# retir/Style-Big-GAN

Hardware: AMD Instinct MI355X
Metric: images/sec (G+D step) StyleGAN2-ADA 256x256 bf16 (higher is better)
Workload: dtype bf16; 1 GPU; configs/sg2ada.yaml @ 256x256: sg2_classic G (skip) + D (orig), softplus + R1(0.01)/4, idle Greg slot /16 (G lr x 16/17), global batch 64 = 1 rank(s) x 2 round(s) x batch_gpu 32 (the rounds of a phase evaluated in one pass, minibatch-std groups and loss those of the separate rounds), bf16 from 8x8 up (num_fp16_res 6; the reference recipe defaults to 4), conv_clamp 256, ADA off; global_batch=64, per_rank_batch=64, parallelism=dp1

## Files before the change

include/sbg_hip.h:

```cpp
#ifndef SBG_HIP_H
#define SBG_HIP_H

#include <stdint.h>

#ifdef __cplusplus
extern "C" {
#endif

typedef void* sbg_stream_t;

enum sbg_status {
    SBG_OK = 0,
    SBG_ERR_INVALID = 1,
    SBG_ERR_UNSUPPORTED = 2,
    SBG_ERR_LAUNCH = 3
};

enum sbg_dtype { SBG_F32 = 0, SBG_F16 = 1, SBG_BF16 = 2 };

enum sbg_act {
    SBG_ACT_LINEAR = 1, SBG_ACT_RELU = 2, SBG_ACT_LRELU = 3, SBG_ACT_TANH = 4, SBG_ACT_SIGMOID = 5,
    SBG_ACT_ELU = 6, SBG_ACT_SELU = 7, SBG_ACT_SOFTPLUS = 8, SBG_ACT_SWISH = 9
};

int         sbg_version(void);
const char* sbg_last_error(void);

int sbg_bias_act(const void* x, const void* b, const void* xref, const void* yref, const void* dy,
                 void* y, int dtype, int grad, int act, float alpha, float gain, float clamp,
                 int64_t sizeX, int sizeB, int64_t stepB, sbg_stream_t stream);

typedef struct sbg_upfirdn2d_params {
    const void*  x;
    const float* f;
    void*        y;
    int dtype;
    int upx, upy, downx, downy, padx0, pady0;
    int flip;
    float gain;
    int     inSize[4];      int64_t inStride[4];
    int     filterSize[2];  int     filterStride[2];
    int     outSize[4];     int64_t outStride[4];
    const float* oscale; const float* noise; int64_t noise_stride_n; const float* bias;
    int act; float alpha, act_gain, clamp;
    int     filter_exact16;
    const void* dact_y; float* dact_partial; int dact_act; float dact_alpha, dact_gain, dact_clamp;
    const float* post_scale;
} sbg_upfirdn2d_params;
int sbg_upfirdn2d_tail_supported(const sbg_upfirdn2d_params* p);
int64_t sbg_upfirdn2d_dact_rows(const sbg_upfirdn2d_params* p);
int sbg_upfirdn2d(const sbg_upfirdn2d_params* p, sbg_stream_t stream);

int sbg_upfirdn2d_separable_supported(int up, int down, int taps);
int sbg_upfirdn2d_separable(const float* x, const float* f, float* y, int M, int IH, int IW, int OH, int OW, int taps,
                            int up, int down, int padx0, int pady0, int flip, float gain, sbg_stream_t stream);

#define SBG_MAX_TAPS 16
typedef struct sbg_conv_params {
    const void* x; const void* w; void* y;
    const float* oscale;
    int xdtype, ydtype;
    int N, IH, IW, Cin, Cout, OH, OW;
    int64_t xs_n, xs_h, xs_w;
    int64_t ys_n, ys_h, ys_w;
    int64_t ws_slab, ws_co;
    int stride;
    int ntaps;
    int tap_dy[SBG_MAX_TAPS], tap_dx[SBG_MAX_TAPS], tap_slab[SBG_MAX_TAPS];
    int accumulate;
    const float* bias; const float* noise; int64_t noise_stride_n;
    int act; float alpha, gain, clamp;
    void* workspace; int ksplit;
    int nphase; int ph_ntaps[4], ph_oh[4], ph_ow[4]; int64_t ph_yoff[4];
} sbg_conv_params;
int64_t sbg_conv2d_igemm_workspace(const sbg_conv_params* p);
int     sbg_conv2d_igemm(const sbg_conv_params* p, sbg_stream_t stream);


typedef struct sbg_wgrad_params {
    const void* a; const void* b; float* out; void* workspace;
    int dtype;
    int N, PH, PW, Ca, BH, BW, Cb;
    int64_t as_n, as_h, as_w;
    int64_t bs_n, bs_h, bs_w;
    int stride;
    int ntaps;
    int tap_dy[SBG_MAX_TAPS], tap_dx[SBG_MAX_TAPS];
    int accumulate;
} sbg_wgrad_params;
int64_t sbg_conv2d_wgrad_workspace(const sbg_wgrad_params* p);
int     sbg_conv2d_wgrad(const sbg_wgrad_params* p, sbg_stream_t stream);


int sbg_scale_nc(const void* x, const float* a, const float* z, void* y, int dtype, int layout,
                 int N, int C, int64_t HW, int64_t z_stride_n, sbg_stream_t stream);
int sbg_scale_shift_nc(const void* x, const float* a, const float* b, void* y, int dtype, int layout,
                       int N, int C, int64_t HW, sbg_stream_t stream);

int sbg_dot_hw_splits(int layout, int N, int C, int64_t HW);
int sbg_dot_hw(const void* u, const void* v, float* partial, int dtype, int layout,
               int N, int C, int64_t HW, sbg_stream_t stream);
int sbg_moments_hw(const void* x, float* r, int dtype, int N, int C, int64_t HW, sbg_stream_t stream);

typedef struct sbg_gg_problem {
    const float *a0, *b0, *a1, *b1;
    float* c; const float* bias; float* rowsum;
    int64_t a0_rs, a0_cs, b0_rs, b0_cs, a1_rs, a1_cs, b1_rs, b1_cs, c_rs, c_cs;
    int M, N, K0, K1, nterms;
    float alpha0, alpha1, bias_scale, rowsum_scale;
} sbg_gg_problem;
int sbg_grouped_gemm(const sbg_gg_problem* problems, int count, sbg_stream_t stream);

int sbg_dot_hw_scale_supported(int C);
int sbg_dot_hw_scale(const void* u, const void* v, const float* scale, void* y, float* partial, int dtype,
                     int N, int C, int64_t HW, sbg_stream_t stream);


int sbg_modconv_bwd_supported(int C);
int sbg_modconv_bwd(const void* dy, const void* y, const float* dcoef, const float* noise, const float* bias,
                    void* d2, float* partial, float* dnoise, int dtype, int N, int C, int64_t HW, int64_t noise_stride_n,
                    int act, float alpha, float gain, float clamp, sbg_stream_t stream);
int sbg_modconv_bwd_prescaled(const void* dy, const void* y, const float* prescale, const float* dcoef, const float* noise, const float* bias,
                              void* d2, float* partial, float* partial3, float* dnoise, int dtype, int N, int C, int64_t HW,
                              int64_t noise_stride_n, int act, float alpha, float gain, float clamp, sbg_stream_t stream);

int64_t sbg_sn_workspace(int rows, int cols);
int sbg_sn_power_iteration(const float* W, const float* u, float* v, float* u_new, float* sigma, void* workspace,
                           int rows, int cols, float eps, sbg_stream_t stream);

int64_t sbg_mbstd_workspace(int N, int C, int HW, int G, int F);
int sbg_mbstd_fwd(const float* x, float* y, void* workspace, int N, int C, int HW, int G, int F, sbg_stream_t stream);
int sbg_mbstd_bwd(const float* x, const float* dy, float* dx, int N, int C, int HW, int G, int F, sbg_stream_t stream);

int sbg_split_bf16_cat(const float* x, void* y, int64_t outer, int64_t C, int64_t inner, int nseg, const int* order, sbg_stream_t stream);
int sbg_split_bf16_cat_nd(const float* x, const int64_t* shape, const int64_t* xstrides, int cat_dim, void* y, int nseg, const int* order, sbg_stream_t stream);

int sbg_attention_supported(int Q, int M, int D, int DV);
int sbg_attention_fwd(const float* theta, const float* phi, const float* g, float* out, int N, int Q, int M, int D, int DV,
                      sbg_stream_t stream);
int sbg_attention_bwd_supported(int Q, int M, int D, int DV);
int64_t sbg_attention_bwd_workspace(int N, int Q);
int sbg_attention_bwd(const float* theta, const float* phi, const float* g, const float* dout, float* dtheta, float* dphi, float* dg,
                      void* workspace, int N, int Q, int M, int D, int DV, sbg_stream_t stream);

int sbg_pack_weight(const float* w, void* out, int out_dtype, int A, int B, int KH, int KW,
                    int64_t sA, int64_t sB, int64_t sKH, int64_t sKW, int Bp, float gain, float* w2, sbg_stream_t stream);
int sbg_unpack_wgrad(const float* dwp, int64_t dwp_tap_stride, int64_t dwp_row_stride, float* dw, const float* w, const float* dw2,
                     int A, int B, int KH, int KW, int64_t sA, int64_t sB, int64_t sKH, int64_t sKW, float gain, sbg_stream_t stream);

int sbg_demod_coefs(const float* styles, const float* w2, float* dcoefs, int N, int O, int I, float eps, sbg_stream_t stream);
int sbg_demod_coefs_bwd(const float* g, const float* dcoefs, const float* styles, const float* w2, float* dstyles, float* dw2,
                        int N, int O, int I, sbg_stream_t stream);

int sbg_torgb_supported(int C, int O);
int sbg_torgb_bwd_blocks(int N, int C, int64_t HW);
int sbg_torgb_fwd(const void* x, const float* wmod, const float* bias, float* y, int dtype, int N, int C, int O, int64_t HW,
                  float clamp, sbg_stream_t stream);
int sbg_torgb_bwd(const void* x, const float* wmod, const float* dy, const float* y, void* dx, float* partial, int dtype,
                  int N, int C, int O, int64_t HW, float clamp, sbg_stream_t stream);

int sbg_fromrgb_supported(int Ci, int Co, int act);
int sbg_fromrgb_bwd_blocks(int N, int64_t HW);
int sbg_fromrgb_fwd(const float* img, const float* w, const float* bias, void* y, int dtype, int N, int Ci, int Co, int64_t HW,
                    int act, float alpha, float gain, float clamp, sbg_stream_t stream);
int sbg_fromrgb_bwd(const float* img, const float* w, const void* dy, const void* y, float* dimg, float* partial, int dtype,
                    int N, int Ci, int Co, int64_t HW, int act, float alpha, float gain, float clamp, sbg_stream_t stream);

typedef struct sbg_grid_sample_params {
    const void* x; const float* grid; const float* theta; const void* dy;
    void* y; void* dx; float* dgrid;
    int N, C, IH, IW, OH, OW;
    int64_t xs_n, xs_c, xs_h, xs_w;
    int64_t ys_n, ys_c, ys_h, ys_w;
    const float* theta_host;
} sbg_grid_sample_params;
int sbg_grid_sample2d(const sbg_grid_sample_params* p, sbg_stream_t stream);
int sbg_grid_sample2d_bwd(const sbg_grid_sample_params* p, sbg_stream_t stream);
int sbg_grid_sample2d_bwd_overwrites(const sbg_grid_sample_params* p);

int sbg_color_transform(const float* x, const float* M, float* y, int N, int64_t HW, sbg_stream_t stream);

int sbg_filter1d_batch(const float* x, const float* taps, float* y, int M, int H, int W, int T, int axis, int pad,
                       int planes_per_filter, int flip, sbg_stream_t stream);

int sbg_ppl_slerp_endpoints(const float* z0, const float* z1, const float* t, float eps, float* out, int B, int D, sbg_stream_t stream);
int sbg_ppl_lerp_endpoints(const float* w0, const float* w1, const float* t, float eps, float* out, int B, int64_t L, sbg_stream_t stream);
int sbg_ppl_prep_images(const float* img, float* out, int N, int C, int H, int W, int64_t sn, int64_t sc, int64_t sh, int64_t sw,
                        int crop, int factor, sbg_stream_t stream);
int64_t sbg_ppl_dist_workspace(int B, int64_t F);
int sbg_ppl_dist(const float* feats, float* dist, void* workspace, int B, int64_t F, float eps2, sbg_stream_t stream);

int64_t sbg_proj_noise_reg_workspace(const int* res, int nbuf);
int sbg_proj_noise_reg(const float* const* bufs, const int* res, int nbuf, float* means, float* reg, void* workspace, sbg_stream_t stream);
int sbg_proj_noise_reg_bwd(const float* const* bufs, float* const* grads, const int* res, int nbuf, const float* means, const float* g,
                           const void* workspace, sbg_stream_t stream);
int64_t sbg_proj_noise_normalize_workspace(const int* res, int nbuf);
int sbg_proj_noise_normalize(float* const* bufs, const int* res, int nbuf, void* workspace, sbg_stream_t stream);
int64_t sbg_proj_sqdist_workspace(int64_t F);
int sbg_proj_sqdist(const float* t, const float* s, float* dist, void* workspace, int64_t F, sbg_stream_t stream);
int sbg_proj_sqdist_bwd(const float* t, const float* s, const float* g, float* ds, int64_t F, sbg_stream_t stream);

enum sbg_quant_rule { SBG_QUANT_GRID = 0, SBG_QUANT_CLAMP = 1 };
int sbg_img_quantize_tile(const float* img, uint8_t* canvas, int N, int C, int H, int W, int64_t sn, int64_t sc, int64_t sh, int64_t sw,
                          int gw, int gh, int cell0, int rule, float lo, float scale, sbg_stream_t stream);
int sbg_ws_truncate_mix(const float* W, const float* w_avg, float psi, const int* rows, const int* cols, const int* mask, float* out,
                        int S, int L, int D, int R, int Cn, sbg_stream_t stream);

int sbg_u8_resample_h(const uint8_t* src, int64_t src_img_stride, int64_t src_pitch, uint8_t* dst, int64_t dst_img_stride, int64_t dst_pitch,
                      int N, int rows, int in_w, int out_w, int C, const int* bounds, const int* coeffs_t, int ksize, int strip, int span,
                      sbg_stream_t stream);
int sbg_u8_resample_v(const uint8_t* src, int64_t src_img_stride, int64_t src_pitch, uint8_t* dst, int64_t dst_img_stride, int64_t dst_pitch,
                      int N, int row_bytes, int in_h, int out_h, const int* bounds, const int* coeffs, int ksize, sbg_stream_t stream);

int64_t sbg_knn_workspace(int R, int C, int k, int membership);
int sbg_knn_kth_radius(const void* rows, const void* manifold, int R, int C, int64_t F, int k, void* out, void* workspace, sbg_stream_t stream);
int sbg_knn_in_manifold(const void* probes, const void* manifold, const void* radius, int P, int C, int64_t F, uint8_t* out, void* workspace,
                        sbg_stream_t stream);
int64_t sbg_knn_probe_workspace(int P, int C);
int sbg_knn_probe(const void* probes, const void* manifold, const void* radius, int P, int C, int64_t F, int32_t* count, void* nearest,
                  void* workspace, sbg_stream_t stream);

int64_t sbg_grad_finish_records(int64_t n);
int sbg_grad_finish_sweep(float* flat, int64_t n, float scale, double* partials, sbg_stream_t stream);
int sbg_grad_finish_merge(const double* partials, int64_t records, double* result, sbg_stream_t stream);

int sbg_u8_gather_images(const uint8_t* store, int64_t S, int C, int H, int W, const int32_t* slot, const uint8_t* flip, int B, void* out,
                         int out_f32, const float* lut, sbg_stream_t stream);

#define SBG_DIFFAUG_WORDS 12
int64_t sbg_diffaug_workspace(int N, int C, int H, int W);
int sbg_diffaug_fwd(const float* x, const int32_t* table, float* y, float* workspace, int N, int C, int H, int W, int drop_b, sbg_stream_t stream);
int sbg_diffaug_adj(const float* g, const int32_t* table, float* dx, float* workspace, int N, int C, int H, int W, sbg_stream_t stream);

enum sbg_kernel_kind {
    SBG_K_BIAS_ACT = 1, SBG_K_UPFIRDN2D = 2, SBG_K_CONV_IGEMM = 3, SBG_K_CONV_WGRAD = 4, SBG_K_WGRAD_REDUCE = 5,
    SBG_K_SCALE_NC = 6, SBG_K_DOT_HW = 7, SBG_K_SN_POWER = 9, SBG_K_ATTENTION = 10, SBG_K_GRID_SAMPLE = 11, SBG_K_FILTER1D = 12, SBG_K_COLOR = 13, SBG_K_WEIGHT_PREP = 14, SBG_K_TORGB = 15, SBG_K_FROMRGB = 16,
    SBG_K_GROUPED_GEMM = 17, SBG_K_PPL = 18,
    SBG_K_PROJECTOR = 19,
    SBG_K_IMAGE_EXPORT = 20,
    SBG_K_RESAMPLE = 21,
    SBG_K_PR = 22,
    SBG_K_GRAD_FINISH = 23,
    SBG_K_RESIDENT = 24,
    SBG_K_DIFFAUG = 25
};
typedef struct sbg_prof_record {
    int    kind;
    int    dims[7];
    double flops;
    double bytes;
    float  ms;
    int    pad;
} sbg_prof_record;
int sbg_prof_enable(int on);
int sbg_prof_fetch(sbg_prof_record* out, int max);

#ifdef __cplusplus
}
#endif
#endif
```

style-big-gan_amd/_lib.py:

```python
import ctypes
import os
import threading

import torch

_HERE = os.path.dirname(os.path.abspath(__file__))
LIB_PATH = os.environ.get("SBG_HIP_LIBRARY") or os.path.join(_HERE, "libsbg_hip.so")

SBG_F32, SBG_F16, SBG_BF16 = 0, 1, 2
SBG_MAX_TAPS = 16

_DTYPES = {torch.float32: SBG_F32, torch.float16: SBG_F16, torch.bfloat16: SBG_BF16}


def dtype_code(dtype):
    try:
        return _DTYPES[dtype]
    except KeyError:
        raise RuntimeError(f"style_big_gan_amd: unsupported dtype {dtype} (float32 / float16 / bfloat16 only)")


class UpfirdnParams(ctypes.Structure):
    _fields_ = [
        ("x", ctypes.c_void_p), ("f", ctypes.c_void_p), ("y", ctypes.c_void_p),
        ("dtype", ctypes.c_int),
        ("upx", ctypes.c_int), ("upy", ctypes.c_int), ("downx", ctypes.c_int), ("downy", ctypes.c_int),
        ("padx0", ctypes.c_int), ("pady0", ctypes.c_int),
        ("flip", ctypes.c_int), ("gain", ctypes.c_float),
        ("inSize", ctypes.c_int * 4), ("inStride", ctypes.c_int64 * 4),
        ("filterSize", ctypes.c_int * 2), ("filterStride", ctypes.c_int * 2),
        ("outSize", ctypes.c_int * 4), ("outStride", ctypes.c_int64 * 4),
        ("oscale", ctypes.c_void_p), ("noise", ctypes.c_void_p), ("noise_stride_n", ctypes.c_int64), ("bias", ctypes.c_void_p),
        ("act", ctypes.c_int), ("alpha", ctypes.c_float), ("act_gain", ctypes.c_float), ("clamp", ctypes.c_float),
        ("filter_exact16", ctypes.c_int),
        ("dact_y", ctypes.c_void_p), ("dact_partial", ctypes.c_void_p), ("dact_act", ctypes.c_int),
        ("dact_alpha", ctypes.c_float), ("dact_gain", ctypes.c_float), ("dact_clamp", ctypes.c_float),
        ("post_scale", ctypes.c_void_p),
    ]


class ConvParams(ctypes.Structure):
    _fields_ = [
        ("x", ctypes.c_void_p), ("w", ctypes.c_void_p), ("y", ctypes.c_void_p), ("oscale", ctypes.c_void_p),
        ("xdtype", ctypes.c_int), ("ydtype", ctypes.c_int),
        ("N", ctypes.c_int), ("IH", ctypes.c_int), ("IW", ctypes.c_int), ("Cin", ctypes.c_int), ("Cout", ctypes.c_int),
        ("OH", ctypes.c_int), ("OW", ctypes.c_int),
        ("xs_n", ctypes.c_int64), ("xs_h", ctypes.c_int64), ("xs_w", ctypes.c_int64),
        ("ys_n", ctypes.c_int64), ("ys_h", ctypes.c_int64), ("ys_w", ctypes.c_int64),
        ("ws_slab", ctypes.c_int64), ("ws_co", ctypes.c_int64),
        ("stride", ctypes.c_int), ("ntaps", ctypes.c_int),
        ("tap_dy", ctypes.c_int * SBG_MAX_TAPS), ("tap_dx", ctypes.c_int * SBG_MAX_TAPS), ("tap_slab", ctypes.c_int * SBG_MAX_TAPS),
        ("accumulate", ctypes.c_int),
        ("bias", ctypes.c_void_p), ("noise", ctypes.c_void_p), ("noise_stride_n", ctypes.c_int64),
        ("act", ctypes.c_int), ("alpha", ctypes.c_float), ("gain", ctypes.c_float), ("clamp", ctypes.c_float),
        ("workspace", ctypes.c_void_p), ("ksplit", ctypes.c_int),
        ("nphase", ctypes.c_int), ("ph_ntaps", ctypes.c_int * 4), ("ph_oh", ctypes.c_int * 4), ("ph_ow", ctypes.c_int * 4), ("ph_yoff", ctypes.c_int64 * 4),
    ]


class WgradParams(ctypes.Structure):
    _fields_ = [
        ("a", ctypes.c_void_p), ("b", ctypes.c_void_p), ("out", ctypes.c_void_p), ("workspace", ctypes.c_void_p),
        ("dtype", ctypes.c_int),
        ("N", ctypes.c_int), ("PH", ctypes.c_int), ("PW", ctypes.c_int), ("Ca", ctypes.c_int),
        ("BH", ctypes.c_int), ("BW", ctypes.c_int), ("Cb", ctypes.c_int),
        ("as_n", ctypes.c_int64), ("as_h", ctypes.c_int64), ("as_w", ctypes.c_int64),
        ("bs_n", ctypes.c_int64), ("bs_h", ctypes.c_int64), ("bs_w", ctypes.c_int64),
        ("stride", ctypes.c_int), ("ntaps", ctypes.c_int),
        ("tap_dy", ctypes.c_int * SBG_MAX_TAPS), ("tap_dx", ctypes.c_int * SBG_MAX_TAPS),
        ("accumulate", ctypes.c_int),
    ]


class GridSampleParams(ctypes.Structure):
    _fields_ = [
        ("x", ctypes.c_void_p), ("grid", ctypes.c_void_p), ("theta", ctypes.c_void_p), ("dy", ctypes.c_void_p),
        ("y", ctypes.c_void_p), ("dx", ctypes.c_void_p), ("dgrid", ctypes.c_void_p),
        ("N", ctypes.c_int), ("C", ctypes.c_int), ("IH", ctypes.c_int), ("IW", ctypes.c_int), ("OH", ctypes.c_int), ("OW", ctypes.c_int),
        ("xs_n", ctypes.c_int64), ("xs_c", ctypes.c_int64), ("xs_h", ctypes.c_int64), ("xs_w", ctypes.c_int64),
        ("ys_n", ctypes.c_int64), ("ys_c", ctypes.c_int64), ("ys_h", ctypes.c_int64), ("ys_w", ctypes.c_int64),
        ("theta_host", ctypes.c_void_p),
    ]


class GgProblem(ctypes.Structure):
    _fields_ = [("a0", ctypes.c_void_p), ("b0", ctypes.c_void_p), ("a1", ctypes.c_void_p), ("b1", ctypes.c_void_p),
                ("c", ctypes.c_void_p), ("bias", ctypes.c_void_p), ("rowsum", ctypes.c_void_p),
                ("a0_rs", ctypes.c_int64), ("a0_cs", ctypes.c_int64), ("b0_rs", ctypes.c_int64), ("b0_cs", ctypes.c_int64),
                ("a1_rs", ctypes.c_int64), ("a1_cs", ctypes.c_int64), ("b1_rs", ctypes.c_int64), ("b1_cs", ctypes.c_int64),
                ("c_rs", ctypes.c_int64), ("c_cs", ctypes.c_int64),
                ("M", ctypes.c_int), ("N", ctypes.c_int), ("K0", ctypes.c_int), ("K1", ctypes.c_int), ("nterms", ctypes.c_int),
                ("alpha0", ctypes.c_float), ("alpha1", ctypes.c_float), ("bias_scale", ctypes.c_float), ("rowsum_scale", ctypes.c_float)]


class ProfRecord(ctypes.Structure):
    _fields_ = [("kind", ctypes.c_int), ("dims", ctypes.c_int * 7), ("flops", ctypes.c_double), ("bytes", ctypes.c_double),
                ("ms", ctypes.c_float), ("pad", ctypes.c_int)]


KERNEL_KINDS = {1: "bias_act", 2: "upfirdn2d", 3: "conv_igemm", 4: "conv_wgrad", 5: "wgrad_reduce", 6: "scale_nc", 7: "dot_hw", 9: "sn_power", 10: "attention",
                11: "grid_sample", 12: "filter1d", 13: "color", 14: "weight_prep", 15: "torgb", 16: "fromrgb", 17: "grouped_gemm", 18: "ppl",
                19: "projector", 20: "image_export", 21: "resample", 22: "pr", 23: "grad_finish", 24: "resident", 25: "diffaug"}
RESIDENT_PATHS = {1: "dword", 2: "byte"}
PPL_VARIANTS = {0: "slerp", 1: "lerp", 2: "prep", 3: "dist"}
PROJ_VARIANTS = {0: "reg", 1: "reg_bwd", 2: "normalize", 3: "sqdist", 4: "sqdist_bwd"}
IMG_VARIANTS = {0: "quantize_tile", 1: "truncate_mix"}
QUANT_RULES = {"grid": 0, "clamp": 1}
RESAMPLE_VARIANTS = {0: "h", 1: "v"}
PR_VARIANTS = {0: "single", 1: "split", 2: "merge", 3: "norms"}
GRAD_FINISH_VARIANTS = {0: "sweep", 1: "merge"}
DIFFAUG_VARIANTS = {0: "sum", 1: "apply", 2: "adj_sum", 3: "adj_apply", 4: "single", 5: "adj_single"}
DIFFAUG_WORDS = 12
ATT_VARIANTS = {0: "single", 1: "stream", 2: "stream_stats", 3: "stream_dq", 4: "stream_dkv"}

_lib = None
_lock = threading.Lock()

_c = ctypes
SYMBOLS = [
    ("sbg_version", _c.c_int, []),
    ("sbg_last_error", _c.c_char_p, []),
    ("sbg_bias_act", _c.c_int, [_c.c_void_p] * 6 + [_c.c_int, _c.c_int, _c.c_int, _c.c_float, _c.c_float, _c.c_float,
                                                   _c.c_int64, _c.c_int, _c.c_int64, _c.c_void_p]),
    ("sbg_upfirdn2d_tail_supported", _c.c_int, [_c.POINTER(UpfirdnParams)]),
    ("sbg_upfirdn2d", _c.c_int, [_c.POINTER(UpfirdnParams), _c.c_void_p]),
    ("sbg_upfirdn2d_dact_rows", _c.c_int64, [_c.POINTER(UpfirdnParams)]),
    ("sbg_upfirdn2d_separable_supported", _c.c_int, [_c.c_int] * 3),
    ("sbg_upfirdn2d_separable", _c.c_int, [_c.c_void_p] * 3 + [_c.c_int] * 11 + [_c.c_float, _c.c_void_p]),
    ("sbg_conv2d_igemm_workspace", _c.c_int64, [_c.POINTER(ConvParams)]),
    ("sbg_conv2d_igemm", _c.c_int, [_c.POINTER(ConvParams), _c.c_void_p]),
    ("sbg_conv2d_wgrad_workspace", _c.c_int64, [_c.POINTER(WgradParams)]),
    ("sbg_conv2d_wgrad", _c.c_int, [_c.POINTER(WgradParams), _c.c_void_p]),
    ("sbg_scale_nc", _c.c_int, [_c.c_void_p] * 4 + [_c.c_int, _c.c_int, _c.c_int, _c.c_int, _c.c_int64, _c.c_int64, _c.c_void_p]),
    ("sbg_scale_shift_nc", _c.c_int, [_c.c_void_p] * 4 + [_c.c_int, _c.c_int, _c.c_int, _c.c_int, _c.c_int64, _c.c_void_p]),
    ("sbg_sn_workspace", _c.c_int64, [_c.c_int, _c.c_int]),
    ("sbg_sn_power_iteration", _c.c_int, [_c.c_void_p] * 6 + [_c.c_int, _c.c_int, _c.c_float, _c.c_void_p]),
    ("sbg_mbstd_workspace", _c.c_int64, [_c.c_int] * 5),
    ("sbg_mbstd_fwd", _c.c_int, [_c.c_void_p] * 3 + [_c.c_int] * 5 + [_c.c_void_p]),
    ("sbg_mbstd_bwd", _c.c_int, [_c.c_void_p] * 3 + [_c.c_int] * 5 + [_c.c_void_p]),
    ("sbg_split_bf16_cat", _c.c_int, [_c.c_void_p, _c.c_void_p, _c.c_int64, _c.c_int64, _c.c_int64, _c.c_int, _c.POINTER(_c.c_int), _c.c_void_p]),
    ("sbg_split_bf16_cat_nd", _c.c_int, [_c.c_void_p, _c.POINTER(_c.c_int64), _c.POINTER(_c.c_int64), _c.c_int, _c.c_void_p, _c.c_int, _c.POINTER(_c.c_int), _c.c_void_p]),
    ("sbg_attention_supported", _c.c_int, [_c.c_int] * 4),
    ("sbg_attention_fwd", _c.c_int, [_c.c_void_p] * 4 + [_c.c_int] * 5 + [_c.c_void_p]),
    ("sbg_attention_bwd_supported", _c.c_int, [_c.c_int] * 4),
    ("sbg_attention_bwd_workspace", _c.c_int64, [_c.c_int, _c.c_int]),
    ("sbg_attention_bwd", _c.c_int, [_c.c_void_p] * 8 + [_c.c_int] * 5 + [_c.c_void_p]),
    ("sbg_dot_hw_splits", _c.c_int, [_c.c_int, _c.c_int, _c.c_int, _c.c_int64]),
    ("sbg_dot_hw", _c.c_int, [_c.c_void_p] * 3 + [_c.c_int, _c.c_int, _c.c_int, _c.c_int, _c.c_int64, _c.c_void_p]),
    ("sbg_moments_hw", _c.c_int, [_c.c_void_p, _c.c_void_p, _c.c_int, _c.c_int, _c.c_int, _c.c_int64, _c.c_void_p]),
    ("sbg_grouped_gemm", _c.c_int, [_c.c_void_p, _c.c_int, _c.c_void_p]),
    ("sbg_dot_hw_scale_supported", _c.c_int, [_c.c_int]),
    ("sbg_dot_hw_scale", _c.c_int, [_c.c_void_p] * 5 + [_c.c_int, _c.c_int, _c.c_int, _c.c_int64, _c.c_void_p]),
    ("sbg_modconv_bwd_supported", _c.c_int, [_c.c_int]),
    ("sbg_modconv_bwd", _c.c_int, [_c.c_void_p] * 8 + [_c.c_int, _c.c_int, _c.c_int, _c.c_int64, _c.c_int64, _c.c_int, _c.c_float, _c.c_float, _c.c_float, _c.c_void_p]),
    ("sbg_modconv_bwd_prescaled", _c.c_int, [_c.c_void_p] * 10 + [_c.c_int, _c.c_int, _c.c_int, _c.c_int64, _c.c_int64, _c.c_int, _c.c_float, _c.c_float, _c.c_float, _c.c_void_p]),
    ("sbg_pack_weight", _c.c_int, [_c.c_void_p, _c.c_void_p, _c.c_int, _c.c_int, _c.c_int, _c.c_int, _c.c_int] + [_c.c_int64] * 4
     + [_c.c_int, _c.c_float, _c.c_void_p, _c.c_void_p]),
    ("sbg_unpack_wgrad", _c.c_int, [_c.c_void_p, _c.c_int64, _c.c_int64, _c.c_void_p, _c.c_void_p, _c.c_void_p] + [_c.c_int] * 4
     + [_c.c_int64] * 4 + [_c.c_float, _c.c_void_p]),
    ("sbg_demod_coefs", _c.c_int, [_c.c_void_p] * 3 + [_c.c_int] * 3 + [_c.c_float, _c.c_void_p]),
    ("sbg_demod_coefs_bwd", _c.c_int, [_c.c_void_p] * 6 + [_c.c_int] * 3 + [_c.c_void_p]),
    ("sbg_torgb_supported", _c.c_int, [_c.c_int, _c.c_int]),
    ("sbg_torgb_bwd_blocks", _c.c_int, [_c.c_int, _c.c_int, _c.c_int64]),
    ("sbg_torgb_fwd", _c.c_int, [_c.c_void_p] * 4 + [_c.c_int] * 4 + [_c.c_int64, _c.c_float, _c.c_void_p]),
    ("sbg_torgb_bwd", _c.c_int, [_c.c_void_p] * 6 + [_c.c_int] * 4 + [_c.c_int64, _c.c_float, _c.c_void_p]),
    ("sbg_fromrgb_supported", _c.c_int, [_c.c_int] * 3),
    ("sbg_fromrgb_bwd_blocks", _c.c_int, [_c.c_int, _c.c_int64]),
    ("sbg_fromrgb_fwd", _c.c_int, [_c.c_void_p] * 4 + [_c.c_int] * 4 + [_c.c_int64, _c.c_int, _c.c_float, _c.c_float, _c.c_float, _c.c_void_p]),
    ("sbg_fromrgb_bwd", _c.c_int, [_c.c_void_p] * 6 + [_c.c_int] * 4 + [_c.c_int64, _c.c_int, _c.c_float, _c.c_float, _c.c_float, _c.c_void_p]),
    ("sbg_grid_sample2d", _c.c_int, [_c.POINTER(GridSampleParams), _c.c_void_p]),
    ("sbg_grid_sample2d_bwd", _c.c_int, [_c.POINTER(GridSampleParams), _c.c_void_p]),
    ("sbg_grid_sample2d_bwd_overwrites", _c.c_int, [_c.POINTER(GridSampleParams)]),
    ("sbg_color_transform", _c.c_int, [_c.c_void_p] * 3 + [_c.c_int, _c.c_int64, _c.c_void_p]),
    ("sbg_filter1d_batch", _c.c_int, [_c.c_void_p] * 3 + [_c.c_int] * 8 + [_c.c_void_p]),
    ("sbg_ppl_slerp_endpoints", _c.c_int, [_c.c_void_p] * 3 + [_c.c_float, _c.c_void_p, _c.c_int, _c.c_int, _c.c_void_p]),
    ("sbg_ppl_lerp_endpoints", _c.c_int, [_c.c_void_p] * 3 + [_c.c_float, _c.c_void_p, _c.c_int, _c.c_int64, _c.c_void_p]),
    ("sbg_ppl_prep_images", _c.c_int, [_c.c_void_p] * 2 + [_c.c_int] * 4 + [_c.c_int64] * 4 + [_c.c_int, _c.c_int, _c.c_void_p]),
    ("sbg_ppl_dist_workspace", _c.c_int64, [_c.c_int, _c.c_int64]),
    ("sbg_ppl_dist", _c.c_int, [_c.c_void_p] * 3 + [_c.c_int, _c.c_int64, _c.c_float, _c.c_void_p]),
    ("sbg_proj_noise_reg_workspace", _c.c_int64, [_c.c_void_p, _c.c_int]),
    ("sbg_proj_noise_reg", _c.c_int, [_c.c_void_p] * 2 + [_c.c_int] + [_c.c_void_p] * 4),
    ("sbg_proj_noise_reg_bwd", _c.c_int, [_c.c_void_p] * 3 + [_c.c_int] + [_c.c_void_p] * 4),
    ("sbg_proj_noise_normalize_workspace", _c.c_int64, [_c.c_void_p, _c.c_int]),
    ("sbg_proj_noise_normalize", _c.c_int, [_c.c_void_p] * 2 + [_c.c_int] + [_c.c_void_p] * 2),
    ("sbg_proj_sqdist_workspace", _c.c_int64, [_c.c_int64]),
    ("sbg_proj_sqdist", _c.c_int, [_c.c_void_p] * 4 + [_c.c_int64, _c.c_void_p]),
    ("sbg_proj_sqdist_bwd", _c.c_int, [_c.c_void_p] * 4 + [_c.c_int64, _c.c_void_p]),
    ("sbg_img_quantize_tile", _c.c_int, [_c.c_void_p] * 2 + [_c.c_int] * 4 + [_c.c_int64] * 4 + [_c.c_int] * 4 + [_c.c_float] * 2 + [_c.c_void_p]),
    ("sbg_ws_truncate_mix", _c.c_int, [_c.c_void_p] * 2 + [_c.c_float] + [_c.c_void_p] * 4 + [_c.c_int] * 5 + [_c.c_void_p]),
    ("sbg_u8_resample_h", _c.c_int, [_c.c_void_p, _c.c_int64, _c.c_int64] * 2 + [_c.c_int] * 5 + [_c.c_void_p] * 2 + [_c.c_int] * 3 + [_c.c_void_p]),
    ("sbg_u8_resample_v", _c.c_int, [_c.c_void_p, _c.c_int64, _c.c_int64] * 2 + [_c.c_int] * 4 + [_c.c_void_p] * 2 + [_c.c_int, _c.c_void_p]),
    ("sbg_knn_workspace", _c.c_int64, [_c.c_int] * 4),
    ("sbg_knn_kth_radius", _c.c_int, [_c.c_void_p] * 2 + [_c.c_int, _c.c_int, _c.c_int64, _c.c_int] + [_c.c_void_p] * 3),
    ("sbg_knn_in_manifold", _c.c_int, [_c.c_void_p] * 3 + [_c.c_int, _c.c_int, _c.c_int64] + [_c.c_void_p] * 3),
    ("sbg_knn_probe_workspace", _c.c_int64, [_c.c_int] * 2),
    ("sbg_knn_probe", _c.c_int, [_c.c_void_p] * 3 + [_c.c_int, _c.c_int, _c.c_int64] + [_c.c_void_p] * 4),
    ("sbg_grad_finish_records", _c.c_int64, [_c.c_int64]),
    ("sbg_grad_finish_sweep", _c.c_int, [_c.c_void_p, _c.c_int64, _c.c_float, _c.c_void_p, _c.c_void_p]),
    ("sbg_grad_finish_merge", _c.c_int, [_c.c_void_p, _c.c_int64, _c.c_void_p, _c.c_void_p]),
    ("sbg_u8_gather_images", _c.c_int, [_c.c_void_p, _c.c_int64, _c.c_int, _c.c_int, _c.c_int, _c.c_void_p, _c.c_void_p, _c.c_int, _c.c_void_p, _c.c_int,
                                        _c.c_void_p, _c.c_void_p]),
    ("sbg_diffaug_workspace", _c.c_int64, [_c.c_int] * 4),
    ("sbg_diffaug_fwd", _c.c_int, [_c.c_void_p] * 4 + [_c.c_int] * 5 + [_c.c_void_p]),
    ("sbg_diffaug_adj", _c.c_int, [_c.c_void_p] * 4 + [_c.c_int] * 4 + [_c.c_void_p]),
    ("sbg_prof_enable", _c.c_int, [_c.c_int]),
    ("sbg_prof_fetch", _c.c_int, [_c.POINTER(ProfRecord), _c.c_int]),
]


def load():
    global _lib
    if _lib is not None:
        return _lib
    with _lock:
        if _lib is not None:
            return _lib
        if not os.path.isfile(LIB_PATH):
            raise RuntimeError(
                f"style_big_gan_amd: HIP extension {LIB_PATH} not found. Build it with "
                f"`make -C {os.path.join(_HERE, 'csrc')}` or `python -c 'import __graft_entry__ as g; g.build()'`. "
                "There is no CPU fallback.")
        lib = ctypes.CDLL(LIB_PATH)
        for name, restype, argtypes in SYMBOLS:
            fn = getattr(lib, name)
            fn.restype = restype
            fn.argtypes = argtypes
        _lib = lib
    return _lib


def check(status, what):
    if status != 0:
        msg = load().sbg_last_error()
        raise RuntimeError(f"{what} failed (status {status}): {msg.decode() if msg else ''}")


def stream_ptr(device=None):
    return ctypes.c_void_p(torch.cuda.current_stream(device).cuda_stream)


def ptr(t):
    return ctypes.c_void_p(t.data_ptr()) if t is not None else None


def require_cuda(t, what):
    if t.device.type != "cuda":
        raise RuntimeError(
            f"{what}: tensor is on '{t.device}'. style_big_gan_amd ops run only as HIP kernels on a ROCm device "
            "(device type 'cuda'); there is no CPU path in the product (the CPU restatement lives in oracle/ and is test-only).")


def require_dtype(t, dtype, what):
    if t.dtype != dtype:
        raise RuntimeError(f"{what}: expects {str(dtype).replace('torch.', '')}, got {t.dtype}")
    return t


def workspace(nbytes, device, what):
    if nbytes < 0:
        check(1, what)
    return torch.empty([max((nbytes + 3) // 4, 1)], dtype=torch.float32, device=device)


def prof_enable(on):
    return load().sbg_prof_enable(int(bool(on)))


def prof_fetch():
    lib = load()
    n = lib.sbg_prof_fetch(None, 0)
    if n <= 0:
        return []
    buf = (ProfRecord * n)()
    n = lib.sbg_prof_fetch(buf, n)
    return [dict(kind=KERNEL_KINDS.get(r.kind, str(r.kind)), dims=tuple(r.dims), flops=r.flops, bytes=r.bytes, ms=r.ms) for r in buf[:n]]
```

style-big-gan_amd/csrc/conv_wgrad.hip:

```cpp
#include "conv_common.h"
#include "lds_asm.h"

namespace {

struct bf16_mfma {}; struct f16_mfma {};
template <class MF> struct Mfma;
template <> struct Mfma<bf16_mfma> {
    static __device__ __forceinline__ float4_t run(short8_t a, short8_t b, float4_t c) {
        return __builtin_amdgcn_mfma_f32_16x16x32_bf16(__builtin_bit_cast(bf16x8_t, a), __builtin_bit_cast(bf16x8_t, b), c, 0, 0, 0);
    }
};
template <> struct Mfma<f16_mfma> {
    static __device__ __forceinline__ float4_t run(short8_t a, short8_t b, float4_t c) {
        return __builtin_amdgcn_mfma_f32_16x16x32_f16(__builtin_bit_cast(f16x8_t, a), __builtin_bit_cast(f16x8_t, b), c, 0, 0, 0);
    }
};

struct WgradArgs {
    const unsigned short* a; const unsigned short* b; float* out; float* ws;
    int N, PH, PW, Ca, BH, BW, Cb;
    int64_t as_n, as_h, as_w, bs_n, bs_h, bs_w;
    int stride, ntaps;
    int tap_dy[SBG_MAX_TAPS], tap_dx[SBG_MAX_TAPS];
    int accumulate;
// ... 196 lines not shown
    const int xblocks = p.PW >> 5;
    const int dy0 = p.tap_dy[0], dx0 = p.tap_dx[0];

    __amdgpu_buffer_rsrc_t ar = __builtin_amdgcn_make_buffer_rsrc((void*)p.a, 0, (int)a_bytes, 0x00020000);
    __amdgpu_buffer_rsrc_t br = __builtin_amdgcn_make_buffer_rsrc((void*)p.b, 0, (int)b_bytes, 0x00020000);

    const int drow = lane >> 3, dchunk = lane & 7;
    auto src_chunk = [&](int R) { return (((dchunk >> 1) ^ ((R >> 1) & 3)) << 1) | (dchunk & 1); };

    struct ChunkC { int py, n, px0; unsigned char* st; };
    auto chunk_coords = [&](int loc) -> ChunkC {
        const int c = chunk_begin + loc;
        const int xb = c % xblocks, rowid = c / xblocks;
        ChunkC r; r.py = rowid % p.PH; r.n = rowid / p.PH; r.px0 = xb << 5; r.st = smem + (loc % NSTAGE) * STAGE;
        return r;
    };
    auto issue_piece = [&](const ChunkC& cc, int i) {
        const int py = cc.py, n = cc.n, px0 = cc.px0;
        unsigned char* st = cc.st;
        {
            const int piece = wave + NWAVE * i;
            if (piece < APIECES) {
                const int R = (piece & 3) * 8 + drow;
                const int ch = ca0 + (piece >> 2) * 64 + src_chunk(R) * 8;
                const unsigned okm = 0u - (unsigned)(ch < p.Ca);
                const unsigned real = (unsigned)(n * (int)p.as_n + py * (int)p.as_h + (px0 + R) * (int)p.as_w + ch) * 2u;
                __builtin_amdgcn_raw_ptr_buffer_load_lds(ar, (lds_void_ptr)(st + piece * 1024), 16, (real & okm) | (SBG_OOB_OFFSET & ~okm), 0, 0, 0);
            } else {
                const int q = piece - APIECES;
                const int r = q / PPR, jb = q - r * PPR;
                const int R = r * PROW + jb * 8 + drow;
                constexpr int NEVEN = (PCOLS + 1) / 2, EVROWS = ((NEVEN + 7) / 8) * 8;
                const int pcol = (S == 1) ? jb * 8 + drow : (jb * 8 < EVROWS ? 2 * (jb * 8 + drow) : 2 * (jb * 8 - EVROWS + drow) + 1);
                const int by = S * py + dy0 + r, bx = S * px0 + dx0 + pcol;
                const int ch = cb0 + src_chunk(R) * 8;
                const unsigned okm = 0u - (unsigned)((q < 3 * PPR) & (pcol < PCOLS) & ((unsigned)by < (unsigned)p.BH) & ((unsigned)bx < (unsigned)p.BW) & (ch < p.Cb));
                const unsigned real = (unsigned)(n * (int)p.bs_n + by * (int)p.bs_h + bx * (int)p.bs_w + ch) * 2u;
                unsigned char* dst = (q < 3 * PPR) ? st + A_BYTES + q * 1024 : smem + DUMP;
                __builtin_amdgcn_raw_ptr_buffer_load_lds(br, (lds_void_ptr)dst, 16, (real & okm) | (SBG_OOB_OFFSET & ~okm), 0, 0, 0);
            }
        }
    };
    auto issue = [&](int loc) {
        const ChunkC cc = chunk_coords(loc);
#pragma unroll
        for (int i = 0; i < PIECES; i++) issue_piece(cc, i);
    };
    constexpr bool late = true;

    const int wa = (wave >> 2) * (BCA / 2), wb = (wave & 3) * 16;
    const int fi = lane & 15, fg = lane >> 4, fq = fi >> 2, fp = fi & 3;
    const unsigned lds_base = (unsigned)(uintptr_t)((lds_void_ptr)smem);
    float4_t acc[NT][TA];
#pragma unroll
    for (int t = 0; t < NT; t++)
#pragma unroll
        for (int i = 0; i < TA; i++) acc[t][i] = float4_t{0.f, 0.f, 0.f, 0.f};

    auto frag_off = [&](int Rrel, int col) {
        const int chunk = (col >> 3) + (fp >> 1);
        const int sw = (((chunk >> 1) ^ ((Rrel >> 1) & 3)) << 1) | (chunk & 1);
        return Rrel * 128 + sw * 16 + (fp & 1) * 8;
    };
    int offA[TA], offB[3];
#pragma unroll
    for (int i = 0; i < TA; i++) {
        const int col = wa + 16 * i;
        offA[i] = (col >> 6) * 4096 + frag_off(4 * fg + fq, col & 63);
    }
#pragma unroll
    for (int d = 0; d < 3; d++) {
        constexpr int EVROWS_ = (((PCOLS + 1) / 2 + 7) / 8) * 8;
        offB[d] = frag_off((S == 1 ? d : (d & 1) * EVROWS_ + (d >> 1)) + 4 * fg + fq, wb);
    }
    auto read_frag = [&](const unsigned char* base, int off, int hi_off) -> short8_t {
        short4_t lo = lds_tr_read(base + off), hi = lds_tr_read(base + off + hi_off);
        return short8_t{lo[0], lo[1], lo[2], lo[3], hi[0], hi[1], hi[2], hi[3]};
    };

#pragma unroll
    for (int s = 0; s < DEPTH; s++) if (s < nloc) issue(s);
    for (int s = 0; s < nloc; s++) {
        {
            const int later = nloc - 1 - s;
            if (DEPTH >= 2 && later >= DEPTH - 1) asm volatile("s_waitcnt vmcnt(%0)" :: "n"((DEPTH - 1) * PIECES) : "memory");
            else if (DEPTH >= 3 && later == DEPTH - 2) asm volatile("s_waitcnt vmcnt(%0)" :: "n"((DEPTH >= 3 ? DEPTH - 2 : 0) * PIECES) : "memory");
            else if (DEPTH >= 4 && later == DEPTH - 3) asm volatile("s_waitcnt vmcnt(%0)" :: "n"((DEPTH >= 4 ? DEPTH - 3 : 0) * PIECES) : "memory");
            else if (DEPTH >= 5 && later == DEPTH - 4) asm volatile("s_waitcnt vmcnt(%0)" :: "n"((DEPTH >= 5 ? DEPTH - 4 : 0) * PIECES) : "memory");
            else                                       asm volatile("s_waitcnt vmcnt(0)" ::: "memory");
        }
        __builtin_amdgcn_s_barrier();
        const bool more = s + DEPTH < nloc;
        ChunkC nxt = chunk_coords(more ? s + DEPTH : s);
        if (more && !late) {
#pragma unroll
            for (int i = 0; i < PIECES; i++) issue_piece(nxt, i);
        }
        const unsigned stage = lds_base + (unsigned)((s % NSTAGE) * STAGE);
        short4_t alo[TA], ahi[TA], blo[3], bhi[3];
        sbg_static_for<TA>([&](auto it) {
            constexpr int i = decltype(it)::value;
            lds_tr_issue<0>(alo[i], stage + (unsigned)offA[i]);
            lds_tr_issue<16 * 128>(ahi[i], stage + (unsigned)offA[i]);
        });
        unsigned pb[3];
#pragma unroll
        for (int d = 0; d < 3; d++) pb[d] = stage + (unsigned)offB[d];
        auto issue_b = [&](auto tt) {
            constexpr int t = decltype(tt)::value, dyi = t / 3, dxi = t % 3, OFF = A_BYTES + dyi * PROW * 128;
            lds_tr_issue<OFF>(blo[t % 3], pb[dxi]);
            lds_tr_issue<OFF + 16 * 128>(bhi[t % 3], pb[dxi]);
        };
        issue_b(std::integral_constant<int, 0>{});
        issue_b(std::integral_constant<int, 1>{});
        sbg_static_for<9>([&](auto tt) {
            constexpr int t = decltype(tt)::value;
            if constexpr (t + 2 < 9) issue_b(std::integral_constant<int, t + 2>{});
            lds_wait<(t + 2 < 9 ? 4 : t + 1 < 9 ? 2 : 0)>(blo[t % 3], bhi[t % 3]);
            const short8_t fb = short8_t{blo[t % 3][0], blo[t % 3][1], blo[t % 3][2], blo[t % 3][3], bhi[t % 3][0], bhi[t % 3][1], bhi[t % 3][2], bhi[t % 3][3]};
#pragma unroll
            for (int i = 0; i < TA; i++) {
                const short8_t fa_i = short8_t{alo[i][0], alo[i][1], alo[i][2], alo[i][3], ahi[i][0], ahi[i][1], ahi[i][2], ahi[i][3]};
                acc[t][i] = Mfma<MF>::run(fa_i, fb, acc[t][i]);
            }
            if (more && late) {
                sbg_static_for<PIECES>([&](auto pt) {
                    constexpr int i = decltype(pt)::value;
                    if constexpr (i * 9 / PIECES == t) issue_piece(nxt, i);
                });
            }
        });
    }

    const bool direct = (p.nsplit == 1);
    float* dst_base = direct ? p.out : p.ws + (int64_t)split * p.ntaps_total * p.Ca * p.Cb;
    const int cb = cb0 + wb + fi;
#pragma unroll
    for (int t = 0; t < NT; t++) {
        if (t >= p.ntaps || cb >= p.Cb) continue;
        float* slab = dst_base + (int64_t)(p.tap0 + t) * p.Ca * p.Cb;
#pragma unroll
        for (int i = 0; i < TA; i++)
#pragma unroll
            for (int e = 0; e < 4; e++) {
                const int ca = ca0 + wa + 16 * i + 4 * fg + e;
                if (ca >= p.Ca) continue;
                float* d = slab + (int64_t)ca * p.Cb + cb;
                const float v = acc[t][i][e];
                *d = (direct && p.accumulate) ? *d + v : v;
            }
    }
}

template <int LANES>
__global__ __launch_bounds__(256) void wgrad_reduce_kernel(const float* ws, float* out, int64_t n, int nsplit, int accumulate)
{
    const int sub = threadIdx.x % LANES;
    const int64_t step = (int64_t)gridDim.x * (256 / LANES);
    for (int64_t i = (int64_t)blockIdx.x * (256 / LANES) + threadIdx.x / LANES; i < n; i += step) {
        float s = 0.f;
        int k = sub;
        for (; k + 7 * LANES < nsplit; k += 8 * LANES) {
            float v[8];
#pragma unroll
            for (int u = 0; u < 8; u++) v[u] = ws[(int64_t)(k + u * LANES) * n + i];
#pragma unroll
            for (int u = 0; u < 8; u++) s += v[u];
        }
        for (; k < nsplit; k += LANES) s += ws[(int64_t)k * n + i];
#pragma unroll
        for (int m = LANES >> 1; m >= 1; m >>= 1) s += __shfl_xor(s, m, 64);
        if (sub == 0) out[i] = accumulate ? out[i] + s : s;
    }
}

template <class MF, int TA, int TB>
__global__ __launch_bounds__(256) void conv_wgrad_thin_kernel(WgradArgs p, int dymin, int dxmin, int RY, int PCOLS, int wave_lds)
{
    extern __shared__ __attribute__((aligned(16))) unsigned char smem[];
    const int tid = threadIdx.x, lane = tid & 63, wave = tid >> 6;
    unsigned short* la = reinterpret_cast<unsigned short*>(smem + wave * wave_lds);
    unsigned short* lb = la + 32 * p.Ca;
    const int slab = blockIdx.x * 4 + wave;
    const int nwaves = gridDim.x * 4;
    const int xblocks = (p.PW + 31) >> 5;
    const int nchunks = p.N * p.PH * xblocks;
    const int fi = lane & 15, fg = lane >> 4;
    const int ca8 = p.Ca >> 3, cb8 = p.Cb >> 3;
    float4_t acc[9][TA][TB];
#pragma unroll
    for (int t = 0; t < 9; t++)
#pragma unroll
        for (int i = 0; i < TA; i++)
#pragma unroll
            for (int j = 0; j < TB; j++) acc[t][i][j] = float4_t{0.f, 0.f, 0.f, 0.f};
    int tdy[9], tdx[9];
#pragma unroll
    for (int t = 0; t < 9; t++) { tdy[t] = (t < p.ntaps ? p.tap_dy[t] : 0) - dymin; tdx[t] = (t < p.ntaps ? p.tap_dx[t] : 0) - dxmin; }

    for (int c = slab; c < nchunks; c += nwaves) {
        const int xb = c % xblocks, rowid = c / xblocks;
        const int py = rowid % p.PH, n = rowid / p.PH;
        const int px0 = xb << 5;
        for (int piece = lane; piece < 32 * ca8; piece += 64) {
            const int px = piece / ca8, ch = (piece - px * ca8) * 8;
            short8_t v = {0, 0, 0, 0, 0, 0, 0, 0};
            if (px0 + px < p.PW) v = *reinterpret_cast<const short8_t*>(p.a + (int64_t)n * p.as_n + (int64_t)py * p.as_h + (int64_t)(px0 + px) * p.as_w + ch);
            *reinterpret_cast<short8_t*>(la + piece * 8) = v;
        }
        const int npieces = RY * PCOLS * cb8;
        for (int piece = lane; piece < npieces; piece += 64) {
            const int ch = (piece % cb8) * 8, pc = piece / cb8;
            const int col = pc % PCOLS, r = pc / PCOLS;
            const int by = p.stride * py + dymin + r, bx = p.stride * px0 + dxmin + col;
            short8_t v = {0, 0, 0, 0, 0, 0, 0, 0};
            if ((unsigned)by < (unsigned)p.BH && (unsigned)bx < (unsigned)p.BW)
                v = *reinterpret_cast<const short8_t*>(p.b + (int64_t)n * p.bs_n + (int64_t)by * p.bs_h + (int64_t)bx * p.bs_w + ch);
            *reinterpret_cast<short8_t*>(lb + piece * 8) = v;
        }
        __builtin_amdgcn_s_waitcnt(0xC07F);
        __builtin_amdgcn_wave_barrier();
        short8_t fa[TA];
#pragma unroll
        for (int i = 0; i < TA; i++)
#pragma unroll
            for (int j = 0; j < 8; j++) fa[i][j] = (short)la[(8 * fg + j) * p.Ca + 16 * i + fi];
#pragma unroll
        for (int t = 0; t < 9; t++) {
            if (t < p.ntaps) {
                const unsigned short* row = lb + (tdy[t] * PCOLS + tdx[t]) * p.Cb;
#pragma unroll
                for (int jb = 0; jb < TB; jb++) {
                    short8_t fb;
#pragma unroll
                    for (int j = 0; j < 8; j++) fb[j] = (short)row[(p.stride * (8 * fg + j)) * p.Cb + 16 * jb + fi];
#pragma unroll
                    for (int i = 0; i < TA; i++) acc[t][i][jb] = Mfma<MF>::run(fa[i], fb, acc[t][i][jb]);
                }
            }
        }
        __builtin_amdgcn_wave_barrier();
    }
    float* dst = p.ws + (int64_t)slab * p.ntaps_total * p.Ca * p.Cb;
#pragma unroll
    for (int t = 0; t < 9; t++) {
        if (t < p.ntaps) {
#pragma unroll
            for (int i = 0; i < TA; i++)
#pragma unroll
                for (int jb = 0; jb < TB; jb++)
#pragma unroll
                    for (int e = 0; e < 4; e++) {
                        const int ca = 16 * i + 4 * fg + e, cb = 16 * jb + fi;
                        if (ca < p.Ca && cb < p.Cb) dst[((int64_t)(p.tap0 + t) * p.Ca + ca) * p.Cb + cb] = acc[t][i][jb][e];
                    }
        }
    }
}

struct ThinPlan { bool ok; int dymin, dxmin, RY, PCOLS, wave_lds, nwg; };

static ThinPlan thin_plan(const sbg_wgrad_params* q)
{
    ThinPlan t; t.ok = false;
    if (q->Ca > 32 || q->Cb > 32 || q->Ca * q->Cb > 512 || q->ntaps > 9 || q->ntaps < 1 || q->stride < 1 || q->stride > 2 || q->N < 1) return t;
    int dy0 = q->tap_dy[0], dy1 = dy0, dx0 = q->tap_dx[0], dx1 = dx0;
    for (int i = 1; i < q->ntaps; i++) {
        if (q->tap_dy[i] < dy0) dy0 = q->tap_dy[i]; if (q->tap_dy[i] > dy1) dy1 = q->tap_dy[i];
        if (q->tap_dx[i] < dx0) dx0 = q->tap_dx[i]; if (q->tap_dx[i] > dx1) dx1 = q->tap_dx[i];
    }
    if (dy1 - dy0 > 2 || dx1 - dx0 > 2) return t;
    t.dymin = dy0; t.dxmin = dx0; t.RY = dy1 - dy0 + 1; t.PCOLS = q->stride * 31 + (dx1 - dx0) + 1;
    t.wave_lds = ((32 * q->Ca + t.RY * t.PCOLS * q->Cb) * 2 + 15) & ~15;
    const int64_t nchunks = (int64_t)q->N * q->PH * ((q->PW + 31) / 32);
    int64_t nwg = (nchunks + 15) / 16;
    if (nwg > 2048) nwg = 2048;
    if (nwg < 1) nwg = 1;
    t.nwg = (int)nwg;
    t.ok = nchunks < INT32_MAX;
    return t;
}

static void plan_split(WgradArgs& a, int bca, int bcb, int target)
{
    a.atiles = (a.Ca + bca - 1) / bca;
    a.btiles = (a.Cb + bcb - 1) / bcb;
    a.nchunks = (int)((a.P + 31) / 32);
    const int tiles = a.atiles * a.btiles;
    int want = (target + tiles - 1) / tiles;
    int maxsplit = a.nchunks / 8; if (maxsplit < 1) maxsplit = 1;
    if (want > maxsplit) want = maxsplit;
    if (want < 1) want = 1;
    a.chunks_per_split = (a.nchunks + want - 1) / want;
    a.nsplit = (a.nchunks + a.chunks_per_split - 1) / a.chunks_per_split;
}

static bool use_big_tile(int ntaps) { return ntaps == 1; }

static int rows_bca(const WgradArgs& a)
{
    return a.Ca >= 128 ? 128 : 64;
}

static constexpr int rows_nstage(int stride, int bca)
{
    if (bca == 128) return 4;
    return stride == 1 ? 4 : 2;
}

static bool rows_kernel_ok(const sbg_wgrad_params* q, const WgradArgs& a)
{
    if ((q->stride != 1 && q->stride != 2) || (q->PW % 32) != 0 || q->ntaps != 9) return false;
    for (int t = 0; t < 9; t++)
        if (q->tap_dy[t] != q->tap_dy[0] + t / 3 || q->tap_dx[t] != q->tap_dx[0] + t % 3) return false;
    if (q->as_n < 0 || q->as_h < 0 || q->as_w < 0 || q->bs_n < 0 || q->bs_h < 0 || q->bs_w < 0) return false;
    const int64_t ab = 2 * ((int64_t)(q->N - 1) * q->as_n + (int64_t)(q->PH - 1) * q->as_h + (int64_t)(q->PW - 1) * q->as_w + q->Ca);
    const int64_t bb = 2 * ((int64_t)(q->N - 1) * q->bs_n + (int64_t)(q->BH - 1) * q->bs_h + (int64_t)(q->BW - 1) * q->bs_w + q->Cb);
    return ab < (int64_t)SBG_OOB_OFFSET && bb < (int64_t)SBG_OOB_OFFSET && a.P > 0;
}

static int fill_args(const sbg_wgrad_params* q, WgradArgs& a)
{
    SBG_CHECK(q && q->a && q->b && q->out, "conv2d_wgrad: null pointer");
    SBG_CHECK(q->dtype == SBG_BF16 || q->dtype == SBG_F16, "conv2d_wgrad: a/b must be bf16 or f16 (fp32 inputs are split by the host)");
    SBG_CHECK(q->N >= 0 && q->PH >= 1 && q->PW >= 1 && q->BH >= 1 && q->BW >= 1, "conv2d_wgrad: bad sizes");
    SBG_CHECK(q->Ca >= 8 && q->Cb >= 8 && (q->Ca % 8) == 0 && (q->Cb % 8) == 0, "conv2d_wgrad: channel counts must be multiples of 8 (pad on the host)");
    SBG_CHECK(q->ntaps >= 1 && q->ntaps <= SBG_MAX_TAPS, "conv2d_wgrad: 1..%d taps", SBG_MAX_TAPS);
    SBG_CHECK(q->stride >= 1, "conv2d_wgrad: stride must be >= 1");
    SBG_CHECK(sbg_aligned16(q->a) && sbg_aligned16(q->b), "conv2d_wgrad: a and b must be 16-byte aligned");
    SBG_CHECK((q->as_n % 8) == 0 && (q->as_h % 8) == 0 && (q->as_w % 8) == 0 && (q->bs_n % 8) == 0 && (q->bs_h % 8) == 0 && (q->bs_w % 8) == 0,
              "conv2d_wgrad: pixel / row strides must be multiples of 8 elements");
    a.a = (const unsigned short*)q->a; a.b = (const unsigned short*)q->b; a.out = q->out; a.ws = (float*)q->workspace;
    a.N = q->N; a.PH = q->PH; a.PW = q->PW; a.Ca = q->Ca; a.BH = q->BH; a.BW = q->BW; a.Cb = q->Cb;
    a.as_n = q->as_n; a.as_h = q->as_h; a.as_w = q->as_w; a.bs_n = q->bs_n; a.bs_h = q->bs_h; a.bs_w = q->bs_w;
    a.stride = q->stride; a.ntaps = q->ntaps; a.accumulate = q->accumulate;
    for (int t = 0; t < SBG_MAX_TAPS; t++) { a.tap_dy[t] = q->tap_dy[t]; a.tap_dx[t] = q->tap_dx[t]; }
    a.P = (int64_t)q->N * q->PH * q->PW;
    a.tap0 = 0; a.ntaps_total = q->ntaps;
    if (use_big_tile(q->ntaps)) plan_split(a, 128, 128, 1024); else plan_split(a, 64, 64, 1024);
    if (rows_kernel_ok(q, a)) plan_split(a, rows_bca(a), 64, 512);
    const ThinPlan tp = thin_plan(q);
    if (tp.ok) { a.atiles = a.btiles = 1; a.nsplit = 4 * tp.nwg; a.chunks_per_split = 0; }
    return SBG_OK;
}

template <class MF, int BCA, int BCB, int NT>
static int launch_wgrad(const WgradArgs& a, hipStream_t stream)
{
    constexpr int lds = 32 * (BCA * 2 + 32) + NT * 32 * (BCB * 2 + 32);
    auto kern = conv_wgrad_kernel<MF, BCA, BCB, NT>;
    if (lds > 64 * 1024 && !SBG_RAISE_LDS_ONCE(kern, lds))
        return sbg_fail(SBG_ERR_LAUNCH, "conv2d_wgrad: cannot raise the dynamic LDS limit to %d bytes", lds);
    SbgProfScope prof(stream, SBG_K_CONV_WGRAD, 2.0 * (double)a.P * a.Ca * (double)a.Cb * a.ntaps,
                      2.0 * (double)a.P * a.Ca + 2.0 * (double)a.N * a.BH * a.BW * a.Cb + 4.0 * a.ntaps * (double)a.Ca * a.Cb * (a.nsplit > 1 ? a.nsplit : 1),
                      {(int)(a.P > INT32_MAX ? INT32_MAX : a.P), a.Ca, a.Cb, a.ntaps, a.stride, a.nsplit, BCA * 1000 + BCB});
    SBG_LAUNCH(kern, dim3(wgrad_grid(a)), dim3(256), lds, stream, a);
    SBG_HIP_LAUNCH_CHECK();
    return SBG_OK;
}

}

extern "C" int64_t sbg_conv2d_wgrad_workspace(const sbg_wgrad_params* q)
{
    WgradArgs a;
    if (fill_args(q, a) != SBG_OK) return -1;
    if (a.nsplit <= 1) return 0;
    return (int64_t)a.nsplit * a.ntaps_total * a.Ca * a.Cb * (int64_t)sizeof(float);
}

extern "C" int sbg_conv2d_wgrad(const sbg_wgrad_params* q, sbg_stream_t stream)
{
    WgradArgs a;
    int rc = fill_args(q, a);
    if (rc != SBG_OK) return rc;
    hipStream_t s = (hipStream_t)stream;
    const int64_t out_n = (int64_t)a.ntaps_total * a.Ca * a.Cb;
    if (a.P == 0) {
        if (!a.accumulate) { if (hipMemsetAsync(a.out, 0, out_n * sizeof(float), s) != hipSuccess) return sbg_fail(SBG_ERR_LAUNCH, "conv2d_wgrad: memset failed"); }
        return SBG_OK;
    }
    SBG_CHECK(a.nsplit == 1 || a.ws != nullptr, "conv2d_wgrad: workspace required (%d pixel splits)", a.nsplit);
    const bool bf = (q->dtype == SBG_BF16);
    const ThinPlan tp = thin_plan(q);
    if (tp.ok) {
        const int ta = (a.Ca + 15) / 16, tb = (a.Cb + 15) / 16;
        const int lds = 4 * tp.wave_lds;
        SbgProfScope prof(s, SBG_K_CONV_WGRAD, 2.0 * (double)a.P * a.Ca * (double)a.Cb * a.ntaps,
                          2.0 * (double)a.P * a.Ca + 2.0 * (double)a.N * a.BH * a.BW * a.Cb + 4.0 * a.ntaps * (double)a.Ca * a.Cb * a.nsplit,
                          {(int)(a.P > INT32_MAX ? INT32_MAX : a.P), a.Ca, a.Cb, a.ntaps, a.stride, a.nsplit, 3000000 + ta * 10 + tb});
#define SBG_THIN_LAUNCH(MFT, A_, B_) do { auto kern = conv_wgrad_thin_kernel<MFT, A_, B_>; \
        if (lds > 64 * 1024 && !SBG_RAISE_LDS_ONCE(kern, lds)) return sbg_fail(SBG_ERR_LAUNCH, "conv2d_wgrad: cannot raise the dynamic LDS limit to %d bytes", lds); \
        SBG_LAUNCH(kern, dim3((unsigned)tp.nwg), dim3(256), lds, s, a, tp.dymin, tp.dxmin, tp.RY, tp.PCOLS, tp.wave_lds); } while (0)
        if (bf) { if (ta == 1 && tb == 1) SBG_THIN_LAUNCH(bf16_mfma, 1, 1); else if (ta == 2 && tb == 1) SBG_THIN_LAUNCH(bf16_mfma, 2, 1);
                  else if (ta == 1) SBG_THIN_LAUNCH(bf16_mfma, 1, 2); else SBG_THIN_LAUNCH(bf16_mfma, 2, 2); }
        else    { if (ta == 1 && tb == 1) SBG_THIN_LAUNCH(f16_mfma, 1, 1); else if (ta == 2 && tb == 1) SBG_THIN_LAUNCH(f16_mfma, 2, 1);
                  else if (ta == 1) SBG_THIN_LAUNCH(f16_mfma, 1, 2); else SBG_THIN_LAUNCH(f16_mfma, 2, 2); }
#undef SBG_THIN_LAUNCH
        SBG_HIP_LAUNCH_CHECK();
    } else if (rows_kernel_ok(q, a)) {
        const unsigned ab = (unsigned)(2 * ((int64_t)(q->N - 1) * q->as_n + (int64_t)(q->PH - 1) * q->as_h + (int64_t)(q->PW - 1) * q->as_w + q->Ca));
        const unsigned bb = (unsigned)(2 * ((int64_t)(q->N - 1) * q->bs_n + (int64_t)(q->BH - 1) * q->bs_h + (int64_t)(q->BW - 1) * q->bs_w + q->Cb));
        const int bca = rows_bca(a);
        const int s_ = q->stride;
        auto stage_kib = [](int S, int BCA) { const int ppr = (S * 31 + 3 + 7) / 8; return BCA / 16 + 3 * ppr; };
        const int lds = (rows_nstage(s_, bca) * stage_kib(s_, bca) + 1) * 1024;
        SbgProfScope prof(s, SBG_K_CONV_WGRAD, 2.0 * (double)a.P * a.Ca * (double)a.Cb * a.ntaps,
                          2.0 * (double)a.P * a.Ca + 2.0 * (double)a.N * a.BH * a.BW * a.Cb + 4.0 * a.ntaps * (double)a.Ca * a.Cb * (a.nsplit > 1 ? a.nsplit : 1),
                          {(int)(a.P > INT32_MAX ? INT32_MAX : a.P), a.Ca, a.Cb, a.ntaps, a.stride, a.nsplit, 1000000 + bca * 1000 + 64});
        const dim3 grid(wgrad_grid(a));
#define SBG_ROWS_LAUNCH(MFT, SS, BB) do { auto kern = conv_wgrad_rows_kernel<MFT, SS, BB, rows_nstage(SS, BB)>; \
        if (lds > 64 * 1024 && !SBG_RAISE_LDS_ONCE(kern, lds)) return sbg_fail(SBG_ERR_LAUNCH, "conv2d_wgrad: cannot raise the dynamic LDS limit to %d bytes", lds); \
        SBG_LAUNCH(kern, grid, dim3(512), lds, s, a, ab, bb); } while (0)
        if (s_ == 1 && bca == 64)       { if (bf) SBG_ROWS_LAUNCH(bf16_mfma, 1, 64);  else SBG_ROWS_LAUNCH(f16_mfma, 1, 64); }
        else if (s_ == 1)               { if (bf) SBG_ROWS_LAUNCH(bf16_mfma, 1, 128); else SBG_ROWS_LAUNCH(f16_mfma, 1, 128); }
        else if (bca == 64)             { if (bf) SBG_ROWS_LAUNCH(bf16_mfma, 2, 64);  else SBG_ROWS_LAUNCH(f16_mfma, 2, 64); }
        else                            { if (bf) SBG_ROWS_LAUNCH(bf16_mfma, 2, 128); else SBG_ROWS_LAUNCH(f16_mfma, 2, 128); }
#undef SBG_ROWS_LAUNCH
        SBG_HIP_LAUNCH_CHECK();
    } else if (use_big_tile(a.ntaps)) {
        rc = bf ? launch_wgrad<bf16_mfma, 128, 128, 1>(a, s) : launch_wgrad<f16_mfma, 128, 128, 1>(a, s);
        if (rc != SBG_OK) return rc;
    } else {
        const int total = a.ntaps;
        for (int t0 = 0; t0 < total; t0 += 9) {
            WgradArgs g = a;
            g.tap0 = t0; g.ntaps = (total - t0 < 9) ? total - t0 : 9;
            for (int t = 0; t < g.ntaps; t++) { g.tap_dy[t] = a.tap_dy[t0 + t]; g.tap_dx[t] = a.tap_dx[t0 + t]; }
            rc = bf ? launch_wgrad<bf16_mfma, 64, 64, 9>(g, s) : launch_wgrad<f16_mfma, 64, 64, 9>(g, s);
            if (rc != SBG_OK) return rc;
        }
    }
    if (a.nsplit > 1) {
        SbgProfScope prof(s, SBG_K_WGRAD_REDUCE, 0.0, 4.0 * out_n * (a.nsplit + 1), {(int)out_n, a.nsplit});
        if (out_n >= (1 << 18) || a.nsplit < 16)
            SBG_LAUNCH(wgrad_reduce_kernel<1>, dim3(sbg_stream_grid(out_n, 256)), dim3(256), 0, s, a.ws, a.out, out_n, a.nsplit, a.accumulate);
        else if (out_n >= (1 << 14))
            SBG_LAUNCH(wgrad_reduce_kernel<4>, dim3(sbg_stream_grid(out_n * 4, 256)), dim3(256), 0, s, a.ws, a.out, out_n, a.nsplit, a.accumulate);
        else
            SBG_LAUNCH(wgrad_reduce_kernel<64>, dim3(sbg_stream_grid(out_n * 64, 256)), dim3(256), 0, s, a.ws, a.out, out_n, a.nsplit, a.accumulate);
        SBG_HIP_LAUNCH_CHECK();
    }
    return SBG_OK;
}
```

style-big-gan_amd/csrc/weight_prep.hip:

```cpp
#include "sbg_common.h"

namespace {

struct PackArgs {
    const float* w; void* out; float* w2;
    int A, B, KH, KW, Bp, dtype;
    int64_t sA, sB, sKH, sKW;
    float gain;
};

template <class T>
__global__ void __launch_bounds__(256) pack_weight_kernel(PackArgs p)
{
    const int64_t total = (int64_t)p.A * p.Bp;
    const int taps = p.KH * p.KW;
    T* out = (T*)p.out;
    for (int64_t i = (int64_t)blockIdx.x * blockDim.x + threadIdx.x; i < total; i += (int64_t)gridDim.x * blockDim.x) {
        const int b = (int)(i % p.Bp), a = (int)(i / p.Bp);
        const bool real = b < p.B;
        const float* src = p.w + (int64_t)a * p.sA + (int64_t)b * p.sB;
        float sq = 0.0f;
        for (int kh = 0; kh < p.KH; kh++)
            for (int kw = 0; kw < p.KW; kw++) {
                const float v = real ? src[kh * p.sKH + kw * p.sKW] * p.gain : 0.0f;
                sq += v * v;
                Elem<T>::st(out + ((int64_t)(kh * p.KW + kw) * p.A + a) * p.Bp + b, v);
            }
        if (p.w2 && real) p.w2[(int64_t)a * p.B + b] = sq;
    }
}

template <class T>
__global__ void __launch_bounds__(256) pack_weight_t_kernel(PackArgs p)
{
    __shared__ float tile[32][33];
    const int tx = threadIdx.x & 31, ty = threadIdx.x >> 5;
    const int a0 = blockIdx.x * 32, b0 = blockIdx.y * 32, t = blockIdx.z;
    const int kh = t / p.KW, kw = t - kh * p.KW;
    const float* src = p.w + (int64_t)kh * p.sKH + (int64_t)kw * p.sKW;
#pragma unroll
    for (int r = 0; r < 4; r++) {
        const int a = a0 + tx, b = b0 + ty + 8 * r;
        tile[ty + 8 * r][tx] = (a < p.A && b < p.B) ? src[(int64_t)a * p.sA + (int64_t)b * p.sB] * p.gain : 0.0f;
    }
    __syncthreads();
    T* out = (T*)p.out + (int64_t)t * p.A * p.Bp;
#pragma unroll
    for (int r = 0; r < 4; r++) {
        const int a = a0 + ty + 8 * r, b = b0 + tx;
        if (a < p.A && b < p.Bp) Elem<T>::st(out + (int64_t)a * p.Bp + b, tile[tx][ty + 8 * r]);
    }
}

struct UnpackArgs {
    const float* dwp; float* dw; const float* w; const float* dw2;
    int A, B, KH, KW;
    int64_t pT, pA;
    int64_t sA, sB, sKH, sKW;
    float gain;
};

__global__ void __launch_bounds__(256) unpack_wgrad_kernel(UnpackArgs p)
{
    const int64_t total = (int64_t)p.A * p.B;
    for (int64_t i = (int64_t)blockIdx.x * blockDim.x + threadIdx.x; i < total; i += (int64_t)gridDim.x * blockDim.x) {
        const int b = (int)(i % p.B), a = (int)(i / p.B);
        const int64_t off = (int64_t)a * p.sA + (int64_t)b * p.sB;
        const float extra = p.dw2 ? 2.0f * p.gain * p.gain * p.dw2[(int64_t)a * p.B + b] : 0.0f;
        for (int kh = 0; kh < p.KH; kh++)
            for (int kw = 0; kw < p.KW; kw++) {
                const int64_t o = off + kh * p.sKH + kw * p.sKW;
                float v = p.dwp ? p.gain * p.dwp[(int64_t)(kh * p.KW + kw) * p.pT + (int64_t)a * p.pA + b] : 0.0f;
                if (p.dw2) v += extra * p.w[o];
                p.dw[o] = v;
            }
    }
}

}

extern "C" int sbg_pack_weight(const float* w, void* out, int out_dtype, int A, int B, int KH, int KW,
                               int64_t sA, int64_t sB, int64_t sKH, int64_t sKW, int Bp, float gain, float* w2, sbg_stream_t stream_)
{
    SBG_CHECK(w && out, "pack_weight: null pointer");
    SBG_CHECK(A >= 1 && B >= 1 && KH >= 1 && KW >= 1 && Bp >= B, "pack_weight: bad sizes");
    SBG_CHECK((int64_t)A * Bp * KH * KW <= INT32_MAX, "pack_weight: tensor too large");
    PackArgs a;
    a.w = w; a.out = out; a.w2 = w2; a.A = A; a.B = B; a.KH = KH; a.KW = KW; a.Bp = Bp; a.dtype = out_dtype;
    a.sA = sA; a.sB = sB; a.sKH = sKH; a.sKW = sKW; a.gain = gain;
    hipStream_t stream = (hipStream_t)stream_;
    const int64_t total = (int64_t)A * Bp;
    const bool transposing = !w2 && sA == 1 && sB >= 64 && A >= 32 && B >= 32 && KH * KW <= 65535;
    SbgProfScope prof(stream, SBG_K_WEIGHT_PREP, 0.0, (double)A * B * KH * KW * (4.0 + sbg_dtype_size(out_dtype)), {A, B, KH * KW, 0, transposing ? 1 : 2, 0, 0});
    dim3 grid(sbg_stream_grid(total, 256)), block(256);
    if (transposing) {
        const dim3 tgrid((unsigned)((A + 31) / 32), (unsigned)((Bp + 31) / 32), (unsigned)(KH * KW));
        if (out_dtype == SBG_BF16)      SBG_LAUNCH(pack_weight_t_kernel<bf16_s>, tgrid, block, 0, stream, a);
        else if (out_dtype == SBG_F16)  SBG_LAUNCH(pack_weight_t_kernel<f16_s>, tgrid, block, 0, stream, a);
        else if (out_dtype == SBG_F32)  SBG_LAUNCH(pack_weight_t_kernel<float>, tgrid, block, 0, stream, a);
        else return sbg_fail(SBG_ERR_INVALID, "pack_weight: bad dtype %d", out_dtype);
        SBG_HIP_LAUNCH_CHECK();
        return 0;
    }
    if (out_dtype == SBG_BF16)      SBG_LAUNCH(pack_weight_kernel<bf16_s>, grid, block, 0, stream, a);
    else if (out_dtype == SBG_F16)  SBG_LAUNCH(pack_weight_kernel<f16_s>, grid, block, 0, stream, a);
    else if (out_dtype == SBG_F32)  SBG_LAUNCH(pack_weight_kernel<float>, grid, block, 0, stream, a);
    else return sbg_fail(SBG_ERR_INVALID, "pack_weight: bad dtype %d", out_dtype);
    SBG_HIP_LAUNCH_CHECK();
    return 0;
}

extern "C" int sbg_unpack_wgrad(const float* dwp, int64_t dwp_tap_stride, int64_t dwp_row_stride, float* dw, const float* w, const float* dw2,
                                int A, int B, int KH, int KW, int64_t sA, int64_t sB, int64_t sKH, int64_t sKW, float gain, sbg_stream_t stream_)
{
    SBG_CHECK(dw && (dwp || dw2), "unpack_wgrad: null pointer");
    SBG_CHECK(!dw2 || w, "unpack_wgrad: dw2 needs w");
    SBG_CHECK(A >= 1 && B >= 1 && KH >= 1 && KW >= 1, "unpack_wgrad: bad sizes");
    UnpackArgs a;
    a.dwp = dwp; a.dw = dw; a.w = w; a.dw2 = dw2; a.A = A; a.B = B; a.KH = KH; a.KW = KW;
    a.pT = dwp_tap_stride; a.pA = dwp_row_stride; a.sA = sA; a.sB = sB; a.sKH = sKH; a.sKW = sKW; a.gain = gain;
    hipStream_t stream = (hipStream_t)stream_;
    SbgProfScope prof(stream, SBG_K_WEIGHT_PREP, 0.0, (double)A * B * KH * KW * 8.0, {A, B, KH * KW, 1, 0, 0, 0});
    SBG_LAUNCH(unpack_wgrad_kernel, dim3(sbg_stream_grid((int64_t)A * B, 256)), dim3(256), 0, stream, a);
    SBG_HIP_LAUNCH_CHECK();
    return 0;
}

namespace {

__global__ void __launch_bounds__(256) demod_coefs_kernel(const float* __restrict__ s, const float* __restrict__ w2, float* __restrict__ d,
                                                          int N, int O, int I, float eps)
{
    const int lane = threadIdx.x & 63;
    const int64_t pair = (int64_t)blockIdx.x * 4 + (threadIdx.x >> 6);
    if (pair >= (int64_t)N * O) return;
    const int n = (int)(pair / O), o = (int)(pair % O);
    const float* sr = s + (int64_t)n * I;
    const float* wr = w2 + (int64_t)o * I;
    float acc = 0.0f;
    for (int i = lane; i < I; i += 64) { const float sv = sr[i]; acc += sv * sv * wr[i]; }
#pragma unroll
    for (int m = 32; m >= 1; m >>= 1) acc += __shfl_xor(acc, m, 64);
    if (lane == 0) d[pair] = rsqrtf(acc + eps);
}

__global__ void __launch_bounds__(256) demod_bwd_styles_kernel(const float* __restrict__ g, const float* __restrict__ d, const float* __restrict__ s,
                                                               const float* __restrict__ w2, float* __restrict__ ds, int N, int O, int I)
{
    extern __shared__ float q[];
    float* part = q + O;
    const int chunks = (I + 63) / 64;
    const int n = blockIdx.x / chunks, lane = threadIdx.x & 63, wave = threadIdx.x >> 6;
    const int i = (blockIdx.x % chunks) * 64 + lane;
    for (int o = threadIdx.x; o < O; o += 256) { const float dv = d[(int64_t)n * O + o]; q[o] = -0.5f * g[(int64_t)n * O + o] * dv * dv * dv; }
    __syncthreads();
    float acc = 0.0f;
    if (i < I) {
        int o = wave;
        for (; o + 28 < O; o += 32) {
            float v[8];
#pragma unroll
            for (int u = 0; u < 8; u++) v[u] = w2[(int64_t)(o + 4 * u) * I + i];
#pragma unroll
            for (int u = 0; u < 8; u++) acc += q[o + 4 * u] * v[u];
        }
        for (; o < O; o += 4) acc += q[o] * w2[(int64_t)o * I + i];
    }
    part[wave * 64 + lane] = acc;
    __syncthreads();
    if (wave == 0 && i < I)
        ds[(int64_t)n * I + i] = 2.0f * s[(int64_t)n * I + i] * (part[lane] + part[64 + lane] + part[128 + lane] + part[192 + lane]);
}

__global__ void __launch_bounds__(256) demod_bwd_w2_kernel(const float* __restrict__ g, const float* __restrict__ d, const float* __restrict__ s,
                                                           float* __restrict__ dw2, int N, int O, int I)
{
    const int64_t idx = (int64_t)blockIdx.x * 256 + threadIdx.x;
    if (idx >= (int64_t)O * I) return;
    const int o = (int)(idx / I), i = (int)(idx % I);
    float acc = 0.0f;
#pragma unroll 8
    for (int n = 0; n < N; n++) {
        const float dv = d[(int64_t)n * O + o], sv = s[(int64_t)n * I + i];
        acc += (-0.5f * g[(int64_t)n * O + o] * dv * dv * dv) * sv * sv;
    }
    dw2[idx] = acc;
}

}

extern "C" int sbg_demod_coefs(const float* styles, const float* w2, float* dcoefs, int N, int O, int I, float eps, sbg_stream_t stream_)
{
    SBG_CHECK(styles && w2 && dcoefs && N >= 1 && O >= 1 && I >= 1, "demod_coefs: bad arguments");
    hipStream_t stream = (hipStream_t)stream_;
    SbgProfScope prof(stream, SBG_K_WEIGHT_PREP, 2.0 * N * O * (double)I, 4.0 * ((double)N * I + (double)O * I + (double)N * O), {N, O, I, 2, 0, 0, 0});
    SBG_LAUNCH(demod_coefs_kernel, dim3((unsigned)(((int64_t)N * O + 3) / 4)), dim3(256), 0, stream, styles, w2, dcoefs, N, O, I, eps);
    SBG_HIP_LAUNCH_CHECK();
    return 0;
}

extern "C" int sbg_demod_coefs_bwd(const float* g, const float* dcoefs, const float* styles, const float* w2, float* dstyles, float* dw2,
                                   int N, int O, int I, sbg_stream_t stream_)
{
    SBG_CHECK(g && dcoefs && styles && w2 && (dstyles || dw2) && N >= 1 && O >= 1 && I >= 1, "demod_coefs_bwd: bad arguments");
    SBG_CHECK((O + 256) * sizeof(float) <= 64 * 1024, "demod_coefs_bwd: too many output channels");
    hipStream_t stream = (hipStream_t)stream_;
    SbgProfScope prof(stream, SBG_K_WEIGHT_PREP, 4.0 * N * O * (double)I, 4.0 * (2.0 * N * I + 2.0 * O * I + 2.0 * N * O), {N, O, I, 3, 0, 0, 0});
    if (dstyles) {
        const int chunks = (I + 63) / 64;
        SBG_LAUNCH(demod_bwd_styles_kernel, dim3((unsigned)(N * chunks)), dim3(256), (O + 256) * sizeof(float), stream, g, dcoefs, styles, w2, dstyles, N, O, I);
        SBG_HIP_LAUNCH_CHECK();
    }
    if (dw2) {
        SBG_LAUNCH(demod_bwd_w2_kernel, dim3((unsigned)(((int64_t)O * I + 255) / 256)), dim3(256), 0, stream, g, dcoefs, styles, dw2, N, O, I);
        SBG_HIP_LAUNCH_CHECK();
    }
    return 0;
}


namespace {
struct SplitArgs { const float* x; unsigned short* y; int64_t total; int64_t C, inner; int nseg; int order[8]; };

__global__ __launch_bounds__(256) void split_bf16_cat_kernel(SplitArgs a)
{
    const int64_t stride = (int64_t)gridDim.x * blockDim.x;
    for (int64_t idx = (int64_t)blockIdx.x * blockDim.x + threadIdx.x; idx < a.total; idx += stride) {
        const int64_t i = idx % a.inner, oc = idx / a.inner;
        const int64_t c = oc % a.C, o = oc / a.C;
        const float v = a.x[idx];
        unsigned short part[3];
        float r = v;
#pragma unroll
        for (int k = 0; k < 3; k++) { part[k] = f32_to_bf16_bits(r); r -= bf16_bits_to_f32(part[k]); }
        unsigned short* dst = a.y + (o * a.nseg * a.C + c) * a.inner + i;
        for (int s = 0; s < a.nseg; s++) dst[(int64_t)s * a.C * a.inner] = part[a.order[s]];
    }
}

struct SplitNdArgs { const float* x; unsigned short* y; int64_t total; int64_t shape[4], xs[4]; int cat; int nseg; int order[8]; };

__global__ __launch_bounds__(256) void split_bf16_cat_nd_kernel(SplitNdArgs a)
{
    const int64_t stride = (int64_t)gridDim.x * blockDim.x;
    for (int64_t idx = (int64_t)blockIdx.x * blockDim.x + threadIdx.x; idx < a.total; idx += stride) {
        int64_t d[4], r = idx;
#pragma unroll
        for (int k = 3; k >= 0; k--) { d[k] = r % a.shape[k]; r /= a.shape[k]; }
        float v = a.x[d[0] * a.xs[0] + d[1] * a.xs[1] + d[2] * a.xs[2] + d[3] * a.xs[3]];
        unsigned short part[3];
#pragma unroll
        for (int k = 0; k < 3; k++) { part[k] = f32_to_bf16_bits(v); v -= bf16_bits_to_f32(part[k]); }
        int64_t off = 0, seg = 1;
#pragma unroll
        for (int k = 0; k < 4; k++) off = off * (k == a.cat ? a.shape[k] * a.nseg : a.shape[k]) + d[k];
#pragma unroll
        for (int k = 3; k >= 0; k--) { if (k == a.cat) { seg *= a.shape[k]; break; } seg *= a.shape[k]; }
        for (int s = 0; s < a.nseg; s++) a.y[off + (int64_t)s * seg] = part[a.order[s]];
    }
}
}

extern "C" int sbg_split_bf16_cat_nd(const float* x, const int64_t* shape, const int64_t* xstrides, int cat_dim, void* y, int nseg, const int* order,
                                     sbg_stream_t stream_)
{
    SBG_CHECK(x && y && order && shape && xstrides, "split_bf16_cat_nd: null pointer");
    SBG_CHECK(cat_dim >= 0 && cat_dim < 4 && nseg >= 1 && nseg <= 8, "split_bf16_cat_nd: bad sizes");
    SplitNdArgs a;
    a.x = x; a.y = (unsigned short*)y; a.cat = cat_dim; a.nseg = nseg; a.total = 1;
    for (int k = 0; k < 4; k++) {
        SBG_CHECK(shape[k] >= 0 && xstrides[k] >= 0, "split_bf16_cat_nd: negative extent or stride");
        a.shape[k] = shape[k]; a.xs[k] = xstrides[k]; a.total *= shape[k];
    }
    for (int s = 0; s < 8; s++) { a.order[s] = s < nseg ? order[s] : 0; SBG_CHECK(a.order[s] >= 0 && a.order[s] <= 2, "split_bf16_cat_nd: part index out of range"); }
    if (a.total == 0) return 0;
    hipStream_t stream = (hipStream_t)stream_;
    SbgProfScope prof(stream, SBG_K_WEIGHT_PREP, 0.0, (double)a.total * (4.0 + 2.0 * nseg), {(int)shape[0], (int)shape[1], (int)shape[2], 5, nseg, (int)shape[3], 0});
    SBG_LAUNCH(split_bf16_cat_nd_kernel, dim3(sbg_stream_grid(a.total, 256)), dim3(256), 0, stream, a);
    SBG_HIP_LAUNCH_CHECK();
    return 0;
}

extern "C" int sbg_split_bf16_cat(const float* x, void* y, int64_t outer, int64_t C, int64_t inner, int nseg, const int* order, sbg_stream_t stream_)
{
    SBG_CHECK(x && y && order, "split_bf16_cat: null pointer");
    SBG_CHECK(outer >= 0 && C >= 1 && inner >= 1 && nseg >= 1 && nseg <= 8, "split_bf16_cat: bad sizes");
    SplitArgs a;
    a.x = x; a.y = (unsigned short*)y; a.total = outer * C * inner; a.C = C; a.inner = inner; a.nseg = nseg;
    for (int s = 0; s < 8; s++) { a.order[s] = s < nseg ? order[s] : 0; SBG_CHECK(a.order[s] >= 0 && a.order[s] <= 2, "split_bf16_cat: part index out of range"); }
    if (a.total == 0) return 0;
    hipStream_t stream = (hipStream_t)stream_;
    SbgProfScope prof(stream, SBG_K_WEIGHT_PREP, 0.0, (double)a.total * (4.0 + 2.0 * nseg), {(int)(outer > INT32_MAX ? INT32_MAX : outer), (int)C, (int)inner, 4, nseg, 0, 0});
    SBG_LAUNCH(split_bf16_cat_kernel, dim3(sbg_stream_grid(a.total, 256)), dim3(256), 0, stream, a);
    SBG_HIP_LAUNCH_CHECK();
    return 0;
}
```

style-big-gan_amd/torch_utils/ops/conv2d_gradfix.py:

```python
import contextlib

import weakref

import numpy as np

import torch

from ... import _lib

enabled = False
weight_gradients_disabled = False


@contextlib.contextmanager
def no_weight_gradients():
    global weight_gradients_disabled
    old = weight_gradients_disabled
    weight_gradients_disabled = True
    try:
        yield
    finally:
        weight_gradients_disabled = old


def _pair(v):
    v = tuple(v) if isinstance(v, (tuple, list)) else (v, v)
    assert len(v) == 2 and all(isinstance(i, int) for i in v)
    return v



def _cl(t):
    return t.contiguous(memory_format=torch.channels_last)


def _pad_channels(t, mult=8):
    c = t.shape[1]
    cp = (c + mult - 1) // mult * mult
    if cp == c:
        return _cl(t)
    out = torch.empty([t.shape[0], cp, t.shape[2], t.shape[3]], dtype=t.dtype, device=t.device, memory_format=torch.channels_last).zero_()
    out[:, :c] = t
    return out


def _split_bf16(t, parts):
    out, rest = [], t
    for _ in range(parts):
        h = rest.to(torch.bfloat16)
        out.append(h)
        rest = rest - h.to(torch.float32)
    return out


def _operand_passes(a, b):
    if a.dtype in (torch.bfloat16, torch.float16):
        return [(a, b)]
    if a.dtype == torch.float32:
        a0, a1, a2 = _split_bf16(a, 3)
        b0, b1, b2 = _split_bf16(b, 3)
        return [(a2, b0), (a0, b2), (a1, b1), (a1, b0), (a0, b1), (a0, b0)]
    raise RuntimeError(f"conv2d: unsupported dtype {a.dtype}")


class Epilogue:
    __slots__ = ("oscale", "noise", "bias", "act", "alpha", "gain", "clamp", "_keep")

    def __init__(self, oscale=None, noise=None, bias=None, act="linear", alpha=0.0, gain=1.0, clamp=-1.0):
        assert act in ("linear", "relu", "lrelu")
        self.oscale, self.noise, self.bias = oscale, noise, bias
        self.act, self.alpha, self.gain, self.clamp = {"linear": 1, "relu": 2, "lrelu": 3}[act], float(alpha), float(gain), float(clamp)
        self._keep = []

    def fill(self, p, n, cout, oh, ow):
        def f32(t, shape):
            t = t.detach().to(torch.float32).reshape(shape).contiguous()
            self._keep.append(t)
            return t
        if self.oscale is not None:
            p.oscale = f32(self.oscale, [n, cout]).data_ptr()
        if self.bias is not None:
            p.bias = f32(self.bias, [cout]).data_ptr()
        if self.noise is not None:
            per_sample = self.noise.numel() != oh * ow
            nz = f32(self.noise, [n if per_sample else 1, oh * ow])
            p.noise, p.noise_stride_n = nz.data_ptr(), (oh * ow if per_sample else 0)
        p.act, p.alpha, p.gain, p.clamp = self.act, self.alpha, self.gain, self.clamp


_KSPLIT_MAX_TILES = 128
_KSPLIT_TARGET = 256

CONCAT_NUMEL = 1 << 28


_ORDER6 = ((2, 0, 1, 1, 0, 0), (0, 2, 1, 0, 1, 0))


def _split_cat(t, dim, order, dense=False):
    import ctypes
    arr = (ctypes.c_int * len(order))(*order)
    if dense and t.ndim <= 4 and not t.is_contiguous():
        lead = 4 - t.ndim
        shape = [1] * lead + list(t.shape)
        out = torch.empty([len(order) * n if d == dim else n for d, n in enumerate(t.shape)], dtype=torch.bfloat16, device=t.device)
        _lib.check(_lib.load().sbg_split_bf16_cat_nd(_lib.ptr(t), (ctypes.c_int64 * 4)(*shape), (ctypes.c_int64 * 4)(*([0] * lead + list(t.stride()))),
                                                     lead + dim, _lib.ptr(out), len(order), arr, _lib.stream_ptr(t.device)), "sbg_split_bf16_cat_nd")
        return out
    perm = sorted(range(t.ndim), key=lambda d: (-t.stride(d), d))
    tt = t.permute(perm)
    if not tt.is_contiguous():
        tt = tt.contiguous()
    k = perm.index(dim)
    outer = int(np.prod(tt.shape[:k], dtype=np.int64)) if k > 0 else 1
    C, inner = tt.shape[k], (int(np.prod(tt.shape[k + 1:], dtype=np.int64)) if k + 1 < tt.ndim else 1)
    out = torch.empty(list(tt.shape[:k]) + [len(order) * C] + list(tt.shape[k + 1:]), dtype=torch.bfloat16, device=t.device)
    _lib.check(_lib.load().sbg_split_bf16_cat(_lib.ptr(tt), _lib.ptr(out), outer, C, inner, len(order), arr, _lib.stream_ptr(t.device)), "sbg_split_bf16_cat")
    inv = [perm.index(d) for d in range(t.ndim)]
    return out.permute(inv)


def _mfma_operands(a, b, a_cat_dim, b_cat_dim, b_dense=False):
    if (a.dtype == torch.float32 and b.dtype == torch.float32 and a.device.type == "cuda" and a.numel() <= CONCAT_NUMEL and a.numel() > 0 and b.numel() > 0):
        return [(_split_cat(a, a_cat_dim, _ORDER6[0]), _split_cat(b, b_cat_dim, _ORDER6[1], dense=b_dense))]
    return _fold_passes(_operand_passes(a, b), a_cat_dim, b_cat_dim)


def _fold_passes(passes, x_cat_dim, w_cat_dim):
    if len(passes) == 1 or passes[0][0].numel() > CONCAT_NUMEL:
        return passes
    a = torch.cat([a_ for a_, _ in passes], dim=x_cat_dim)
    b = torch.cat([b_ for _, b_ in passes], dim=w_cat_dim)
    if x_cat_dim == 1:
        a = a.contiguous(memory_format=torch.channels_last)
    return [(a, b)]



_pack_cache = {}
_ptr_epoch = {}


def _on_optimizer_step(optimizer, args, kwargs):
    for group in optimizer.param_groups:
        for q in group["params"]:
            if isinstance(q, torch.Tensor) and q.device.type == "cuda":
                k = q.data_ptr()
                _ptr_epoch[k] = _ptr_epoch.get(k, 0) + 1


from torch.optim.optimizer import register_optimizer_step_post_hook as _register_step_hook
_register_step_hook(_on_optimizer_step)


def invalidate_packed_weights():
    _pack_cache.clear()


def is_mixed(x, w):
    return w.dtype == torch.float32 and x.dtype in (torch.bfloat16, torch.float16)


def _packed_weight(w, rows_dim, dtype, bp, gain):
    assert w.dtype == torch.float32 and w.ndim == 4 and rows_dim in (0, 1)
    a_dim, b_dim = rows_dim, 1 - rows_dim
    A, B, kh, kw = w.shape[a_dim], w.shape[b_dim], w.shape[2], w.shape[3]
    base = w._base if w._base is not None else w
    cacheable = isinstance(base, torch.nn.Parameter)
    key = None
    if cacheable:
        key = (base.data_ptr(), w.storage_offset(), tuple(w.shape), tuple(w.stride()), rows_dim, dtype, bp, float(gain))
        hit = _pack_cache.get(key)
        stamp = (base._version, _ptr_epoch.get(base.data_ptr(), 0))
        if hit is not None and hit[0]() is base and hit[1] == stamp:
            return hit[2], hit[3]
    out = torch.empty([kh * kw, A, bp], dtype=dtype, device=w.device)
    w2 = torch.empty([A, B], dtype=torch.float32, device=w.device) if rows_dim == 0 else None
    wd = w.detach()
    _lib.check(_lib.load().sbg_pack_weight(wd.data_ptr(), out.data_ptr(), _lib.dtype_code(dtype), A, B, kh, kw, wd.stride(a_dim), wd.stride(b_dim),
                                           wd.stride(2), wd.stride(3), bp, float(gain), _lib.ptr(w2), _lib.stream_ptr(w.device)), "sbg_pack_weight")
    if cacheable:
        if len(_pack_cache) > 256:
            for k in [k for k, v in _pack_cache.items() if v[0]() is None]:
                del _pack_cache[k]
            if len(_pack_cache) > 2048:
                _pack_cache.clear()
        _pack_cache[key] = (weakref.ref(base), (base._version, _ptr_epoch.get(base.data_ptr(), 0)), out, w2)
    return out, w2


def _unpack_wgrad(out, ca, cb, wshape, wstride, rows_dim, gain, w=None, dw2=None):
    dev = out.device if out is not None else w.device
    dw = torch.empty_strided(wshape, wstride, dtype=torch.float32, device=dev)
    a_dim, b_dim = rows_dim, 1 - rows_dim
    assert wshape[a_dim] == ca and wshape[b_dim] == cb
    _lib.check(_lib.load().sbg_unpack_wgrad(_lib.ptr(out), out.stride(0) if out is not None else 0, out.stride(1) if out is not None else 0,
                                            dw.data_ptr(), _lib.ptr(w), _lib.ptr(dw2), ca, cb, wshape[2], wshape[3],
                                            wstride[a_dim], wstride[b_dim], wstride[2], wstride[3], float(gain), _lib.stream_ptr(dev)), "sbg_unpack_wgrad")
    return dw


def _igemm(x, wp, y, taps, stride, oh, ow, y_off=(0, 0), y_step=(1, 1), oscale=None, accumulate=False, epi=None):
    lib = _lib.load()
    p = _lib.ConvParams()
    n, cin, ih, iw = x.shape
    cout = wp.shape[1]
    assert wp.shape[2] == cin and x.stride(1) == 1 and y.stride(1) == 1 and wp.is_contiguous() and x.dtype == wp.dtype
    es = y.element_size()
    p.x, p.w = x.data_ptr(), wp.data_ptr()
    p.y = y.data_ptr() + (y_off[0] * y.stride(2) + y_off[1] * y.stride(3)) * es
    p.oscale = oscale.data_ptr() if oscale is not None else None
    p.xdtype, p.ydtype = _lib.dtype_code(x.dtype), _lib.dtype_code(y.dtype)
    p.N, p.IH, p.IW, p.Cin, p.Cout, p.OH, p.OW = n, ih, iw, cin, cout, oh, ow
    p.xs_n, p.xs_h, p.xs_w = x.stride(0), x.stride(2), x.stride(3)
    p.ys_n, p.ys_h, p.ys_w = y.stride(0), y.stride(2) * y_step[0], y.stride(3) * y_step[1]
    p.ws_slab, p.ws_co = wp.stride(0), wp.stride(1)
    p.stride, p.ntaps = stride, len(taps)
    assert 1 <= len(taps) <= _lib.SBG_MAX_TAPS
    for i, (dy, dx, slab) in enumerate(taps):
        p.tap_dy[i], p.tap_dx[i], p.tap_slab[i] = dy, dx, slab
    p.accumulate = int(accumulate)
    p.act, p.alpha, p.gain, p.clamp = 1, 0.0, 1.0, -1.0
    if epi is not None:
        assert not accumulate and y_step == (1, 1)
        epi.fill(p, n, cout, oh, ow)
    ws = None
    tiles = -(-(n * oh * ow) // 128) * -(-cout // 128)
    ksteps = len(taps) * -(-cin // 64)
    plain_f32 = epi is None and y.dtype == torch.float32
    if ((epi is None or not accumulate) and (y.dtype == torch.float32 or not accumulate) and y_step == (1, 1) and y_off == (0, 0) and cout > 64
            and (cout % 8 == 0 or plain_f32) and tiles < _KSPLIT_MAX_TILES and ksteps >= 16 and y.is_contiguous(memory_format=torch.channels_last)):
        p.ksplit = max(1, min(ksteps // 4, -(-_KSPLIT_TARGET // tiles)))
        if p.ksplit > 1:
            ws = torch.empty([lib.sbg_conv2d_igemm_workspace(p) // 4], dtype=torch.float32, device=x.device)
            p.workspace = ws.data_ptr()
    _lib.check(lib.sbg_conv2d_igemm(p, _lib.stream_ptr(x.device)), "sbg_conv2d_igemm")


def _igemm_phases(x, wp, y, phases, s):
    lib = _lib.load()
    p = _lib.ConvParams()
    n, cin, ih, iw = x.shape
    cout = wp.shape[1]
    p.x, p.w, p.y = x.data_ptr(), wp.data_ptr(), y.data_ptr()
    p.xdtype, p.ydtype = _lib.dtype_code(x.dtype), _lib.dtype_code(y.dtype)
    p.N, p.IH, p.IW, p.Cin, p.Cout = n, ih, iw, cin, cout
    p.OH, p.OW = max(ph[2] for ph in phases), max(ph[3] for ph in phases)
    p.xs_n, p.xs_h, p.xs_w = x.stride(0), x.stride(2), x.stride(3)
    p.ys_n, p.ys_h, p.ys_w = y.stride(0), y.stride(2) * s, y.stride(3) * s
    p.ws_slab, p.ws_co = wp.stride(0), wp.stride(1)
    p.stride = 1
    p.act, p.alpha, p.gain, p.clamp = 1, 0.0, 1.0, -1.0
    t = 0
    for i, (a, b, goh, gow, taps) in enumerate(phases):
        p.ph_ntaps[i], p.ph_oh[i], p.ph_ow[i] = len(taps), goh, gow
        p.ph_yoff[i] = a * y.stride(2) + b * y.stride(3)
        for dy, dx, slab in taps:
            p.tap_dy[t], p.tap_dx[t], p.tap_slab[t] = dy, dx, slab
            t += 1
    p.ntaps, p.nphase = t, len(phases)
    _lib.check(lib.sbg_conv2d_igemm(p, _lib.stream_ptr(x.device)), "sbg_conv2d_igemm")


def _launch_groups(taps):
    m = _lib.SBG_MAX_TAPS
    return [taps[i:i + m] for i in range(0, len(taps), m)]


def epilogue_fusable(x):
    return x.dtype in (torch.bfloat16, torch.float16)


def _conv_forward(x, w, stride, padding, epi=None, wgain=1.0):
    n, cin, ih, iw = x.shape
    cout, cin_w, kh, kw = w.shape
    mixed = is_mixed(x, w)
    assert cin == cin_w and (x.dtype == w.dtype or mixed) and (mixed or wgain == 1.0)
    (sh, sw), (ph, pw) = stride, padding
    assert sh == sw, "conv2d: only square strides are implemented"
    oh = (ih + 2 * ph - kh) // sh + 1
    ow = (iw + 2 * pw - kw) // sw + 1
    assert oh >= 1 and ow >= 1
    xp = _pad_channels(x)
    taps = [(i - ph, j - pw, i * kw + j) for i in range(kh) for j in range(kw)]
    if mixed:
        passes = [(xp, _packed_weight(w, 0, x.dtype, xp.shape[1], wgain)[0])]
    else:
        wpk = w.permute(2, 3, 0, 1).reshape(kh * kw, cout, cin)
        if xp.shape[1] != cin:
            wpk = torch.nn.functional.pad(wpk, (0, xp.shape[1] - cin))
        passes = _mfma_operands(xp, wpk, 1, 2, b_dense=True)
    multi = len(passes) > 1 or len(taps) > _lib.SBG_MAX_TAPS
    y = torch.empty([n, cout, oh, ow], dtype=torch.float32 if multi else x.dtype, device=x.device, memory_format=torch.channels_last)
    assert epi is None or (not multi)
    first = True
    for xa, wa in passes:
        wa = wa.contiguous()
        for grp in _launch_groups(taps):
            _igemm(xa, wa, y, grp, sh, oh, ow, accumulate=not first, epi=epi)
            first = False
    return y.to(x.dtype) if y.dtype != x.dtype else y


def _conv_transpose_forward(x, w, stride, padding, output_padding, wgain=1.0):
    n, cin, ih, iw = x.shape
    cin_w, cout, kh, kw = w.shape
    mixed = is_mixed(x, w)
    assert cin == cin_w and (x.dtype == w.dtype or mixed) and (mixed or wgain == 1.0)
    (sh, sw), (ph, pw), (oph, opw) = stride, padding, output_padding
    assert sh == sw, "conv_transpose2d: only square strides are implemented"
    s = sh
    oh = (ih - 1) * s - 2 * ph + kh + oph
    ow = (iw - 1) * s - 2 * pw + kw + opw
    assert oh >= 1 and ow >= 1
    xp = _pad_channels(x)
    if mixed:
        passes = [(xp, _packed_weight(w, 1, x.dtype, xp.shape[1], wgain)[0])]
    else:
        wpk = w.permute(2, 3, 1, 0).reshape(kh * kw, cout, cin)
        if xp.shape[1] != cin:
            wpk = torch.nn.functional.pad(wpk, (0, xp.shape[1] - cin))
        passes = _mfma_operands(xp, wpk, 1, 2, b_dense=True)
    phases = []
    need_zero = False
    for a in range(s):
        for b in range(s):
            goh, gow = (oh - a + s - 1) // s, (ow - b + s - 1) // s
            if goh <= 0 or gow <= 0:
                continue
            taps = [((a + ph - i) // s, (b + pw - j) // s, i * kw + j)
                    for i in range(kh) if (a + ph - i) % s == 0
                    for j in range(kw) if (b + pw - j) % s == 0]
            if not taps:
                need_zero = True
                continue
            phases.append((a, b, goh, gow, taps))
    multi = len(passes) > 1 or any(len(t) > _lib.SBG_MAX_TAPS for *_, t in phases)
    y = torch.empty([n, cout, oh, ow], dtype=torch.float32 if multi else x.dtype, device=x.device, memory_format=torch.channels_last)
    if need_zero:
        y.zero_()
    first = True
    if (not multi and 2 <= len(phases) <= 4 and sum(len(t) for *_, t in phases) <= _lib.SBG_MAX_TAPS):
        xa, wa = passes[0]
        _igemm_phases(xa, wa.contiguous(), y, phases, s)
        return y
    for xa, wa in passes:
        wa = wa.contiguous()
        for a, b, goh, gow, taps in phases:
            for gi, grp in enumerate(_launch_groups(taps)):
                _igemm(xa, wa, y, grp, 1, goh, gow, y_off=(a, b), y_step=(s, s), accumulate=(not first) or gi > 0)
        first = False
    return y.to(x.dtype) if y.dtype != x.dtype else y


def _wgrad(a, b, stride, taps):
    lib = _lib.load()
    assert a.dtype == b.dtype and a.shape[0] == b.shape[0]
    ca, cb = a.shape[1], b.shape[1]
    pw = a.shape[3]
    if (len(taps) == 9 and stride in (1, 2) and pw in (8, 16)
            and all(taps[t] == (taps[0][0] + t // 3, taps[0][1] + t % 3) for t in range(9))):
        a = torch.nn.functional.pad(a, (0, 32 - pw))
    ap, bp = _pad_channels(a), _pad_channels(b)
    cap, cbp = ap.shape[1], bp.shape[1]
    out = torch.empty([len(taps), cap, cbp], dtype=torch.float32, device=a.device)
    first = True
    for aa, bb in _mfma_operands(ap, bp, 0, 0):
        aa, bb = _cl(aa), _cl(bb)
        for g0 in range(0, len(taps), _lib.SBG_MAX_TAPS):
            grp = taps[g0:g0 + _lib.SBG_MAX_TAPS]
            p = _lib.WgradParams()
            p.a, p.b, p.out = aa.data_ptr(), bb.data_ptr(), out[g0:].data_ptr()
            p.dtype = _lib.dtype_code(aa.dtype)
            p.N, p.PH, p.PW, p.Ca = aa.shape[0], aa.shape[2], aa.shape[3], cap
            p.BH, p.BW, p.Cb = bb.shape[2], bb.shape[3], cbp
            p.as_n, p.as_h, p.as_w = aa.stride(0), aa.stride(2), aa.stride(3)
            p.bs_n, p.bs_h, p.bs_w = bb.stride(0), bb.stride(2), bb.stride(3)
            p.stride, p.ntaps = stride, len(grp)
            for i, (dy, dx) in enumerate(grp):
                p.tap_dy[i], p.tap_dx[i] = dy, dx
            p.accumulate = int(not first)
            nbytes = lib.sbg_conv2d_wgrad_workspace(p)
            if nbytes < 0:
                _lib.check(1, "sbg_conv2d_wgrad_workspace")
            ws = torch.empty([max(nbytes, 4) // 4], dtype=torch.float32, device=a.device) if nbytes > 0 else None
            p.workspace = ws.data_ptr() if ws is not None else None
            _lib.check(lib.sbg_conv2d_wgrad(p, _lib.stream_ptr(a.device)), "sbg_conv2d_wgrad")
        first = False
    return out[:, :ca, :cb]



def _output_padding_for(transpose, stride, padding, in_hw, out_hw, k_hw):
    if transpose:
        return (0, 0)
    return tuple(in_hw[i] - (out_hw[i] - 1) * stride[i] - (1 - 2 * padding[i]) - (k_hw[i] - 1) for i in range(2))


class _Conv(torch.autograd.Function):

    @staticmethod
    def forward(ctx, x, w, cfg):
        transpose, stride, padding, output_padding = cfg[:4]
        wgain = cfg[4] if len(cfg) > 4 else 1.0
        _lib.require_cuda(x, "conv2d")
        if x.dtype != w.dtype and not is_mixed(x, w):
            raise RuntimeError(f"conv2d: input ({x.dtype}) and weight ({w.dtype}) must have the same dtype (or an fp32 weight with 16-bit input)")
        if not transpose:
            y = _conv_forward(x, w, stride, padding, wgain=wgain)
        else:
            y = _conv_transpose_forward(x, w, stride, padding, output_padding, wgain=wgain)
        ctx.save_for_backward(x, w)
        ctx.cfg = cfg
        return y

    @staticmethod
    def backward(ctx, dy):
        x, w = ctx.saved_tensors
        transpose, stride, padding, output_padding = ctx.cfg[:4]
        wgain = ctx.cfg[4] if len(ctx.cfg) > 4 else 1.0
        dx = dw = None
        if ctx.needs_input_grad[0]:
            op = _output_padding_for(transpose, stride, padding, x.shape[2:], dy.shape[2:], w.shape[2:])
            if dy.dtype != x.dtype:
                dy = dy.to(x.dtype)
            dx = _Conv.apply(dy, w, (not transpose, stride, padding, op, wgain))
            assert dx.shape == x.shape
        if ctx.needs_input_grad[1] and not weight_gradients_disabled:
            dw = _ConvWgrad.apply(dy, x, ctx.cfg, tuple(w.shape), wmeta_of(x, w))
        return dx, dw, None


def wmeta_of(x, w):
    return tuple(w.stride()) if is_mixed(x, w) else None


class _ConvWgrad(torch.autograd.Function):

    @staticmethod
    def forward(ctx, dy, x, cfg, wshape, wmeta=None):
        transpose, stride, padding, _ = cfg[:4]
        wgain = cfg[4] if len(cfg) > 4 else 1.0
        kh, kw = wshape[2], wshape[3]
        taps = [(i - padding[0], j - padding[1]) for i in range(kh) for j in range(kw)]
        assert stride[0] == stride[1]
        if dy.dtype != x.dtype:
            dy = dy.to(x.dtype)
        if not transpose:
            out = _wgrad(dy, x, stride[0], taps)
        else:
            out = _wgrad(x, dy, stride[0], taps)
        if wmeta is not None:
            dw = _unpack_wgrad(out, wshape[0], wshape[1], wshape, wmeta, 0, wgain)
        else:
            dw = out.reshape(kh, kw, wshape[0], wshape[1]).permute(2, 3, 0, 1).to(x.dtype)
        ctx.save_for_backward(dy, x)
        ctx.cfg, ctx.wshape = cfg, wshape
        return dw

    @staticmethod
    def backward(ctx, ddw):
        dy, x = ctx.saved_tensors
        transpose, stride, padding, output_padding = ctx.cfg[:4]
        d_dy = d_x = None
        if ctx.needs_input_grad[0]:
            d_dy = _Conv.apply(x, ddw, ctx.cfg)
            assert d_dy.shape == dy.shape
        if ctx.needs_input_grad[1]:
            op = _output_padding_for(transpose, stride, padding, x.shape[2:], dy.shape[2:], ctx.wshape[2:])
            d_x = _Conv.apply(dy, ddw, (not transpose, stride, padding, op) + tuple(ctx.cfg[4:]))
            assert d_x.shape == x.shape
        return d_dy, d_x, None, None, None


def _grouped(fn, input, weight, groups, transpose):
    cin_g = input.shape[1] // groups
    outs = []
    wg = weight.shape[0] // groups
    for g in range(groups):
        outs.append(fn(input[:, g * cin_g:(g + 1) * cin_g], weight[g * wg:(g + 1) * wg]))
    return torch.cat(outs, dim=1)


def _add_bias(y, bias):
    if bias is None:
        return y
    from . import bias_act
    return bias_act.bias_act(y, bias.to(y.dtype))


def conv2d(input, weight, bias=None, stride=1, padding=0, dilation=1, groups=1, wgain=1.0):
    _lib.require_cuda(input, "conv2d")
    assert _pair(dilation) == (1, 1), "conv2d: dilation is not implemented"
    cfg = (False, _pair(stride), _pair(padding), (0, 0), float(wgain))
    assert groups == 1 or not is_mixed(input, weight)
    assert all(p >= 0 for p in cfg[2]) and all(s >= 1 for s in cfg[1])
    if groups == 1:
        y = _Conv.apply(input, weight, cfg)
    else:
        y = _grouped(lambda a, b: _Conv.apply(a, b, cfg), input, weight, groups, False)
    return _add_bias(y, bias)


def conv_transpose2d(input, weight, bias=None, stride=1, padding=0, output_padding=0, groups=1, dilation=1, wgain=1.0):
    _lib.require_cuda(input, "conv_transpose2d")
    assert _pair(dilation) == (1, 1), "conv_transpose2d: dilation is not implemented"
    cfg = (True, _pair(stride), _pair(padding), _pair(output_padding), float(wgain))
    assert groups == 1 or not is_mixed(input, weight)
    assert all(0 <= cfg[3][i] < max(cfg[1][i], 1) or cfg[3][i] == 0 for i in range(2))
    if groups == 1:
        y = _Conv.apply(input, weight, cfg)
    else:
        y = _grouped(lambda a, b: _Conv.apply(a, b, cfg), input, weight, groups, True)
    return _add_bias(y, bias)
```

style-big-gan_amd/torch_utils/ops/modconv.py:

```python
import torch

from ... import _lib
from . import bias_act as _ba
from . import conv2d_gradfix as _cg
from . import modulate as _mod
from . import upfirdn2d as _up

enabled = True
import os as _os
chain_heads = _os.environ.get("SBG_CHAIN_HEADS", "1") != "0"

_ACT = {"linear": 1, "relu": 2, "lrelu": 3}


def usable(x, weight, act, up):
    return (enabled and up == 1 and act in _ACT and x.device.type == "cuda" and x.dtype in (torch.bfloat16, torch.float16)
            and weight.shape[2] == weight.shape[3] and bool(_lib.load().sbg_modconv_bwd_supported(weight.shape[0])))


class _ModConvBiasAct(torch.autograd.Function):

    @staticmethod
    def forward(ctx, x, w, styles, dcoefs, noise, b, cfg, x_tail=None):
        ctx.x_tail = x_tail
        padding, act, alpha, gain, clamp = cfg
        xs = _mod._scale_nc_launch(x, styles, None)
        epi = _cg.Epilogue(oscale=dcoefs, noise=noise, bias=b, act=act, alpha=alpha, gain=gain, clamp=clamp)
        y = _cg._conv_forward(xs, w, (1, 1), (padding, padding), epi=epi)
        ctx.save_for_backward(x, xs, w, styles, dcoefs, noise, b, y)
        ctx.cfg = cfg
        return y

    @staticmethod
    def backward(ctx, dy):
        x, xs, w, styles, dcoefs, noise, b, y = ctx.saved_tensors
        padding, act, alpha, gain, clamp = ctx.cfg
        if torch.is_grad_enabled():
            raise RuntimeError("modconv: the fused layer is first-order only; set torch_utils.ops.modconv.enabled = False "
                               "before building a graph that is differentiated twice (path-length regularisation)")
        n, cout, h, wd = y.shape
        want_dn = noise is not None and ctx.needs_input_grad[4]
        d2, sums, dn, dc32 = _up.backward_head(dy, y, dcoefs, noise, b, act, alpha, gain, clamp, want_dn)
        dx = dw = dstyles = ddcoefs = dnoise = db = None
        if ctx.needs_input_grad[3]:
            ddcoefs = (sums[1] / dc32).to(dcoefs.dtype).reshape(dcoefs.shape)
        if b is not None and ctx.needs_input_grad[5]:
            db = sums[0].sum(0).to(b.dtype)
        if want_dn:
            dnoise = dn if noise.numel() != h * wd else dn.sum(0, keepdim=True)
            dnoise = dnoise.reshape(noise.shape).to(noise.dtype)
        ccfg = (False, (1, 1), (padding, padding), (0, 0))
        if ctx.needs_input_grad[0] or ctx.needs_input_grad[2]:
            dxs = _cg._Conv.apply(d2, w, (True, (1, 1), (padding, padding), (0, 0)))
            tail = ctx.x_tail
            both = None
            if (tail is not None and ctx.needs_input_grad[0] and ctx.needs_input_grad[2] and dxs.dtype == x.dtype
                    and _lib.load().sbg_modconv_bwd_supported(x.shape[1])):
                hd2, hsums, hdn, hdc32, dst = _up.backward_head(dxs, x, tail.dcoefs, tail.noise, tail.b, tail.act, tail.alpha, tail.act_gain, tail.clamp,
                                                                tail.noise is not None, prescale=styles)
                tail.result = dict(ptr=hd2.data_ptr(), sums=hsums, dn=hdn, dc32=hdc32)
                dx, dstyles = hd2, dst.to(styles.dtype).reshape(styles.shape)
            else:
                if ctx.needs_input_grad[0] and ctx.needs_input_grad[2]:
                    both = _mod._dot_hw_scale_launch(dxs, x, styles)
                if both is not None:
                    dx, dstyles = both[0], both[1].to(styles.dtype).reshape(styles.shape)
                else:
                    if ctx.needs_input_grad[0]:
                        dx = _mod._scale_nc_launch(dxs, styles, None)
                    if ctx.needs_input_grad[2]:
                        dstyles = _mod._dot_hw_launch(dxs, x).to(styles.dtype).reshape(styles.shape)
        if ctx.needs_input_grad[1] and not _cg.weight_gradients_disabled:
            dw = _cg._ConvWgrad.apply(d2, xs, ccfg, tuple(w.shape), _cg.wmeta_of(xs, w))
        return dx, dw, dstyles, ddcoefs, dnoise, db, None, None


class _DemodCoefs(torch.autograd.Function):

    @staticmethod
    def forward(ctx, weight, styles, act_dtype):
        assert weight.dtype == torch.float32 and weight.ndim == 4
        o, i = weight.shape[0], weight.shape[1]
        n = styles.shape[0]
        _, w2 = _cg._packed_weight(weight, 0, act_dtype, (i + 7) // 8 * 8, 1.0)
        s32 = styles.detach().to(torch.float32).contiguous()
        d = torch.empty([n, o], dtype=torch.float32, device=weight.device)
        _lib.check(_lib.load().sbg_demod_coefs(s32.data_ptr(), w2.data_ptr(), d.data_ptr(), n, o, i, 1e-8, _lib.stream_ptr(weight.device)), "sbg_demod_coefs")
        ctx.save_for_backward(weight, s32, w2, d)
        ctx.s_dtype = styles.dtype
        return d

    @staticmethod
    def backward(ctx, g):
        weight, s32, w2, d = ctx.saved_tensors
        if torch.is_grad_enabled():
            raise RuntimeError("demod_coefs: first-order only; set torch_utils.ops.modconv.enabled = False for double backward")
        n, o = d.shape
        i = s32.shape[1]
        g = g.to(torch.float32).contiguous()
        ds = torch.empty_like(s32) if ctx.needs_input_grad[1] else None
        dw2 = torch.empty_like(w2) if ctx.needs_input_grad[0] else None
        _lib.check(_lib.load().sbg_demod_coefs_bwd(g.data_ptr(), d.data_ptr(), s32.data_ptr(), w2.data_ptr(), _lib.ptr(ds), _lib.ptr(dw2), n, o, i,
                                                   _lib.stream_ptr(g.device)), "sbg_demod_coefs_bwd")
        dw = None
        if dw2 is not None:
            dw = _cg._unpack_wgrad(None, o, i, tuple(weight.shape), tuple(weight.stride()), 0, 1.0, w=weight.detach(), dw2=dw2)
        return dw, (ds.to(ctx.s_dtype) if ds is not None else None), None


def demod_coefs(weight, styles, act_dtype):
    return _DemodCoefs.apply(weight, styles, act_dtype)


def modconv_bias_act(x, weight, styles, dcoefs, noise, bias, padding, act="lrelu", alpha=None, gain=None, clamp=None, x_sole_consumer=False):
    spec = _ba.activation_funcs[act]
    cfg = (int(padding), act, float(alpha if alpha is not None else spec.def_alpha), float(gain if gain is not None else spec.def_gain),
           float(clamp if clamp is not None else -1))
    x_tail = getattr(x, "_sbg_tail", None) if (x_sole_consumer and chain_heads) else None
    return _ModConvBiasAct.apply(x, weight, styles, dcoefs, noise, bias, cfg, x_tail)
```

style-big-gan_amd/train_parts/generators.py:

```python
import numpy as np
import torch

from .. import utils
from ..torch_utils import misc
from ..torch_utils.ops import bias_act, conv2d_gradfix, conv2d_resample, conv_bias_act, grouped_gemm, modconv, modulate, torgb, upfirdn2d

generators = utils.ClassRegistry()

LOW_PRECISION = torch.bfloat16
import os as _os
style_bank_enabled = _os.environ.get('SBG_STYLE_BANK', '1') != '0'
premodulate = _os.environ.get('SBG_PREMODULATE', '1') != '0'


def set_low_precision(dtype):
    global LOW_PRECISION
    assert dtype in (torch.bfloat16, torch.float16)
    LOW_PRECISION = dtype


def low_precision():
    return LOW_PRECISION


# ... 337 lines not shown


def _attention_module(channels):
    from ..biggan.layers import Attention
    return Attention(channels)


class SynthesisBlock(torch.nn.Module):
    def __init__(self,
        in_channels         = None,
        out_channels        = None,
        w_dim               = None,
        resolution          = None,
        img_channels        = None,
        is_last             = None,
        architecture        = 'skip',
        resample_filter     = (1,3,3,1),
        conv_clamp          = None,
        use_fp16            = False,
        fp16_channels_last  = False,
        attention           = False,
        layer_kwargs        = Synthlayerkwargs(),
    ):
        assert None not in (in_channels, out_channels, w_dim, resolution, img_channels, is_last)
        assert architecture in ['orig', 'skip', 'resnet']
        super().__init__()
        self.in_channels = in_channels
        self.w_dim = w_dim
        self.resolution = resolution
        self.img_channels = img_channels
        self.is_last = is_last
        self.architecture = architecture
        self.use_fp16 = use_fp16
        self.channels_last = bool(use_fp16)
        self.register_buffer('resample_filter', upfirdn2d.setup_filter(list(resample_filter)))
        self.num_conv = 0
        self.num_torgb = 0
        self.attention = _attention_module(out_channels) if attention else None

        if in_channels == 0:
            self.const = torch.nn.Parameter(torch.randn([out_channels, resolution, resolution]))
        lk = dict(layer_kwargs.items()) if layer_kwargs is not None else {}
        lk.update(in_channels=in_channels, out_channels=out_channels, w_dim=w_dim, resolution=resolution, up=2,
                  resample_filter=resample_filter, conv_clamp=conv_clamp, channels_last=self.channels_last)
        if in_channels != 0:
            self.conv0 = SynthesisLayer(**lk)
            self.num_conv += 1
        lk.update(in_channels=out_channels, up=1, resample_filter=[1, 3, 3, 1])
        self.conv1 = SynthesisLayer(**lk)
        self.num_conv += 1
        if is_last or architecture == 'skip':
            self.torgb = ToRGBLayer(out_channels, img_channels, w_dim=w_dim, conv_clamp=conv_clamp, channels_last=self.channels_last)
            self.num_torgb += 1
        if in_channels != 0 and architecture == 'resnet':
            self.skip = Conv2dLayer(in_channels, out_channels, kernel_size=1, bias=False, up=2,
                                    resample_filter=resample_filter, channels_last=self.channels_last)

    def forward(self, x, img, ws, force_fp32=False, fused_modconv=None, styles=None, **layer_kwargs):
        s0, s1, srgb = styles if styles is not None else (None, None, None)
        misc.assert_shape(ws, [None, self.num_conv + self.num_torgb, self.w_dim])
        w_iter = iter(ws.unbind(dim=1))
        reduced = self.use_fp16 and not force_fp32
        dtype = LOW_PRECISION if reduced else torch.float32
        fmt = torch.channels_last if reduced else torch.contiguous_format
        if fused_modconv is None:
            fused_modconv = (not self.training) and (dtype == torch.float32 or int(x.shape[0]) == 1)

        lk = dict(fused_modconv=fused_modconv, **layer_kwargs)
        first = self.in_channels == 0
        if first:
            x = self.const.to(dtype=dtype, memory_format=fmt).unsqueeze(0).repeat([ws.shape[0], 1, 1, 1])
        else:
            misc.assert_shape(x, [None, self.in_channels, self.resolution // 2, self.resolution // 2])
            x = x.to(dtype=dtype, memory_format=fmt)

        residual = (not first) and self.architecture == 'resnet'
        shortcut = self.skip(x, gain=np.sqrt(0.5)) if residual else None
        sole = not first
        g1 = np.sqrt(0.5) if residual else 1
        records_graph = torch.is_grad_enabled() and (x.requires_grad or ws.requires_grad or self.conv1.weight.requires_grad or (sole and self.conv0.weight.requires_grad))
        if sole and premodulate and self.conv1.premodulated_input_ok(dtype, x.device, records_graph):
            w0, w1 = next(w_iter), next(w_iter)
            styles1 = self.conv1.affine(w1) if s1 is None else s1
            x = self.conv0(x, w0, post_scale=styles1, styles=s0, **lk)
            x = self.conv1(x, w1, gain=g1, styles=styles1, x_premodulated=True, **lk)
        else:
            if not first:
                x = self.conv0(x, next(w_iter), styles=s0, **lk)
            x = self.conv1(x, next(w_iter), gain=g1, x_sole_consumer=sole, styles=s1, **lk)
        if residual:
            x = shortcut + x
        if self.attention is not None:
            x = self.attention(x.to(torch.float32)).to(dtype)

        if img is not None:
            misc.assert_shape(img, [None, self.img_channels, self.resolution // 2, self.resolution // 2])
            img = upfirdn2d.upsample2d(img, self.resample_filter)
        if self.is_last or self.architecture == 'skip':
            rgb = self.torgb(x, next(w_iter), fused_modconv=fused_modconv, styles=srgb).to(dtype=torch.float32, memory_format=torch.contiguous_format)
            img = rgb if img is None else img.add_(rgb)
        assert x.dtype == dtype and (img is None or img.dtype == torch.float32)
        return x, img


Synthblockkwargs = generators.make_dataclass_from_init(SynthesisBlock.__init__, 'Synthblockkwargs', None)


class SynthesisNetwork(torch.nn.Module):
    def __init__(self,
        w_dim           = None,
        img_resolution  = None,
        img_channels    = None,
        channel_base    = 32768,
        channel_max     = 512,
        num_fp16_res    = 0,
        attentions      = (),
        block_kwargs    = Synthblockkwargs(),
    ):
        assert None not in (w_dim, img_resolution, img_channels)
        assert img_resolution >= 4 and img_resolution & (img_resolution - 1) == 0
        super().__init__()
        self.w_dim = w_dim
        self.img_resolution = img_resolution
        self.img_resolution_log2 = int(np.log2(img_resolution))
        self.img_channels = img_channels
        self.block_resolutions = [2 ** i for i in range(2, self.img_resolution_log2 + 1)]
        channels = {res: min(channel_base // res, channel_max) for res in self.block_resolutions}
        fp16_resolution = max(2 ** (self.img_resolution_log2 + 1 - num_fp16_res), 8)
        bk = dict(block_kwargs.items()) if block_kwargs is not None else {}
        self.num_ws = 0
        for res in self.block_resolutions:
            bk.update(in_channels=(channels[res // 2] if res > 4 else 0), out_channels=channels[res], w_dim=w_dim, resolution=res,
                      img_channels=img_channels, is_last=(res == img_resolution), use_fp16=(res >= fp16_resolution),
                      attention=(res in attentions))
            block = SynthesisBlock(**bk)
            self.num_ws += block.num_conv
            if res == img_resolution:
                self.num_ws += block.num_torgb
            setattr(self, f'b{res}', block)

    def forward(self, ws, **block_kwargs):
        misc.assert_shape(ws, [None, self.num_ws, self.w_dim])
        ws = ws.to(torch.float32)
        per_block, w_idx = [], 0
        for res in self.block_resolutions:
            block = getattr(self, f'b{res}')
            per_block.append(ws.narrow(1, w_idx, block.num_conv + block.num_torgb))
            w_idx += block.num_conv
        x = img = None
        plan = self.pass_plan(ws.shape[0]) if ws.shape[0] > 1 else None
        tail, chunk = plan if plan is not None else (0, ws.shape[0])
        head = len(self.block_resolutions) - tail
        bank = self._style_bank(ws)
        for res, cur_ws in zip(self.block_resolutions[:head], per_block[:head]):
            x, img = getattr(self, f'b{res}')(x, img, cur_ws, styles=(bank[res] if bank else None), **block_kwargs)
        if tail > 0:
            imgs = []
            for i in range(0, ws.shape[0], chunk):
                xc, ic = x.narrow(0, i, chunk), (img.narrow(0, i, chunk) if img is not None else None)
                for res, cur_ws in zip(self.block_resolutions[head:], per_block[head:]):
                    st = tuple(None if s is None else s.narrow(0, i, chunk) for s in bank[res]) if bank else None
                    xc, ic = getattr(self, f'b{res}')(xc, ic, cur_ws.narrow(0, i, chunk), styles=st, **block_kwargs)
                imgs.append(ic)
            img = misc.cat0(imgs)
        return img

    def _style_bank(self, ws):
        if not (style_bank_enabled and ws.is_cuda and ws.dtype == torch.float32 and (modconv.enabled or not torch.is_grad_enabled())):
            return None
        layers, where, w_idx = [], [], 0
        for res in self.block_resolutions:
            block = getattr(self, f'b{res}')
            has0 = block.in_channels != 0
            entries = [(block.conv0.affine, w_idx, 1.0) if has0 else None, (block.conv1.affine, w_idx + (1 if has0 else 0), 1.0),
                       (block.torgb.affine, w_idx + block.num_conv, float(block.torgb.weight_gain)) if block.num_torgb else None]
            for pos, e in enumerate(entries):
                if e is None:
                    continue
                fc, slot, post = e
                if fc.activation != 'linear' or fc.bias is None or fc.weight.dtype != torch.float32 or not fc.weight.is_contiguous():
                    return None
                layers.append((slot, fc.weight, fc.bias, float(fc.weight_gain) * post, float(fc.bias_gain) * post))
                where.append((res, pos))
            w_idx += block.num_conv
        styles = grouped_gemm.style_bank(ws, layers)
        bank = {res: [None, None, None] for res in self.block_resolutions}
        for (res, pos), s in zip(where, styles):
            bank[res][pos] = s
        return {res: tuple(v) for res, v in bank.items()}

    pass_bytes_limit = 1 << 31

    def pass_plan(self, n):
        cache = self.__dict__.setdefault('_pass_plans', {})
        key = (n, self.pass_bytes_limit)
        if key not in cache:
            blocks = [getattr(self, f'b{res}') for res in self.block_resolutions]
            peaks = [int(b.conv1.weight.shape[0]) * (b.resolution + 1) ** 2 * (2 if b.use_fp16 else 12) for b in blocks]
            k = 0
            while k < len(peaks) - 1 and n * peaks[-1 - k] >= self.pass_bytes_limit:
                k += 1
            plan = (0, n)
            if k > 0:
                plan = None
                if not any(b.attention is not None for b in blocks[len(blocks) - k:]):
                    for chunk in range(n // 2, 0, -1):
                        if n % chunk == 0 and chunk * max(peaks[len(peaks) - k:]) < self.pass_bytes_limit:
                            plan = (k, chunk)
                            break
            cache[key] = plan
        return cache[key]


Mappingkwargs = generators.make_dataclass_from_init(MappingNetwork.__init__, 'Mappingkwargs', None)
Synthesiskwargs = generators.make_dataclass_from_init(SynthesisNetwork.__init__, 'Synthesiskwargs', None)


@generators.add_to_registry("sg2_classic")
class Generator(torch.nn.Module):
    def __init__(self,
        z_dim               = 128,
        c_dim               = None,
        w_dim               = 128,
        img_resolution      = None,
        img_channels        = None,
        attentions          = (),
        mapping_kwargs      = Mappingkwargs(),
        synthesis_kwargs    = Synthesiskwargs(),
    ):
        super().__init__()
        self.z_dim, self.c_dim, self.w_dim = z_dim, c_dim, w_dim
        self.img_resolution, self.img_channels = img_resolution, img_channels
        sk = dict(synthesis_kwargs.items()) if synthesis_kwargs is not None else {}
        sk.update(w_dim=w_dim, img_resolution=img_resolution, img_channels=img_channels, attentions=attentions)
        self.synthesis = SynthesisNetwork(**sk)
        self.num_ws = self.synthesis.num_ws
        mk = dict(mapping_kwargs.items()) if mapping_kwargs is not None else {}
        mk.update(z_dim=z_dim, c_dim=c_dim, w_dim=w_dim, num_ws=self.num_ws)
        self.mapping = MappingNetwork(**mk)
        self.rounds_mergeable = len(tuple(attentions)) == 0

    def peak_activation_bytes(self):
        blocks = [getattr(self.synthesis, f'b{res}') for res in self.synthesis.block_resolutions]
        return max(int(b.conv1.weight.shape[0]) * (b.resolution + 1) ** 2 * (2 if b.use_fp16 else 12) for b in blocks)

    def forward(self, z, c, truncation_psi=1, truncation_cutoff=None, **synthesis_kwargs):
        ws = self.mapping(z, c, truncation_psi=truncation_psi, truncation_cutoff=truncation_cutoff)
        return self.synthesis(ws, **synthesis_kwargs)



def _dcgan_up(cin, cout, k, stride, pad, last=False):
    conv = torch.nn.ConvTranspose2d(cin, cout, k, stride, pad, bias=False)
    return [conv, torch.nn.Tanh()] if last else [conv, torch.nn.BatchNorm2d(cout), torch.nn.ReLU(True)]


class Generator_dcgan(torch.nn.Module):

    def __init__(self, z_dim, M):
        super().__init__()
        self.z_dim = z_dim
        layers = _dcgan_up(z_dim, 1024, M, 1, 0)
        for cin, cout in [(1024, 512), (512, 256), (256, 128)]:
            layers += _dcgan_up(cin, cout, 4, 2, 1)
        layers += _dcgan_up(128, 3, 4, 2, 1, last=True)
        self.main = torch.nn.Sequential(*layers)

    def forward(self, z, c, noise_mode=None):
        return self.main(z.view(-1, self.z_dim, 1, 1))


@generators.add_to_registry("cnn32_dcgan")
class Generator32_dcgan(Generator_dcgan):
    def __init__(self, z_dim, c_dim, img_resolution, *args, **kwargs):
        super().__init__(z_dim, M=2)
        self.c_dim = c_dim
        self.img_resolution = img_resolution


@generators.add_to_registry("cnn48_dcgan")
class Generator48_dcgan(Generator_dcgan):
    def __init__(self, z_dim):
        super().__init__(z_dim, M=4)



def G_arch(ch=64, attention='64', ksize='333333', dilation='111111'):
    att = [int(item) for item in attention.split('_')]
    table = {512: ([16, 16, 8, 8, 4, 2, 1], [16, 8, 8, 4, 2, 1, 1]), 256: ([16, 16, 8, 8, 4, 2], [16, 8, 8, 4, 2, 1]),
             128: ([16, 16, 8, 4, 2], [16, 8, 4, 2, 1]), 64: ([16, 16, 8, 4], [16, 8, 4, 2]), 32: ([4, 4, 4], [4, 4, 4])}
    arch = {}
    for res, (cin, cout) in table.items():
        resolutions = [2 ** i for i in range(3, int(np.log2(res)) + 1)]
        arch[res] = {'in_channels': [ch * m for m in cin], 'out_channels': [ch * m for m in cout], 'upsample': [True] * len(cin),
                     'resolution': resolutions, 'attention': {r: (r in att) for r in resolutions}}
    return arch


@generators.add_to_registry("big_gan")
class BigGAnGenerator(torch.nn.Module):
    def __init__(self, G_ch=64, z_dim=128, c_dim=10, bottom_width=4, img_resolution=128,
                 G_kernel_size=3, G_attn='64', n_classes=10,
                 num_G_SVs=1, num_G_SV_itrs=1,
                 G_shared=True, shared_dim=0, hier=False,
                 cross_replica=False, mybn=False,
                 G_activation='relu',
                 BN_eps=1e-5, SN_eps=1e-12, G_mixed_precision=False, G_fp16=False,
                 G_init='ortho',
                 G_param='SN', norm_style='bn',
                 **kwargs):
        super().__init__()
        import functools
        from ..biggan import layers
        self.c_dim, self.ch, self.z_dim = c_dim, G_ch, z_dim
        self.bottom_width, self.img_resolution = bottom_width, img_resolution
        self.kernel_size, self.attention, self.n_classes = G_kernel_size, G_attn, n_classes
        self.G_shared = G_shared
        self.shared_dim = shared_dim if shared_dim > 0 else z_dim
# ... 63 lines not shown
```

style-big-gan_amd/train_parts/trainers.py:

```python
import copy
import json
import os
import time

import numpy as np
import torch

from .. import utils
from ..parallel import GradReducer
from ..torch_utils import misc, training_stats
from ..utils import EasyDict
from .discriminators import discriminators
from .generators import generators
from .losses_base import losses_arch
from .optimizers import optimizers

trainers = utils.ClassRegistry()

merge_rounds = os.environ.get('SBG_MERGE_ROUNDS', '1') != '0'


def setup_snapshot_image_grid(training_set, random_seed=0):
    rnd = np.random.RandomState(random_seed)
    gw = int(np.clip(7680 // training_set.image_shape[2], 7, 32))
    gh = int(np.clip(4320 // training_set.image_shape[1], 4, 32))
    if not training_set.has_labels:
        all_indices = list(range(len(training_set)))
        rnd.shuffle(all_indices)
        grid_indices = [all_indices[i % len(all_indices)] for i in range(gw * gh)]
    else:
        label_groups = dict()
        for idx in range(len(training_set)):
            label = tuple(training_set.get_details(idx).raw_label.flat[::-1])
            label_groups.setdefault(label, []).append(idx)
        label_order = sorted(label_groups.keys())
        for label in label_order:
            rnd.shuffle(label_groups[label])
        grid_indices = []
        for y in range(gh):
            label = label_order[y % len(label_order)]
            indices = label_groups[label]
            grid_indices += [indices[x % len(indices)] for x in range(gw)]
            label_groups[label] = [indices[(i + gw) % len(indices)] for i in range(len(indices))]
    images, labels = zip(*[training_set[i] for i in grid_indices])
    return (gw, gh), np.stack(images), np.stack(labels)


def write_grid_png(canvas, fname):
    import PIL.Image
    canvas = np.ascontiguousarray(canvas)
    assert canvas.ndim == 3 and canvas.shape[2] in [1, 3]
    if canvas.shape[2] == 1:
        PIL.Image.fromarray(canvas[:, :, 0], 'L').save(fname)
    else:
        PIL.Image.fromarray(canvas, 'RGB').save(fname)


def save_image_grid(img, fname, drange, grid_size):
    from ..torch_utils.ops import image_export
    img = img if isinstance(img, torch.Tensor) else torch.from_numpy(np.ascontiguousarray(img))
    gw, gh = grid_size
    assert img.shape[0] == gw * gh
    write_grid_png(image_export.tile(img.to(torch.float32), (gw, gh), 'grid', drange).cpu().numpy(), fname)


def lazy_reg_opt_kwargs(opt_kwargs, interval):
    mb_ratio = interval / (interval + 1)
    out = dict(opt_kwargs)
    out['lr'] = opt_kwargs['lr'] * mb_ratio
    out['betas'] = [beta ** mb_ratio for beta in opt_kwargs['betas']]
    return out


def format_time(seconds):
    s = int(np.rint(seconds))
    if s < 60:
        return f"{s}s"
    if s < 60 * 60:
        return f"{s // 60}m {s % 60:02}s"
    if s < 24 * 60 * 60:
        return f"{s // (60 * 60)}h {(s // 60) % 60:02}m {s % 60:02}s"
    return f"{s // (24 * 60 * 60)}d {(s // (60 * 60)) % 24:02}h {(s // 60) % 60:02}m"


def cpu_mem_gb():
    try:
        with open("/proc/self/statm") as fh:
            return int(fh.read().split()[1]) * os.sysconf("SC_PAGE_SIZE") / 2 ** 30
    except (OSError, ValueError, IndexError):
        return 0.0


def _option_lines(obj, tabs=0):
    out = []
    for key, value in obj.items():
        if isinstance(value, dict):
            out.append(" " * tabs + f"{key}:")
            out += _option_lines(value, tabs + 4)
        else:
            out.append(" " * tabs + f"{key} : {value}")
    return out


@trainers.add_to_registry("step_engine")
class StepEngine:

    def __init__(self, device, generator='sg2_classic', discriminator='sg2_classic', gen_kwargs=None, disc_kwargs=None,
                 loss_arch='sg2', loss='softplus', loss_arch_kwargs=None, gen_regs=(), dis_regs=(('r1', dict(r1_gamma=10.)),),
                 optim_gen=('adam', dict(lr=0.0025, betas=[0, 0.99], eps=1e-8)), optim_disc=('adam', dict(lr=0.0025, betas=[0, 0.99], eps=1e-8)),
                 g_reg_interval=16, d_reg_interval=4, n_dis=1, batch=64, batch_gpu=32, ema_kimg=10., ema_rampup=None, use_ema=True,
                 world_size=1, rank=0, process_group=None, seed=0,
                 augment_kwargs=None, augment_type='sg2_ada', augment_p=0.0, ada_target=None, ada_interval=4, ada_kimg=500):
        self.device = torch.device(device)
        self.rank, self.world_size = rank, world_size
        self.batch, self.batch_gpu = batch, batch_gpu
        assert batch % batch_gpu == 0
        self.ema_kimg, self.ema_rampup, self.use_ema = ema_kimg, ema_rampup, use_ema
        self.cur_nimg = 0
        self.batch_idx = 0
        self._round_plan = {}
        self._round_proven = set()
        self._count_nonfinite = False
        self.comm_stats = None
        self.time_phases = False
        self.report_grad_health = False
        self._phase_events = {}

        torch.manual_seed(seed * max(world_size, 1) + rank)
        self.G = generators[generator](**(gen_kwargs or {})).train().requires_grad_(False).to(self.device)
        self.D = discriminators[discriminator](**(disc_kwargs or {})).train().requires_grad_(False).to(self.device)
        self.G_ema = copy.deepcopy(self.G).eval() if use_ema else None
        self.z_dim = self.G.z_dim
        self.c_dim = self.G.c_dim or 0

        self.sg2 = (loss_arch == 'sg2')
        dp = dict(world_size=world_size, process_group=process_group)
        if self.sg2:
            self.dp_modules = dict(G_mapping=GradReducer(self.G.mapping, **dp), G_synthesis=GradReducer(self.G.synthesis, **dp),
                                   D=GradReducer(self.D, **dp))
            la = dict(G_mapping=self.dp_modules['G_mapping'], G_synthesis=self.dp_modules['G_synthesis'])
        else:
            self.dp_modules = dict(G=GradReducer(self.G, **dp), D=GradReducer(self.D, **dp))
            la = dict(G=self.dp_modules['G'])
        la.update(loss_arch_kwargs or {})
        if self.G_ema is not None:
            misc.copy_params_and_buffers(self.G, self.G_ema, require_all=True)

        self.augment_pipe, self.ada_stats = None, None
        self.ada_target, self.ada_interval, self.ada_kimg = ada_target, ada_interval, ada_kimg
        if augment_kwargs is not None and (augment_p > 0 or ada_target is not None):
            from .augmentations import augmentations
            self.augment_pipe = augmentations[augment_type](**augment_kwargs).train().requires_grad_(False).to(self.device)
            self.augment_pipe.p.copy_(torch.as_tensor(float(augment_p)))
            if ada_target is not None:
                self.ada_stats = training_stats.Collector(regex='Loss/signs/real')
                self._ada_sync = os.environ.get('SBG_ADA_SYNC', '0') == '1' or self.device.type != 'cuda'
                if not self._ada_sync:
                    self._ada_acc = torch.zeros([2], dtype=torch.float64, device=self.device)
                    def tap(v, acc=self._ada_acc):
                        if v.device == acc.device:
                            acc.add_(torch.stack([torch.full([], float(v.numel()), dtype=torch.float64, device=v.device), v.sum(dtype=torch.float64)]))
                    self._ada_tap = training_stats.add_tap('Loss/signs/real', tap)
                    self._ada_adopt_at = None
            la['augment_pipe'] = self.augment_pipe
        from ..torch_utils.ops import modconv
        modconv.enabled = True
        self.loss = losses_arch[loss_arch](device=self.device, gen_regs=list(gen_regs), dis_regs=list(dis_regs),
                                           D=self.dp_modules['D'], loss=loss, **la)

        self.phases = []
        g_reducers = [self.dp_modules[k] for k in self.dp_modules if k.startswith('G')]
        for name, module, reducers, (opt_name, opt_kwargs), interval, both_interval in [
                ('G', self.G, g_reducers, optim_gen, g_reg_interval, int(n_dis)),
                ('D', self.D, [self.dp_modules['D']], optim_disc, d_reg_interval, 1)]:
            if interval is None or interval <= 0:
                opt = optimizers[opt_name](params=module.parameters(), **dict(opt_kwargs))
                slots = [(name + 'both', both_interval)]
            else:
                opt = optimizers[opt_name](params=module.parameters(), **lazy_reg_opt_kwargs(dict(opt_kwargs), interval))
                slots = [(name + 'main', 1), (name + 'reg', int(interval))]
            for phase_name, phase_interval in slots:
                self.phases.append(EasyDict(name=phase_name, module=module, reducers=reducers, opt=opt, interval=phase_interval,
                                            idle=len(self.loss.program(phase_name)) == 0))

    def close(self):
        tap = getattr(self, '_ada_tap', None)
        if tap is not None:
            training_stats.remove_tap('Loss/signs/real', tap)
            self._ada_tap = None

    def __del__(self):
        try:
            self.close()
        except Exception:
            pass

    def train_iteration(self, real_img, real_c, all_gen_z=None, all_gen_c=None):
        assert real_img.shape[0] == self.batch
        if getattr(self, '_ada_adopt_at', None) is not None and self.batch_idx >= self._ada_adopt_at:
            self.augment_pipe.adopt_strength()
            self._ada_adopt_at = None
        n_phase = len(self.phases)
        if all_gen_z is None:
            all_gen_z = torch.randn([n_phase * self.batch, self.z_dim], device=self.device)
        if all_gen_c is None:
            all_gen_c = real_c.repeat(n_phase, 1) if real_c is not None and real_c.numel() else torch.zeros([n_phase * self.batch, self.c_dim], device=self.device)
        reals = real_img.split(self.batch_gpu)
        real_cs = (real_c if real_c is not None else torch.zeros([self.batch, self.c_dim], device=self.device)).split(self.batch_gpu)
        zs = [z.split(self.batch_gpu) for z in all_gen_z.split(self.batch)]
        cs = [c.split(self.batch_gpu) for c in all_gen_c.split(self.batch)]
        rounds = self.batch // self.batch_gpu

        for phase, phase_z, phase_c in zip(self.phases, zs, cs):
            if phase.idle or self.batch_idx % phase.interval != 0:
                continue
            events = None
            if self.time_phases and self.device.type == 'cuda':
                events = self._phase_events.get(phase.name) or (torch.cuda.Event(enable_timing=True), torch.cuda.Event(enable_timing=True))
                self._phase_events[phase.name] = None
                events[0].record(torch.cuda.current_stream(self.device))
            with torch.autograd.profiler.record_function(phase.name):
                for r in phase.reducers:
                    r.zero_grad()
                phase.module.requires_grad_(True)
                merged = self._rounds_in_one_pass(phase.name, rounds)
                if merged:
                    mapping = getattr(self.G, 'mapping', None)
                    first_try = (phase.name, rounds) not in self._round_proven
                    w_avg0 = mapping.w_avg.clone() if first_try and mapping is not None and hasattr(mapping, 'w_avg') else None
                    if mapping is not None:
                        mapping.w_avg_rounds = rounds
                    try:
                        self.loss.accumulate_gradients(phase=phase.name, real_img=real_img, real_c=torch.cat(real_cs), gen_z=torch.cat(phase_z),
                                                       gen_c=torch.cat(phase_c), sync=True, gain=phase.interval * rounds, segments=rounds)
                        self._round_proven.add((phase.name, rounds))
                    except torch.OutOfMemoryError:
                        if not first_try:
                            raise
                        merged = False
                        self._round_plan[(phase.name, rounds)] = False
                        for r in phase.reducers:
                            r.finish(nan_to_num=False, reduce=False); r.zero_grad()
                        if w_avg0 is not None:
                            mapping.w_avg.copy_(w_avg0)
                        torch.cuda.empty_cache()
                    finally:
                        if mapping is not None:
                            mapping.w_avg_rounds = 1
                if not merged:
                    for round_idx, (img, c, z, gc) in enumerate(zip(reals, real_cs, phase_z, phase_c)):
                        sync = (round_idx == rounds - 1)
                        self.loss.accumulate_gradients(phase=phase.name, real_img=img, real_c=c, gen_z=z, gen_c=gc, sync=sync, gain=phase.interval)
                phase.module.requires_grad_(False)
            with torch.autograd.profiler.record_function(phase.name + '_opt'):
                st = self.comm_stats.setdefault(phase.name, dict(pairs=[], nonfinite=torch.zeros([], dtype=torch.int64, device=self.device), runs=0)) \
                    if self.comm_stats is not None else None
                for r in phase.reducers:
                    if st is not None and self._count_nonfinite:
                        r.nonfinite = st['nonfinite']
                    r.finish()
                    if st is not None:
                        st['pairs'].extend(r.timing or []); r.timing = []
                        r.nonfinite = None
                if st is not None:
                    st['runs'] += 1
                if self.report_grad_health:
                    self._report_grad_health(phase)
                phase.opt.step()
            if events is not None:
                events[1].record(torch.cuda.current_stream(self.device))
                self._phase_events[phase.name] = events

        if self.G_ema is not None:
            with torch.autograd.profiler.record_function('Gema'):
                self.update_ema()
        self.cur_nimg += self.batch * self.world_size
        self.batch_idx += 1

        if self.ada_stats is not None and self.batch_idx % self.ada_interval == 0:
            step = (self.batch * self.world_size * self.ada_interval) / (self.ada_kimg * 1000)
            if self._ada_sync:
                self.ada_stats.update()
                adjust = np.sign(self.ada_stats['Loss/signs/real'] - self.ada_target) * step
                self.augment_pipe.p.copy_((self.augment_pipe.p + adjust).clamp_(min=0))
            else:
                acc = self._ada_acc
                if self.world_size > 1:
                    torch.distributed.all_reduce(acc)
                mean = acc[1] / acc[0].clamp(min=1)
                adjust = torch.where(acc[0] > 0, torch.sign(mean - self.ada_target) * step, torch.zeros_like(mean))
                self.augment_pipe.p.copy_((self.augment_pipe.p + adjust.to(self.augment_pipe.p.dtype)).clamp_(min=0))
                acc.zero_()
                self.augment_pipe.announce_strength_update()
                self._ada_adopt_at = self.batch_idx + 1

    def set_grad_health(self, on=True):
        self.report_grad_health = bool(on)
        for r in self.dp_modules.values():
            r.health = bool(on)

    def _report_grad_health(self, phase):
        health = [r.last_health for r in phase.reducers if r.last_health is not None]
        if not health:
            return
        h = torch.stack(health)
        training_stats.report(f'Grad/{phase.name}/norm', h[:, 1].sum().sqrt())
        training_stats.report(f'Grad/{phase.name}/absmax', h[:, 2].max())
        training_stats.report(f'Grad/{phase.name}/nonfinite', h[:, 0].sum())

    def phase_times(self):
        out = {}
        for name, events in self._phase_events.items():
            if events is not None:
                events[1].synchronize()
                out[name] = events[0].elapsed_time(events[1])
        return out

    def collect_comm_stats(self, on=True, nonfinite=True):
        self.comm_stats = {} if on else None
        self._count_nonfinite = bool(nonfinite)
        for r in self.dp_modules.values():
            r.timing = [] if on else None
            r.nonfinite = None

    def _rounds_in_one_pass(self, phase_name, rounds):
        if rounds <= 1 or not merge_rounds or not getattr(self.G, 'rounds_mergeable', False):
            return False
        hit = self._round_plan.get((phase_name, rounds))
        if hit is None:
            syn = getattr(self.G, 'synthesis', None)
            fits = syn.pass_plan(rounds * self.batch_gpu) is not None if hasattr(syn, 'pass_plan') else True
            hit = fits and self.loss.rounds_mergeable(phase_name, self.batch_gpu, rounds)
            self._round_plan[(phase_name, rounds)] = hit
        return hit

    def state_dict(self):
        opts = {}
        for ph in self.phases:
            opts.setdefault(ph.name[0], ph.opt.state_dict())
        out = dict(G=self.G.state_dict(), D=self.D.state_dict(), optimizers=opts,
                   progress=dict(cur_nimg=int(self.cur_nimg), batch_idx=int(self.batch_idx)))
        if self.G_ema is not None:
            out['G_ema'] = self.G_ema.state_dict()
        if self.augment_pipe is not None:
            out['augment_pipe'] = self.augment_pipe.state_dict()
        return out

    def load_state_dict(self, state, strict=True, networks_only=False):
        self.G.load_state_dict(state['G'], strict=strict)
        self.D.load_state_dict(state['D'], strict=strict)
        if self.G_ema is not None:
            self.G_ema.load_state_dict(state.get('G_ema', state['G']), strict=strict)
        if self.augment_pipe is not None and 'augment_pipe' in state and not networks_only:
            self.augment_pipe.load_state_dict(state['augment_pipe'], strict=strict)
            self.augment_pipe._strength()
            self._ada_adopt_at = None
        if networks_only:
            return
        for ph in self.phases:
            if ph.name[0] in state.get('optimizers', {}):
                ph.opt.load_state_dict(state['optimizers'][ph.name[0]])
        self.cur_nimg = int(state['progress']['cur_nimg'])
        self.batch_idx = int(state['progress']['batch_idx'])

    @torch.no_grad()
    def update_ema(self):
        global_batch = self.batch * self.world_size
        ema_nimg = self.ema_kimg * 1000
        if self.ema_rampup is not None:
            ema_nimg = min(ema_nimg, self.cur_nimg * self.ema_rampup)
        beta = 0.5 ** (global_batch / max(ema_nimg, 1e-8))
        p_ema, p = list(self.G_ema.parameters()), list(self.G.parameters())
        torch._foreach_lerp_(p_ema, p, 1.0 - beta)
        b_ema, b = list(self.G_ema.buffers()), list(self.G.buffers())
# ... 504 lines not shown
```

Measured before the change: 624.1 img/s.

## Batch weight packing and demod coefficients into table launches; fuse wgrad unpack

Adds table-driven kernels that pack all conv weights in one launch at the start of each phase, and compute all generator demodulation coefficients in one launch per forward. Per-layer calls then look up precomputed slices. The wgrad split-K reduce kernel can now write straight into the parameter's layout with gain and the dw2 term applied, which removes the separate unpack kernel. The aim is fewer small kernel launches and less host overhead, at the cost of more bookkeeping and a risk of stale cached tables.

New measurement: 626.6 img/s (median of 6 runs). About the same (+0.4%).

```diff
diff --git a/include/sbg_hip.h b/include/sbg_hip.h
--- a/include/sbg_hip.h
+++ b/include/sbg_hip.h
@@ -87,6 +87,10 @@
     int ntaps;
     int tap_dy[SBG_MAX_TAPS], tap_dx[SBG_MAX_TAPS];
     int accumulate;
+    float dw_gain;
+    float* dw; const float* dw_w; const float* dw_dw2;
+    int64_t dw_sA, dw_sB, dw_sKH, dw_sKW;
+    int dw_A, dw_B, dw_KW;
 } sbg_wgrad_params;
 int64_t sbg_conv2d_wgrad_workspace(const sbg_wgrad_params* p);
 int     sbg_conv2d_wgrad(const sbg_wgrad_params* p, sbg_stream_t stream);
@@ -151,6 +155,23 @@
 int sbg_demod_coefs(const float* styles, const float* w2, float* dcoefs, int N, int O, int I, float eps, sbg_stream_t stream);
 int sbg_demod_coefs_bwd(const float* g, const float* dcoefs, const float* styles, const float* w2, float* dstyles, float* dw2,
                         int N, int O, int I, sbg_stream_t stream);
+
+#define SBG_TABLE_MAX 32
+enum { SBG_PACK_CAST = 0, SBG_PACK_SPLIT = 1 };
+typedef struct sbg_pack_desc {
+    const float* w; void* out; float* w2;
+    int64_t sA, sB, sKH, sKW;
+    int A, B, KH, KW, Bp, out_dtype, kind;
+    float gain;
+    int nseg; unsigned char order[8];
+} sbg_pack_desc;
+int sbg_pack_weight_table(const sbg_pack_desc* entries, int count, sbg_stream_t stream);
+
+typedef struct sbg_demod_desc {
+    const float* styles; const float* w2; float* dcoefs;
+    int N, O, I;
+} sbg_demod_desc;
+int sbg_demod_coefs_table(const sbg_demod_desc* entries, int count, float eps, sbg_stream_t stream);
 
 int sbg_torgb_supported(int C, int O);
 int sbg_torgb_bwd_blocks(int N, int C, int64_t HW);
diff --git a/style-big-gan_amd/_lib.py b/style-big-gan_amd/_lib.py
--- a/style-big-gan_amd/_lib.py
+++ b/style-big-gan_amd/_lib.py
@@ -69,6 +69,10 @@
         ("stride", ctypes.c_int), ("ntaps", ctypes.c_int),
         ("tap_dy", ctypes.c_int * SBG_MAX_TAPS), ("tap_dx", ctypes.c_int * SBG_MAX_TAPS),
         ("accumulate", ctypes.c_int),
+        ("dw_gain", ctypes.c_float),
+        ("dw", ctypes.c_void_p), ("dw_w", ctypes.c_void_p), ("dw_dw2", ctypes.c_void_p),
+        ("dw_sA", ctypes.c_int64), ("dw_sB", ctypes.c_int64), ("dw_sKH", ctypes.c_int64), ("dw_sKW", ctypes.c_int64),
+        ("dw_A", ctypes.c_int), ("dw_B", ctypes.c_int), ("dw_KW", ctypes.c_int),
     ]
 
 
@@ -91,6 +95,23 @@
                 ("c_rs", ctypes.c_int64), ("c_cs", ctypes.c_int64),
                 ("M", ctypes.c_int), ("N", ctypes.c_int), ("K0", ctypes.c_int), ("K1", ctypes.c_int), ("nterms", ctypes.c_int),
                 ("alpha0", ctypes.c_float), ("alpha1", ctypes.c_float), ("bias_scale", ctypes.c_float), ("rowsum_scale", ctypes.c_float)]
+
+
+SBG_TABLE_MAX = 32
+SBG_PACK_CAST, SBG_PACK_SPLIT = 0, 1
+
+
+class PackDesc(ctypes.Structure):
+    _fields_ = [("w", ctypes.c_void_p), ("out", ctypes.c_void_p), ("w2", ctypes.c_void_p),
+                ("sA", ctypes.c_int64), ("sB", ctypes.c_int64), ("sKH", ctypes.c_int64), ("sKW", ctypes.c_int64),
+                ("A", ctypes.c_int), ("B", ctypes.c_int), ("KH", ctypes.c_int), ("KW", ctypes.c_int), ("Bp", ctypes.c_int),
+                ("out_dtype", ctypes.c_int), ("kind", ctypes.c_int), ("gain", ctypes.c_float),
+                ("nseg", ctypes.c_int), ("order", ctypes.c_ubyte * 8)]
+
+
+class DemodDesc(ctypes.Structure):
+    _fields_ = [("styles", ctypes.c_void_p), ("w2", ctypes.c_void_p), ("dcoefs", ctypes.c_void_p),
+                ("N", ctypes.c_int), ("O", ctypes.c_int), ("I", ctypes.c_int)]
 
 
 class ProfRecord(ctypes.Structure):
@@ -160,6 +181,8 @@
      + [_c.c_int64] * 4 + [_c.c_float, _c.c_void_p]),
     ("sbg_demod_coefs", _c.c_int, [_c.c_void_p] * 3 + [_c.c_int] * 3 + [_c.c_float, _c.c_void_p]),
     ("sbg_demod_coefs_bwd", _c.c_int, [_c.c_void_p] * 6 + [_c.c_int] * 3 + [_c.c_void_p]),
+    ("sbg_pack_weight_table", _c.c_int, [_c.c_void_p, _c.c_int, _c.c_void_p]),
+    ("sbg_demod_coefs_table", _c.c_int, [_c.c_void_p, _c.c_int, _c.c_float, _c.c_void_p]),
     ("sbg_torgb_supported", _c.c_int, [_c.c_int, _c.c_int]),
     ("sbg_torgb_bwd_blocks", _c.c_int, [_c.c_int, _c.c_int, _c.c_int64]),
     ("sbg_torgb_fwd", _c.c_int, [_c.c_void_p] * 4 + [_c.c_int] * 4 + [_c.c_int64, _c.c_float, _c.c_void_p]),
diff --git a/style-big-gan_amd/csrc/conv_wgrad.hip b/style-big-gan_amd/csrc/conv_wgrad.hip
--- a/style-big-gan_amd/csrc/conv_wgrad.hip
+++ b/style-big-gan_amd/csrc/conv_wgrad.hip
@@ -372,8 +372,15 @@
     }
 }
 
-template <int LANES>
-__global__ __launch_bounds__(256) void wgrad_reduce_kernel(const float* ws, float* out, int64_t n, int nsplit, int accumulate)
+struct WgradDest {
+    float* dw; const float* w; const float* dw2;
+    int64_t sA, sB, sKH, sKW;
+    int A, B, KW, Ca, Cb;
+    float gain;
+};
+
+template <int LANES, bool DEST>
+__global__ __launch_bounds__(256) void wgrad_reduce_kernel(const float* ws, float* out, int64_t n, int nsplit, int accumulate, WgradDest dst)
 {
     const int sub = threadIdx.x % LANES;
     const int64_t step = (int64_t)gridDim.x * (256 / LANES);
@@ -390,7 +397,20 @@
         for (; k < nsplit; k += LANES) s += ws[(int64_t)k * n + i];
 #pragma unroll
         for (int m = LANES >> 1; m >= 1; m >>= 1) s += __shfl_xor(s, m, 64);
-        if (sub == 0) out[i] = accumulate ? out[i] + s : s;
+        if (sub != 0) continue;
+        if (!DEST) { out[i] = accumulate ? out[i] + s : s; continue; }
+        const unsigned ta = (unsigned)i / (unsigned)dst.Cb;
+        const int b = (int)((unsigned)i - ta * (unsigned)dst.Cb);
+        const int t = (int)(ta / (unsigned)dst.Ca), a = (int)(ta - (unsigned)t * (unsigned)dst.Ca);
+        if (a >= dst.A || b >= dst.B) continue;
+        const int kh = t / dst.KW, kw = t - kh * dst.KW;
+        const int64_t o = (int64_t)a * dst.sA + (int64_t)b * dst.sB + kh * dst.sKH + kw * dst.sKW;
+        float v = dst.gain * s;
+        if (dst.dw2) {
+            const float extra = 2.0f * dst.gain * dst.gain * dst.dw2[(int64_t)a * dst.B + b];
+            v = __builtin_fmaf(extra, dst.w[o], v);
+        }
+        dst.dw[o] = v;
     }
 }
 
@@ -541,7 +561,14 @@
 
 static int fill_args(const sbg_wgrad_params* q, WgradArgs& a)
 {
-    SBG_CHECK(q && q->a && q->b && q->out, "conv2d_wgrad: null pointer");
+    SBG_CHECK(q && q->a && q->b, "conv2d_wgrad: null pointer");
+    if (q->dw) {
+        SBG_CHECK(!q->accumulate, "conv2d_wgrad: a destination in the parameter's layout cannot accumulate");
+        SBG_CHECK(q->dw_A >= 1 && q->dw_A <= q->Ca && q->dw_B >= 1 && q->dw_B <= q->Cb && q->dw_KW >= 1 && (q->ntaps % q->dw_KW) == 0,
+                  "conv2d_wgrad: destination extents do not match the launch");
+        SBG_CHECK(!q->dw_dw2 || q->dw_w, "conv2d_wgrad: dw2 needs w");
+        SBG_CHECK((int64_t)q->ntaps * q->Ca * q->Cb <= INT32_MAX, "conv2d_wgrad: result too large for a destination");
+    }
     SBG_CHECK(q->dtype == SBG_BF16 || q->dtype == SBG_F16, "conv2d_wgrad: a/b must be bf16 or f16 (fp32 inputs are split by the host)");
     SBG_CHECK(q->N >= 0 && q->PH >= 1 && q->PW >= 1 && q->BH >= 1 && q->BW >= 1, "conv2d_wgrad: bad sizes");
     SBG_CHECK(q->Ca >= 8 && q->Cb >= 8 && (q->Ca % 8) == 0 && (q->Cb % 8) == 0, "conv2d_wgrad: channel counts must be multiples of 8 (pad on the host)");
@@ -596,6 +623,7 @@
     if (rc != SBG_OK) return rc;
     hipStream_t s = (hipStream_t)stream;
     const int64_t out_n = (int64_t)a.ntaps_total * a.Ca * a.Cb;
+    SBG_CHECK(a.out != nullptr || (a.P > 0 && a.nsplit > 1), "conv2d_wgrad: out required (the pixel sum is not split)");
     if (a.P == 0) {
         if (!a.accumulate) { if (hipMemsetAsync(a.out, 0, out_n * sizeof(float), s) != hipSuccess) return sbg_fail(SBG_ERR_LAUNCH, "conv2d_wgrad: memset failed"); }
         return SBG_OK;
@@ -652,13 +680,23 @@
         }
     }
     if (a.nsplit > 1) {
-        SbgProfScope prof(s, SBG_K_WGRAD_REDUCE, 0.0, 4.0 * out_n * (a.nsplit + 1), {(int)out_n, a.nsplit});
+        const bool dest = q->dw != nullptr;
+        WgradDest d = {};
+        if (dest) {
+            d.dw = q->dw; d.w = q->dw_w; d.dw2 = q->dw_dw2; d.sA = q->dw_sA; d.sB = q->dw_sB; d.sKH = q->dw_sKH; d.sKW = q->dw_sKW;
+            d.A = q->dw_A; d.B = q->dw_B; d.KW = q->dw_KW; d.Ca = a.Ca; d.Cb = a.Cb; d.gain = q->dw_gain;
+        }
+        SbgProfScope prof(s, SBG_K_WGRAD_REDUCE, 0.0, 4.0 * out_n * (a.nsplit + 1), {(int)out_n, a.nsplit, dest ? 1 : 0});
+#define SBG_REDUCE_LAUNCH(L, items) do { \
+        if (dest) SBG_LAUNCH((wgrad_reduce_kernel<L, true>), dim3(sbg_stream_grid((items), 256)), dim3(256), 0, s, a.ws, a.out, out_n, a.nsplit, a.accumulate, d); \
+        else      SBG_LAUNCH((wgrad_reduce_kernel<L, false>), dim3(sbg_stream_grid((items), 256)), dim3(256), 0, s, a.ws, a.out, out_n, a.nsplit, a.accumulate, d); } while (0)
         if (out_n >= (1 << 18) || a.nsplit < 16)
-            SBG_LAUNCH(wgrad_reduce_kernel<1>, dim3(sbg_stream_grid(out_n, 256)), dim3(256), 0, s, a.ws, a.out, out_n, a.nsplit, a.accumulate);
+            SBG_REDUCE_LAUNCH(1, out_n);
         else if (out_n >= (1 << 14))
-            SBG_LAUNCH(wgrad_reduce_kernel<4>, dim3(sbg_stream_grid(out_n * 4, 256)), dim3(256), 0, s, a.ws, a.out, out_n, a.nsplit, a.accumulate);
+            SBG_REDUCE_LAUNCH(4, out_n * 4);
         else
-            SBG_LAUNCH(wgrad_reduce_kernel<64>, dim3(sbg_stream_grid(out_n * 64, 256)), dim3(256), 0, s, a.ws, a.out, out_n, a.nsplit, a.accumulate);
+            SBG_REDUCE_LAUNCH(64, out_n * 64);
+#undef SBG_REDUCE_LAUNCH
         SBG_HIP_LAUNCH_CHECK();
     }
     return SBG_OK;
diff --git a/style-big-gan_amd/csrc/host_tests/table_split_main.cpp b/style-big-gan_amd/csrc/host_tests/table_split_main.cpp
--- /dev/null
+++ b/style-big-gan_amd/csrc/host_tests/table_split_main.cpp
@@ -0,0 +1,84 @@
+#include <cstdio>
+#include <cstdlib>
+#include <vector>
+#include "../table_split.h"
+
+static int failures = 0;
+#define EXPECT(cond) do { if (!(cond)) { std::printf("FAILED %s:%d: %s\n", __FILE__, __LINE__, #cond); failures++; } } while (0)
+
+struct Launch { int first, n, tiles; };
+static std::vector<Launch> walk(const std::vector<int>& tiles, int max_entries)
+{
+    std::vector<Launch> out;
+    const int count = (int)tiles.size();
+    std::vector<int> tile0((size_t)max_entries + 1, -1);
+    for (int first = 0; first < count;) {
+        const int n = sbg_table_next_launch(tiles.data(), count, first, max_entries, tile0.data());
+        EXPECT(n >= 1 && n <= max_entries && first + n <= count);
+        if (n < 1) break;
+        EXPECT(tile0[0] == 0);
+        for (int e = 0; e < n; e++) EXPECT(tile0[e + 1] - tile0[e] == tiles[(size_t)(first + e)]);
+        for (int wg = 0; wg < tile0[n]; wg++) {
+            const int e = sbg_table_find(tile0.data(), n, wg);
+            EXPECT(e >= 0 && e < n && tile0[e] <= wg && wg < tile0[e + 1]);
+        }
+        out.push_back({first, n, tile0[n]});
+        first += n;
+    }
+    return out;
+}
+
+int main()
+{
+    const int MAX = 32;
+    int tile0[MAX + 1];
+
+    EXPECT(sbg_table_next_launch(nullptr, 0, 0, MAX, tile0) == 0);
+    EXPECT(walk({}, MAX).empty());
+
+    {
+        std::vector<int> t(MAX);
+        for (int i = 0; i < MAX; i++) t[(size_t)i] = 1 + (i * 7) % 5;
+        const auto l = walk(t, MAX);
+        EXPECT(l.size() == 1 && l[0].first == 0 && l[0].n == MAX);
+        EXPECT(sbg_table_next_launch(t.data(), MAX, MAX, MAX, tile0) == 0);
+    }
+    {
+        std::vector<int> t(MAX + 1, 3);
+        const auto l = walk(t, MAX);
+        EXPECT(l.size() == 2 && l[0].n == MAX && l[0].tiles == 3 * MAX && l[1].first == MAX && l[1].n == 1 && l[1].tiles == 3);
+    }
+    {
+        const auto l = walk({0, 4, 0, 0, 2, 0}, MAX);
+        EXPECT(l.size() == 1 && l[0].n == 6 && l[0].tiles == 6);
+        const int t[] = {0, 4, 0, 0, 2, 0};
+        EXPECT(sbg_table_next_launch(t, 6, 0, MAX, tile0) == 6);
+        EXPECT(sbg_table_find(tile0, 6, 0) == 1 && sbg_table_find(tile0, 6, 3) == 1 && sbg_table_find(tile0, 6, 4) == 4 && sbg_table_find(tile0, 6, 5) == 4);
+        const auto z = walk({0, 0}, MAX);
+        EXPECT(z.size() == 1 && z[0].tiles == 0);
+    }
+    {
+        const auto l = walk({5, 1, 2, 9, 1, 1, 1}, 3);
+        EXPECT(l.size() == 3 && l[0].n == 3 && l[1].n == 3 && l[2].n == 1 && l[2].first == 6);
+    }
+    {
+        const int big = (int)(SBG_TABLE_MAX_TILES / 2 + 1);
+        const int t[] = {big, big, 1};
+        EXPECT(sbg_table_next_launch(t, 3, 0, MAX, tile0) == 1 && tile0[1] == big);
+        EXPECT(sbg_table_next_launch(t, 3, 1, MAX, tile0) == 2 && tile0[2] == big + 1);
+        const int over[] = {1, 2147483647};
+        EXPECT(sbg_table_next_launch(over, 2, 0, MAX, tile0) == -1);
+    }
+    {
+        const int t[] = {1, -1, 1};
+        EXPECT(sbg_table_next_launch(t, 3, 0, MAX, tile0) == -1);
+        EXPECT(sbg_table_next_launch(nullptr, 3, 0, MAX, tile0) == -1);
+        EXPECT(sbg_table_next_launch(t, -1, 0, MAX, tile0) == -1);
+        EXPECT(sbg_table_next_launch(t, 3, -1, MAX, tile0) == -1);
+        EXPECT(sbg_table_next_launch(t, 3, 4, MAX, tile0) == -1);
+        EXPECT(sbg_table_next_launch(t, 3, 0, 0, tile0) == -1);
+        EXPECT(sbg_table_next_launch(t, 3, 0, MAX, nullptr) == -1);
+    }
+    if (failures == 0) std::printf("table_split: all checks held\n");
+    return failures == 0 ? 0 : 1;
+}
diff --git a/style-big-gan_amd/csrc/table_split.h b/style-big-gan_amd/csrc/table_split.h
--- /dev/null
+++ b/style-big-gan_amd/csrc/table_split.h
@@ -0,0 +1,32 @@
+#pragma once
+#include <stdint.h>
+
+constexpr int64_t SBG_TABLE_MAX_TILES = (int64_t)1 << 30;
+
+static inline int sbg_table_next_launch(const int* tiles, int count, int first, int max_entries, int* tile0)
+{
+    if (count < 0 || first < 0 || first > count || max_entries < 1 || !tile0) return -1;
+    if (count > 0 && !tiles) return -1;
+    int64_t sum = 0;
+    int n = 0;
+    tile0[0] = 0;
+    while (first + n < count && n < max_entries) {
+        const int t = tiles[first + n];
+        if (t < 0 || (int64_t)t > SBG_TABLE_MAX_TILES) return -1;
+        if (n > 0 && sum + t > SBG_TABLE_MAX_TILES) break;
+        sum += t;
+        n++;
+        tile0[n] = (int)sum;
+    }
+    return n;
+}
+
+#ifdef __HIPCC__
+__host__ __device__
+#endif
+static inline int sbg_table_find(const int* tile0, int n, int wg)
+{
+    int e = 0;
+    while (e + 1 < n && wg >= tile0[e + 1]) e++;
+    return e;
+}
diff --git a/style-big-gan_amd/csrc/weight_prep.hip b/style-big-gan_amd/csrc/weight_prep.hip
--- a/style-big-gan_amd/csrc/weight_prep.hip
+++ b/style-big-gan_amd/csrc/weight_prep.hip
@@ -1,4 +1,5 @@
 #include "sbg_common.h"
+#include <vector>
 
 namespace {
 
@@ -295,3 +296,230 @@
     SBG_HIP_LAUNCH_CHECK();
     return 0;
 }
+
+
+#include "table_split.h"
+
+namespace {
+
+enum { PATH_PAIRS = 0, PATH_TILES = 1, PATH_SPLIT = 2 };
+
+struct PackTable { sbg_pack_desc e[SBG_TABLE_MAX]; int tile0[SBG_TABLE_MAX + 1]; int count; };
+static_assert(sizeof(PackTable) <= 4096, "the pack table must fit the kernel arguments");
+
+template <class T, int K>
+__device__ __forceinline__ void table_pack_pairs(const sbg_pack_desc& p, int tile, int ntiles)
+{
+    const unsigned total = (unsigned)p.A * (unsigned)p.Bp, step = (unsigned)ntiles * 256u;
+    const int KH = K ? K : p.KH, KW = K ? K : p.KW;
+    T* out = (T*)p.out;
+    for (unsigned i = (unsigned)tile * 256u + threadIdx.x; i < total; i += step) {
+        const int a = (int)(i / (unsigned)p.Bp), b = (int)(i - (unsigned)a * (unsigned)p.Bp);
+        const bool real = b < p.B;
+        const float* src = p.w + (int64_t)a * p.sA + (int64_t)b * p.sB;
+        float sq = 0.0f;
+        if constexpr (K > 0) {
+            float v[K * K];
+#pragma unroll
+            for (int t = 0; t < K * K; t++) v[t] = real ? src[(t / K) * p.sKH + (t % K) * p.sKW] * p.gain : 0.0f;
+#pragma unroll
+            for (int t = 0; t < K * K; t++) {
+                sq = __builtin_fmaf(v[t], v[t], sq);
+                Elem<T>::st(out + ((int64_t)t * p.A + a) * p.Bp + b, v[t]);
+            }
+        } else {
+            for (int kh = 0; kh < KH; kh++)
+                for (int kw = 0; kw < KW; kw++) {
+                    const float x = real ? src[kh * p.sKH + kw * p.sKW] * p.gain : 0.0f;
+                    sq = __builtin_fmaf(x, x, sq);
+                    Elem<T>::st(out + ((int64_t)(kh * KW + kw) * p.A + a) * p.Bp + b, x);
+                }
+        }
+        if (p.w2 && real) p.w2[(int64_t)a * p.B + b] = sq;
+    }
+}
+
+template <class T>
+__device__ __forceinline__ void table_pack_pairs_any(const sbg_pack_desc& p, int tile, int ntiles)
+{
+    if (p.KH == 3 && p.KW == 3)      table_pack_pairs<T, 3>(p, tile, ntiles);
+    else if (p.KH == 1 && p.KW == 1) table_pack_pairs<T, 1>(p, tile, ntiles);
+    else                             table_pack_pairs<T, 0>(p, tile, ntiles);
+}
+
+template <class T>
+__device__ __forceinline__ void table_pack_tiles(const sbg_pack_desc& p, int tile, float (&lds)[32][33])
+{
+    const int tx = threadIdx.x & 31, ty = threadIdx.x >> 5;
+    const int atiles = (p.A + 31) / 32, btiles = (p.Bp + 31) / 32;
+    const int a0 = (tile % atiles) * 32, b0 = ((tile / atiles) % btiles) * 32, t = tile / (atiles * btiles);
+    const int kh = t / p.KW, kw = t - kh * p.KW;
+    const float* src = p.w + (int64_t)kh * p.sKH + (int64_t)kw * p.sKW;
+#pragma unroll
+    for (int r = 0; r < 4; r++) {
+        const int a = a0 + tx, b = b0 + ty + 8 * r;
+        lds[ty + 8 * r][tx] = (a < p.A && b < p.B) ? src[(int64_t)a * p.sA + (int64_t)b * p.sB] * p.gain : 0.0f;
+    }
+    __syncthreads();
+    T* out = (T*)p.out + (int64_t)t * p.A * p.Bp;
+#pragma unroll
+    for (int r = 0; r < 4; r++) {
+        const int a = a0 + ty + 8 * r, b = b0 + tx;
+        if (a < p.A && b < p.Bp) Elem<T>::st(out + (int64_t)a * p.Bp + b, lds[tx][ty + 8 * r]);
+    }
+}
+
+__device__ __forceinline__ void table_pack_split(const sbg_pack_desc& p, int tile, int ntiles)
+{
+    const int64_t total = (int64_t)p.KH * p.KW * p.A * p.B;
+    unsigned short* y = (unsigned short*)p.out;
+    for (int64_t idx = (int64_t)tile * 256 + threadIdx.x; idx < total; idx += (int64_t)ntiles * 256) {
+        const int b = (int)(idx % p.B);
+        const int64_t ta = idx / p.B;
+        const int a = (int)(ta % p.A), t = (int)(ta / p.A);
+        const int kh = t / p.KW, kw = t - kh * p.KW;
+        float v = p.w[(int64_t)kh * p.sKH + (int64_t)kw * p.sKW + (int64_t)a * p.sA + (int64_t)b * p.sB];
+        unsigned short part[3];
+#pragma unroll
+        for (int k = 0; k < 3; k++) { part[k] = f32_to_bf16_bits(v); v -= bf16_bits_to_f32(part[k]); }
+        unsigned short* dst = y + ((int64_t)t * p.A + a) * ((int64_t)p.nseg * p.B) + b;
+        for (int s = 0; s < p.nseg; s++) {
+            const int o = p.order[s];
+            dst[(int64_t)s * p.B] = o == 0 ? part[0] : o == 1 ? part[1] : part[2];
+        }
+    }
+}
+
+__global__ void __launch_bounds__(256) pack_weight_table_kernel(PackTable tb)
+{
+    __shared__ float lds[32][33];
+    const int pi = sbg_table_find(tb.tile0, tb.count, (int)blockIdx.x);
+    const sbg_pack_desc& p = tb.e[pi];
+    const int tile = (int)blockIdx.x - tb.tile0[pi], ntiles = tb.tile0[pi + 1] - tb.tile0[pi];
+    if (p.kind == PATH_SPLIT) { table_pack_split(p, tile, ntiles); return; }
+    if (p.kind == PATH_TILES) {
+        if (p.out_dtype == SBG_BF16)     table_pack_tiles<bf16_s>(p, tile, lds);
+        else if (p.out_dtype == SBG_F16) table_pack_tiles<f16_s>(p, tile, lds);
+        else                             table_pack_tiles<float>(p, tile, lds);
+        return;
+    }
+    if (p.out_dtype == SBG_BF16)     table_pack_pairs_any<bf16_s>(p, tile, ntiles);
+    else if (p.out_dtype == SBG_F16) table_pack_pairs_any<f16_s>(p, tile, ntiles);
+    else                             table_pack_pairs_any<float>(p, tile, ntiles);
+}
+
+struct DemodTable { sbg_demod_desc e[SBG_TABLE_MAX]; int tile0[SBG_TABLE_MAX + 1]; int count; float eps; };
+static_assert(sizeof(DemodTable) <= 4096, "the demodulation table must fit the kernel arguments");
+
+constexpr int DEMOD_NB = 8, DEMOD_R = 8;
+
+__global__ void __launch_bounds__(256) demod_coefs_table_kernel(DemodTable tb)
+{
+    const int pi = sbg_table_find(tb.tile0, tb.count, (int)blockIdx.x);
+    const sbg_demod_desc& p = tb.e[pi];
+    const int lane = threadIdx.x & 63;
+    const int64_t w = (int64_t)((int)blockIdx.x - tb.tile0[pi]) * 4 + (threadIdx.x >> 6);
+    const int nruns = (p.N + DEMOD_NB - 1) / DEMOD_NB;
+    if (w >= (int64_t)p.O * nruns) return;
+    const int o = (int)(w % p.O), n0 = (int)(w / p.O) * DEMOD_NB;
+    const float* wr = p.w2 + (int64_t)o * p.I;
+    const bool held = p.I <= 64 * DEMOD_R;
+    float wv[DEMOD_R];
+#pragma unroll
+    for (int r = 0; r < DEMOD_R; r++) wv[r] = (held && lane + 64 * r < p.I) ? wr[lane + 64 * r] : 0.0f;
+#pragma unroll
+    for (int k = 0; k < DEMOD_NB; k++) {
+        const int n = n0 + k;
+        if (n >= p.N) break;
+        const float* sr = p.styles + (int64_t)n * p.I;
+        float acc = 0.0f;
+        if (held) {
+#pragma unroll
+            for (int r = 0; r < DEMOD_R; r++)
+                if (lane + 64 * r < p.I) { const float sv = sr[lane + 64 * r]; acc = __builtin_fmaf(sv * sv, wv[r], acc); }
+        } else {
+            for (int i = lane; i < p.I; i += 64) { const float sv = sr[i]; acc = __builtin_fmaf(sv * sv, wr[i], acc); }
+        }
+#pragma unroll
+        for (int m = 32; m >= 1; m >>= 1) acc += __shfl_xor(acc, m, 64);
+        if (lane == 0) p.dcoefs[(int64_t)n * p.O + o] = rsqrtf(acc + tb.eps);
+    }
+}
+
+}
+
+extern "C" int sbg_pack_weight_table(const sbg_pack_desc* entries, int count, sbg_stream_t stream_)
+{
+    SBG_CHECK(count >= 0 && (entries || count == 0), "pack_weight_table: bad table");
+    if (count == 0) return 0;
+    hipStream_t stream = (hipStream_t)stream_;
+    std::vector<int> tiles((size_t)count), path((size_t)count);
+    double bytes = 0.0;
+    for (int i = 0; i < count; i++) {
+        const sbg_pack_desc& d = entries[i];
+        SBG_CHECK(d.w && d.out, "pack_weight_table: entry %d: null pointer", i);
+        SBG_CHECK(d.A >= 1 && d.B >= 1 && d.KH >= 1 && d.KW >= 1 && d.Bp >= d.B, "pack_weight_table: entry %d: bad sizes", i);
+        if (d.kind == SBG_PACK_SPLIT) {
+            SBG_CHECK(d.nseg >= 1 && d.nseg <= 8 && d.Bp == d.B && !d.w2 && d.gain == 1.0f && d.out_dtype == SBG_BF16,
+                      "pack_weight_table: entry %d: a split entry has 1..8 parts, no padding, no w2, gain 1, bf16 output", i);
+            SBG_CHECK(d.sA >= 0 && d.sB >= 0 && d.sKH >= 0 && d.sKW >= 0, "pack_weight_table: entry %d: negative stride", i);
+            for (int s = 0; s < d.nseg; s++) SBG_CHECK(d.order[s] <= 2, "pack_weight_table: entry %d: part index out of range", i);
+            const int64_t total = (int64_t)d.A * d.B * d.KH * d.KW;
+            SBG_CHECK(total * d.nseg <= INT32_MAX, "pack_weight_table: entry %d: tensor too large", i);
+            path[i] = PATH_SPLIT; tiles[i] = (int)sbg_stream_grid(total, 256);
+            bytes += (double)total * (4.0 + 2.0 * d.nseg);
+            continue;
+        }
+        SBG_CHECK(d.kind == SBG_PACK_CAST, "pack_weight_table: entry %d: bad kind %d", i, d.kind);
+        SBG_CHECK(d.out_dtype == SBG_BF16 || d.out_dtype == SBG_F16 || d.out_dtype == SBG_F32, "pack_weight_table: entry %d: bad dtype %d", i, d.out_dtype);
+        SBG_CHECK((int64_t)d.A * d.Bp * d.KH * d.KW <= INT32_MAX, "pack_weight_table: entry %d: tensor too large", i);
+        const bool transposing = !d.w2 && d.sA == 1 && d.sB >= 64 && d.A >= 32 && d.B >= 32 && d.KH * d.KW <= 65535;
+        path[i] = transposing ? PATH_TILES : PATH_PAIRS;
+        tiles[i] = transposing ? ((d.A + 31) / 32) * ((d.Bp + 31) / 32) * (d.KH * d.KW) : (int)sbg_stream_grid((int64_t)d.A * d.Bp, 256);
+        bytes += (double)d.A * d.B * d.KH * d.KW * (4.0 + sbg_dtype_size(d.out_dtype));
+    }
+    for (int first = 0; first < count;) {
+        PackTable tb;
+        const int n = sbg_table_next_launch(tiles.data(), count, first, SBG_TABLE_MAX, tb.tile0);
+        SBG_CHECK(n >= 1, "pack_weight_table: cannot split the table");
+        for (int i = 0; i < n; i++) { tb.e[i] = entries[first + i]; tb.e[i].kind = path[first + i]; }
+        tb.count = n;
+        if (tb.tile0[n] > 0) {
+            SbgProfScope prof(stream, SBG_K_WEIGHT_PREP, 0.0, first == 0 ? bytes : 0.0, {n, tb.tile0[n], count, 6, 0, 0, 0});
+            SBG_LAUNCH(pack_weight_table_kernel, dim3((unsigned)tb.tile0[n]), dim3(256), 0, stream, tb);
+            SBG_HIP_LAUNCH_CHECK();
+        }
+        first += n;
+    }
+    return 0;
+}
+
+extern "C" int sbg_demod_coefs_table(const sbg_demod_desc* entries, int count, float eps, sbg_stream_t stream_)
+{
+    SBG_CHECK(count >= 0 && (entries || count == 0), "demod_coefs_table: bad table");
+    if (count == 0) return 0;
+    hipStream_t stream = (hipStream_t)stream_;
+    std::vector<int> tiles((size_t)count);
+    double flops = 0.0, bytes = 0.0;
+    for (int i = 0; i < count; i++) {
+        const sbg_demod_desc& d = entries[i];
+        SBG_CHECK(d.styles && d.w2 && d.dcoefs && d.N >= 1 && d.O >= 1 && d.I >= 1, "demod_coefs_table: entry %d: bad arguments", i);
+        const int64_t waves = (int64_t)d.O * ((d.N + DEMOD_NB - 1) / DEMOD_NB);
+        SBG_CHECK((waves + 3) / 4 <= SBG_TABLE_MAX_TILES, "demod_coefs_table: entry %d: too large", i);
+        tiles[i] = (int)((waves + 3) / 4);
+        flops += 2.0 * d.N * d.O * (double)d.I;
+        bytes += 4.0 * ((double)d.N * d.I + (double)d.O * d.I + (double)d.N * d.O);
+    }
+    for (int first = 0; first < count;) {
+        DemodTable tb;
+        const int n = sbg_table_next_launch(tiles.data(), count, first, SBG_TABLE_MAX, tb.tile0);
+        SBG_CHECK(n >= 1, "demod_coefs_table: cannot split the table");
+        for (int i = 0; i < n; i++) tb.e[i] = entries[first + i];
+        tb.count = n; tb.eps = eps;
+        SbgProfScope prof(stream, SBG_K_WEIGHT_PREP, first == 0 ? flops : 0.0, first == 0 ? bytes : 0.0, {n, tb.tile0[n], count, 7, 0, 0, 0});
+        SBG_LAUNCH(demod_coefs_table_kernel, dim3((unsigned)tb.tile0[n]), dim3(256), 0, stream, tb);
+        SBG_HIP_LAUNCH_CHECK();
+        first += n;
+    }
+    return 0;
+}
diff --git a/style-big-gan_amd/torch_utils/ops/conv2d_gradfix.py b/style-big-gan_amd/torch_utils/ops/conv2d_gradfix.py
--- a/style-big-gan_amd/torch_utils/ops/conv2d_gradfix.py
+++ b/style-big-gan_amd/torch_utils/ops/conv2d_gradfix.py
@@ -1,5 +1,5 @@
 import contextlib
-
+import ctypes
 import weakref
 
 import numpy as np
@@ -140,6 +140,10 @@
 _pack_cache = {}
 _ptr_epoch = {}
 
+table_paths = True
+
+_pack_plan = {}
+
 
 def _on_optimizer_step(optimizer, args, kwargs):
     for group in optimizer.param_groups:
@@ -155,6 +159,49 @@
 
 def invalidate_packed_weights():
     _pack_cache.clear()
+
+
+def _stamp(base):
+    return (base._version, _ptr_epoch.get(base.data_ptr(), 0))
+
+
+def refresh_packed_weights(params=None):
+    if not table_paths or not _pack_plan:
+        return 0
+    ids = None if params is None else {id(q) for q in params}
+    by_device, dead = {}, []
+    for key, (ref, delta, desc) in _pack_plan.items():
+        base = ref()
+        if base is None or base.data_ptr() != key[0]:
+            dead.append(key)
+            continue
+        if ids is not None and id(base) not in ids:
+            continue
+        stamp = _stamp(base)
+        hit = _pack_cache.get(key)
+        if hit is not None and hit[0]() is base and hit[1] == stamp:
+            continue
+        by_device.setdefault(base.device, []).append((key, base, stamp, hit, delta, desc))
+    for key in dead:
+        del _pack_plan[key]
+        _pack_cache.pop(key, None)
+    total = 0
+    for device, stale in by_device.items():
+        table = (_lib.PackDesc * len(stale))()
+        fresh = []
+        for i, (key, base, stamp, hit, delta, desc) in enumerate(stale):
+            if hit is not None and hit[0]() is base:
+                out, w2 = hit[2], hit[3]
+            else:
+                out = torch.empty([desc.KH * desc.KW, desc.A, desc.Bp], dtype=key[5], device=device)
+                w2 = torch.empty([desc.A, desc.B], dtype=torch.float32, device=device) if key[4] == 0 else None
+            desc.w, desc.out, desc.w2 = key[0] + delta, out.data_ptr(), (w2.data_ptr() if w2 is not None else None)
+            table[i] = desc
+            fresh.append((key, (weakref.ref(base), stamp, out, w2)))
+        _lib.check(_lib.load().sbg_pack_weight_table(ctypes.addressof(table), len(stale), _lib.stream_ptr(device)), "sbg_pack_weight_table")
+        _pack_cache.update(fresh)
+        total += len(stale)
+    return total
 
 
 def is_mixed(x, w):
@@ -171,7 +218,7 @@
     if cacheable:
         key = (base.data_ptr(), w.storage_offset(), tuple(w.shape), tuple(w.stride()), rows_dim, dtype, bp, float(gain))
         hit = _pack_cache.get(key)
-        stamp = (base._version, _ptr_epoch.get(base.data_ptr(), 0))
+        stamp = _stamp(base)
         if hit is not None and hit[0]() is base and hit[1] == stamp:
             return hit[2], hit[3]
     out = torch.empty([kh * kw, A, bp], dtype=dtype, device=w.device)
@@ -185,7 +232,13 @@
                 del _pack_cache[k]
             if len(_pack_cache) > 2048:
                 _pack_cache.clear()
-        _pack_cache[key] = (weakref.ref(base), (base._version, _ptr_epoch.get(base.data_ptr(), 0)), out, w2)
+        _pack_cache[key] = (weakref.ref(base), _stamp(base), out, w2)
+        if key not in _pack_plan:
+            if len(_pack_plan) > 2048:
+                _pack_plan.clear()
+            desc = _lib.PackDesc(sA=wd.stride(a_dim), sB=wd.stride(b_dim), sKH=wd.stride(2), sKW=wd.stride(3), A=A, B=B, KH=kh, KW=kw, Bp=bp,
+                                 out_dtype=_lib.dtype_code(dtype), kind=_lib.SBG_PACK_CAST, gain=float(gain))
+            _pack_plan[key] = (weakref.ref(base), wd.data_ptr() - base.data_ptr(), desc)
     return out, w2
 
 
@@ -353,7 +406,7 @@
     return y.to(x.dtype) if y.dtype != x.dtype else y
 
 
-def _wgrad(a, b, stride, taps):
+def _wgrad(a, b, stride, taps, dest=None):
     lib = _lib.load()
     assert a.dtype == b.dtype and a.shape[0] == b.shape[0]
     ca, cb = a.shape[1], b.shape[1]
@@ -363,14 +416,17 @@
         a = torch.nn.functional.pad(a, (0, 32 - pw))
     ap, bp = _pad_channels(a), _pad_channels(b)
     cap, cbp = ap.shape[1], bp.shape[1]
-    out = torch.empty([len(taps), cap, cbp], dtype=torch.float32, device=a.device)
+    out = None
     first = True
-    for aa, bb in _mfma_operands(ap, bp, 0, 0):
+    passes = _mfma_operands(ap, bp, 0, 0)
+    if dest is not None and (len(passes) != 1 or len(taps) > _lib.SBG_MAX_TAPS):
+        dest = None
+    for aa, bb in passes:
         aa, bb = _cl(aa), _cl(bb)
         for g0 in range(0, len(taps), _lib.SBG_MAX_TAPS):
             grp = taps[g0:g0 + _lib.SBG_MAX_TAPS]
             p = _lib.WgradParams()
-            p.a, p.b, p.out = aa.data_ptr(), bb.data_ptr(), out[g0:].data_ptr()
+            p.a, p.b = aa.data_ptr(), bb.data_ptr()
             p.dtype = _lib.dtype_code(aa.dtype)
             p.N, p.PH, p.PW, p.Ca = aa.shape[0], aa.shape[2], aa.shape[3], cap
             p.BH, p.BW, p.Cb = bb.shape[2], bb.shape[3], cbp
@@ -385,6 +441,18 @@
                 _lib.check(1, "sbg_conv2d_wgrad_workspace")
             ws = torch.empty([max(nbytes, 4) // 4], dtype=torch.float32, device=a.device) if nbytes > 0 else None
             p.workspace = ws.data_ptr() if ws is not None else None
+            if dest is not None and nbytes > 0:
+                wshape, wstride, w, dw2 = dest['wshape'], dest['wstride'], dest.get('w'), dest.get('dw2')
+                assert wshape[0] <= cap and wshape[1] <= cbp and wshape[2] * wshape[3] == len(taps)
+                dw = dest['dw'] = torch.empty_strided(wshape, wstride, dtype=torch.float32, device=a.device)
+                p.dw, p.dw_w, p.dw_dw2, p.dw_gain = dw.data_ptr(), _lib.ptr(w), _lib.ptr(dw2), float(dest['gain'])
+                p.dw_sA, p.dw_sB, p.dw_sKH, p.dw_sKW = wstride
+                p.dw_A, p.dw_B, p.dw_KW = wshape[0], wshape[1], wshape[3]
+                _lib.check(lib.sbg_conv2d_wgrad(p, _lib.stream_ptr(a.device)), "sbg_conv2d_wgrad")
+                return None
+            if out is None:
+                out = torch.empty([len(taps), cap, cbp], dtype=torch.float32, device=a.device)
+            p.out = out[g0:].data_ptr()
             _lib.check(lib.sbg_conv2d_wgrad(p, _lib.stream_ptr(a.device)), "sbg_conv2d_wgrad")
         first = False
     return out[:, :ca, :cb]
@@ -446,11 +514,14 @@
         assert stride[0] == stride[1]
         if dy.dtype != x.dtype:
             dy = dy.to(x.dtype)
+        dest = dict(wshape=wshape, wstride=wmeta, gain=wgain) if wmeta is not None and table_paths else None
         if not transpose:
-            out = _wgrad(dy, x, stride[0], taps)
+            out = _wgrad(dy, x, stride[0], taps, dest)
         else:
-            out = _wgrad(x, dy, stride[0], taps)
-        if wmeta is not None:
+            out = _wgrad(x, dy, stride[0], taps, dest)
+        if out is None:
+            dw = dest['dw']
+        elif wmeta is not None:
             dw = _unpack_wgrad(out, wshape[0], wshape[1], wshape, wmeta, 0, wgain)
         else:
             dw = out.reshape(kh, kw, wshape[0], wshape[1]).permute(2, 3, 0, 1).to(x.dtype)
diff --git a/style-big-gan_amd/torch_utils/ops/modconv.py b/style-big-gan_amd/torch_utils/ops/modconv.py
--- a/style-big-gan_amd/torch_utils/ops/modconv.py
+++ b/style-big-gan_amd/torch_utils/ops/modconv.py
@@ -1,3 +1,5 @@
+import ctypes
+
 import torch
 
 from ... import _lib
@@ -84,8 +86,10 @@
         n = styles.shape[0]
         _, w2 = _cg._packed_weight(weight, 0, act_dtype, (i + 7) // 8 * 8, 1.0)
         s32 = styles.detach().to(torch.float32).contiguous()
-        d = torch.empty([n, o], dtype=torch.float32, device=weight.device)
-        _lib.check(_lib.load().sbg_demod_coefs(s32.data_ptr(), w2.data_ptr(), d.data_ptr(), n, o, i, 1e-8, _lib.stream_ptr(weight.device)), "sbg_demod_coefs")
+        d = _table_rows(weight, s32, w2)
+        if d is None:
+            d = torch.empty([n, o], dtype=torch.float32, device=weight.device)
+            _lib.check(_lib.load().sbg_demod_coefs(s32.data_ptr(), w2.data_ptr(), d.data_ptr(), n, o, i, 1e-8, _lib.stream_ptr(weight.device)), "sbg_demod_coefs")
         ctx.save_for_backward(weight, s32, w2, d)
         ctx.s_dtype = styles.dtype
         return d
@@ -108,6 +112,46 @@
         return dw, (ds.to(ctx.s_dtype) if ds is not None else None), None
 
 
+_demod_rows = {}
+
+
+def demod_coefs_table(layers, act_dtype):
+    if not layers:
+        return []
+    dev = layers[0][0].device
+    rows = [(st.shape[0], w.shape[0], w.shape[1]) for w, st in layers]
+    flat = torch.empty([sum(n * o for n, o, _ in rows)], dtype=torch.float32, device=dev)
+    table = (_lib.DemodDesc * len(layers))()
+    off, token = 0, []
+    for q, (w, st), (n, o, i) in zip(table, layers, rows):
+        assert st.dtype == torch.float32 and st.is_contiguous() and st.shape[1] == i and w.dtype == torch.float32
+        _, w2 = _cg._packed_weight(w, 0, act_dtype, (i + 7) // 8 * 8, 1.0)
+        d = flat[off:off + n * o].view(n, o)
+        off += n * o
+        q.styles, q.w2, q.dcoefs, q.N, q.O, q.I = st.data_ptr(), w2.data_ptr(), d.data_ptr(), n, o, i
+        _demod_rows[id(w)] = (st.detach(), w2, d)
+        token.append(id(w))
+    _lib.check(_lib.load().sbg_demod_coefs_table(ctypes.addressof(table), len(layers), 1e-8, _lib.stream_ptr(dev)), "sbg_demod_coefs_table")
+    return token
+
+
+def demod_coefs_table_done(token):
+    for k in token:
+        _demod_rows.pop(k, None)
+
+
+def _table_rows(weight, s32, w2):
+    rec = _demod_rows.get(id(weight))
+    if rec is None or rec[1] is not w2:
+        return None
+    full, _, d = rec
+    row = full.shape[1] * 4
+    delta = s32.data_ptr() - full.data_ptr()
+    if s32.shape[1] != full.shape[1] or delta < 0 or delta % row or delta // row + s32.shape[0] > full.shape[0]:
+        return None
+    return d.narrow(0, delta // row, s32.shape[0])
+
+
 def demod_coefs(weight, styles, act_dtype):
     return _DemodCoefs.apply(weight, styles, act_dtype)
 
diff --git a/style-big-gan_amd/train_parts/generators.py b/style-big-gan_amd/train_parts/generators.py
--- a/style-big-gan_amd/train_parts/generators.py
+++ b/style-big-gan_amd/train_parts/generators.py
@@ -513,18 +513,35 @@
         tail, chunk = plan if plan is not None else (0, ws.shape[0])
         head = len(self.block_resolutions) - tail
         bank = self._style_bank(ws)
-        for res, cur_ws in zip(self.block_resolutions[:head], per_block[:head]):
-            x, img = getattr(self, f'b{res}')(x, img, cur_ws, styles=(bank[res] if bank else None), **block_kwargs)
-        if tail > 0:
-            imgs = []
-            for i in range(0, ws.shape[0], chunk):
-                xc, ic = x.narrow(0, i, chunk), (img.narrow(0, i, chunk) if img is not None else None)
-                for res, cur_ws in zip(self.block_resolutions[head:], per_block[head:]):
-                    st = tuple(None if s is None else s.narrow(0, i, chunk) for s in bank[res]) if bank else None
-                    xc, ic = getattr(self, f'b{res}')(xc, ic, cur_ws.narrow(0, i, chunk), styles=st, **block_kwargs)
-                imgs.append(ic)
-            img = misc.cat0(imgs)
+        demod = self._demod_table(bank, block_kwargs)
+        try:
+            for res, cur_ws in zip(self.block_resolutions[:head], per_block[:head]):
+                x, img = getattr(self, f'b{res}')(x, img, cur_ws, styles=(bank[res] if bank else None), **block_kwargs)
+            if tail > 0:
+                imgs = []
+                for i in range(0, ws.shape[0], chunk):
+                    xc, ic = x.narrow(0, i, chunk), (img.narrow(0, i, chunk) if img is not None else None)
+                    for res, cur_ws in zip(self.block_resolutions[head:], per_block[head:]):
+                        st = tuple(None if s is None else s.narrow(0, i, chunk) for s in bank[res]) if bank else None
+                        xc, ic = getattr(self, f'b{res}')(xc, ic, cur_ws.narrow(0, i, chunk), styles=st, **block_kwargs)
+                    imgs.append(ic)
+                img = misc.cat0(imgs)
+        finally:
+            modconv.demod_coefs_table_done(demod)
         return img
+
+    def _demod_table(self, bank, block_kwargs):
+        if bank is None or not (conv2d_gradfix.table_paths and modconv.enabled) or block_kwargs.get('force_fp32'):
+            return []
+        layers = []
+        for res in self.block_resolutions:
+            block = getattr(self, f'b{res}')
+            if not block.use_fp16:
+                continue
+            for conv, st in ((block.conv0 if block.in_channels != 0 else None, bank[res][0]), (block.conv1, bank[res][1])):
+                if conv is not None and st is not None and conv.weight.dtype == torch.float32 and conv.weight.is_cuda:
+                    layers.append((conv.weight, st))
+        return modconv.demod_coefs_table(layers, LOW_PRECISION)
 
     def _style_bank(self, ws):
         if not (style_bank_enabled and ws.is_cuda and ws.dtype == torch.float32 and (modconv.enabled or not torch.is_grad_enabled())):
diff --git a/style-big-gan_amd/train_parts/trainers.py b/style-big-gan_amd/train_parts/trainers.py
--- a/style-big-gan_amd/train_parts/trainers.py
+++ b/style-big-gan_amd/train_parts/trainers.py
@@ -9,6 +9,7 @@
 from .. import utils
 from ..parallel import GradReducer
 from ..torch_utils import misc, training_stats
+from ..torch_utils.ops import conv2d_gradfix
 from ..utils import EasyDict
 from .discriminators import discriminators
 from .generators import generators
@@ -220,6 +221,10 @@
                 self._phase_events[phase.name] = None
                 events[0].record(torch.cuda.current_stream(self.device))
             with torch.autograd.profiler.record_function(phase.name):
+                if self.device.type == 'cuda':
+                    if getattr(self, '_pack_params', None) is None:
+                        self._pack_params = list(self.G.parameters()) + list(self.D.parameters())
+                    conv2d_gradfix.refresh_packed_weights(self._pack_params)
                 for r in phase.reducers:
                     r.zero_grad()
                 phase.module.requires_grad_(True)
```
